# BruceCanovas/supersurfel_fusion

Hardware: AMD Instinct MI355X
Metric: frames_per_sec (higher is better)
Workload: dtype f32; 1 GPU; 640x480 synthetic RGB-D orbit (seed 1234), map seeded with 1000000 supersurfels (~993223 live, ~86081 visible), reference rgbd_benchmark parameters, extract+ICP+fuse per frame; width=640, height=480, n_model=993223, n_visible=86081, superpixels=1200, icp_iter_max=10, icp_forced=False, seed_order=seeded, exchange=none, pipeline_depth=2, extract_batch=8

## Files before the change

### supersurfel_fusion_amd/csrc/lab/host_probes.inc

```

int ssf_dbg_last_icp_record(ssf_handle* h, int64_t* out29) {
    if (!h || !out29) return SSF_ERR_INVALID_ARG;
    for (int i = 0; i < 29; i++) out29[i] = h->h_icp_local[i];
    return SSF_OK;
}
int ssf_dbg_device_icp_records(ssf_handle* h, int64_t* out64) {
    if (!h || !out64) return SSF_ERR_INVALID_ARG;
    HCK(hipStreamSynchronize(h->stream));
    HCK(hipMemcpy(out64, h->d_icp, 64 * sizeof(int64_t), hipMemcpyDeviceToHost));
    return SSF_OK;
}
void ssf_dbg_stall_before_match_us(ssf_handle* h, long long us) { if (h) h->dbg_stall_before_match_us = us; }
int ssf_dbg_host_times(ssf_handle* h, double* out8) {
    if (!h || !out8) return SSF_ERR_INVALID_ARG;
    for (int i = 0; i < 8; i++) { out8[i] = h->host_us[i]; h->host_us[i] = 0; }
    return SSF_OK;
}
double ssf_dbg_extract_only(ssf_handle* h, const void* const* rgb, const void* const* depth, int nlist, int n) {
    if (!h || !rgb || !depth || nlist <= 0 || !h->pending.empty()) return -1.0;
    int nsub = 0;
    double t0 = 0;
    for (int i = 0; i < n; i++) {
        if (i == n / 4) { for (auto& c : h->ctx) (void)hipStreamSynchronize(c.stream); (void)hipStreamSynchronize(h->stream); t0 = now_us(); }
        while (nsub < n && !h->ctx[h->open_ctx].launched) {
            if (submit_extract(h, rgb[nsub % nlist], depth[nsub % nlist], 1, nullptr)) return -1.0;
            nsub++;
        }
        if (activate_oldest(h) || retire_active(h)) return -1.0;
        h->stamp++;
    }
    for (auto& c : h->ctx) (void)hipStreamSynchronize(c.stream);
    (void)hipStreamSynchronize(h->stream);
    return (now_us() - t0) / (double)(n - n / 4);
}
double ssf_dbg_time_icp(ssf_handle* h, int reps, int dbg) {
    if (!h || !h->have_frame) return -1.0;
    Rt T; T.R = m3_transpose(h->pose.R); T.t = negate(m3_mulv(T.R, h->pose.t));
    hipEvent_t e0, e1; (void)hipEventCreate(&e0); (void)hipEventCreate(&e1);
    for (int i = 0; i < 3; i++) launch_icp(h->stream, h->cam, h->model[h->mcur], h->n_visible, h->cc->maps.pix2, h->cc->maps.fpack, T, h->d_icp_replicas, h->d_tickets + 8, h->d_icp, h->mb_dev, ++h->icp_seq, dbg);
    (void)hipEventRecord(e0, h->stream);
    for (int i = 0; i < reps; i++) launch_icp(h->stream, h->cam, h->model[h->mcur], h->n_visible, h->cc->maps.pix2, h->cc->maps.fpack, T, h->d_icp_replicas, h->d_tickets + 8, h->d_icp, h->mb_dev, ++h->icp_seq, dbg);
    (void)hipEventRecord(e1, h->stream);
    (void)hipStreamSynchronize(h->stream);
    float ms = 0.f; (void)hipEventElapsedTime(&ms, e0, e1);
    (void)hipMemsetAsync(h->d_icp_replicas, 0, 2 * SSF_ICP_REPLICAS * 32 * sizeof(long long), h->stream);
    (void)hipMemsetAsync(h->d_tickets, 0, 512 * sizeof(unsigned int), h->stream);
    (void)hipStreamSynchronize(h->stream);
    (void)hipEventDestroy(e0); (void)hipEventDestroy(e1);
    return 1000.0 * ms / reps;
}
double ssf_dbg_time_fuse(ssf_handle* h, int reps, int mode, long long* blocks2 ) {
    if (!h || !h->have_frame || !h->cc) return -1.0;
    SurfelSoA& M = h->model[h->mcur];
    PartitionWs ws;
    uint32_t* set = h->d_part + (size_t)h->part_set * h->part_words;
    ws.sup_vis = set; ws.sup_oov = set + h->part_sup_vis; ws.tot = ws.sup_oov + h->part_sup_oov;
    ws.ticket = h->d_part_ticket; ws.other = h->d_part + (size_t)(h->part_set ^ 1) * h->part_words; ws.words = h->part_words;
    const int S = (mode & 2) ? 0 : h->S, nvis = (mode & 4) ? 0 : h->n_visible, span = (mode & 1) ? 0 : h->oov_tail - h->oov_head;
    auto launch = [&] {
        ClassifyArgs ca = h->classify; ca.plane_depth = h->cc->maps.plane_depth;
        launch_fuse(h->stream, M, h->cc->frame, h->pose, h->stamp, h->id_offset, nvis, AssocTables{h->cc->d_best, h->cc->d_matched, h->d_cand, S},
                    (nvis > 0 && S > 0) ? 1 : 0, h->cfg.nb_supersurfels_max, ShardArgs{0, 1, 0, h->cfg.shard_tile}, h->d_cnt,
                    h->oov[h->ocur], span, ca, h->d_state, h->d_state_oov, h->d_bc_oov, ws, 1);
    };
    hipEvent_t e0, e1; (void)hipEventCreate(&e0); (void)hipEventCreate(&e1);
    for (int i = 0; i < 3 && reps > 0; i++) launch();
    (void)hipEventRecord(e0, h->stream);
    for (int i = 0; i < reps; i++) launch();
    (void)hipEventRecord(e1, h->stream);
    (void)hipStreamSynchronize(h->stream);
    float ms = 0.f; (void)hipEventElapsedTime(&ms, e0, e1);
    (void)hipEventDestroy(e0); (void)hipEventDestroy(e1);
    if (blocks2) {
        const int nb = (span + 255) / 256;
        std::vector<uint32_t> bc((size_t)std::max(nb, 1));
        if (nb > 0) (void)hipMemcpy(bc.data(), h->d_bc_oov, (size_t)nb * 4, hipMemcpyDeviceToHost);
        blocks2[0] = nb; blocks2[1] = 0;
        for (int i = 0; i < nb; i++) blocks2[1] += bc[i] != 0u;
    }
    return reps > 0 ? 1000.0 * ms / reps : 0.0;
}
int ssf_dbg_trace_fuse(ssf_handle* h, unsigned long long* out, int cap_wgs, int* arms4, int mode ) {
    if (!h || !h->have_frame || !h->cc || !out || !arms4) return -1;
    arms4[0] = (mode & 2) ? 0 : (h->S + 31) / 32; arms4[1] = (mode & 2) ? 0 : (h->S + 255) / 256; arms4[2] = (mode & 4) ? 0 : (h->n_visible + 255) / 256;
    long long b2[2];
    unsigned long long* d = nullptr;
    const size_t words = (size_t)3 * 65536;
    if (hipMalloc((void**)&d, words * 8) != hipSuccess) return -2;
    (void)hipMemset(d, 0, words * 8);
    set_fuse_trace(d);
    (void)ssf_dbg_time_fuse(h, 1, mode, b2);
    set_fuse_trace(nullptr);
    std::vector<unsigned long long> all(words);
    (void)hipMemcpy(all.data(), d, words * 8, hipMemcpyDeviceToHost);
    (void)hipFree(d);
    int n = 0;
    for (int i = 0; i < 65536; i++) if (all[3 * (size_t)i]) n = i + 1;
    arms4[3] = n - arms4[0] - arms4[1] - arms4[2];
    const int m = n < cap_wgs ? n : cap_wgs;
    std::memcpy(out, all.data(), (size_t)m * 24);
    return m;
}
int ssf_dbg_pass_stats_enable(int on) { set_pass_stats(on ? 1 : 0); return SSF_OK; }
int ssf_dbg_pass_stats(ssf_handle* h, uint32_t* out64) {
    if (!h || !h->active.ctx || !out64) return SSF_ERR_INVALID_ARG;
    HCK(hipStreamSynchronize(h->active.ctx->stream));
    HCK(hipMemcpy(out64, h->active.maps.epoch, 64 * sizeof(uint32_t), hipMemcpyDeviceToHost));
    return SSF_OK;
}
double ssf_dbg_time_pass(ssf_handle* h, int reps, int rgbd, int dbg, int nb) {
    if (!h || !h->active.ctx) return -1.0;
    ExtractCtx& c = *h->active.ctx;
    nb = std::max(1, std::min(nb, h->batch));
    hipEvent_t e0, e1; (void)hipEventCreate(&e0); (void)hipEventCreate(&e1);
    const int ox[4] = {0, 1, 0, 1}, oy[4] = {0, 1, 1, 0};
    for (int i = 0; i < 4; i++) launch_update_pass(h->stream, h->seg, c.maps, nb, 20 + i, ox[i & 3], oy[i & 3], rgbd != 0, dbg);
    (void)hipEventRecord(e0, h->stream);
    for (int i = 0; i < reps; i++) launch_update_pass(h->stream, h->seg, c.maps, nb, 24 + i, ox[i & 3], oy[i & 3], rgbd != 0, dbg);
    (void)hipEventRecord(e1, h->stream);
    (void)hipStreamSynchronize(h->stream);
    float ms = 0.f; (void)hipEventElapsedTime(&ms, e0, e1);
    (void)hipEventDestroy(e0); (void)hipEventDestroy(e1);
    return 1000.0 * ms / reps;
}
int ssf_dbg_trace_pass(ssf_handle* h, int rgbd, int nb, unsigned long long* out, int cap_wgs, int* grid3) {
    if (!h || !h->active.ctx || !out || !grid3) return -1;
    ExtractCtx& c = *h->active.ctx;
    nb = std::max(1, std::min(nb, h->batch));
    const int ox[4] = {0, 1, 0, 1}, oy[4] = {0, 1, 1, 0};
    grid3[0] = (h->cfg.width + 30 + 31) / 32; grid3[1] = (h->cfg.height + 31) / 32; grid3[2] = nb;
    const int n = grid3[0] * grid3[1] * grid3[2];
    unsigned long long* d = nullptr;
    if (hipMalloc((void**)&d, (size_t)n * 40) != hipSuccess) return -2;
    (void)hipMemset(d, 0, (size_t)n * 40);
    for (int i = 0; i < 4; i++) launch_update_pass(h->stream, h->seg, c.maps, nb, 20 + i, ox[i & 3], oy[i & 3], rgbd != 0, 0);
    (void)hipStreamSynchronize(h->stream);
    set_pass_trace(d);
    launch_update_pass(h->stream, h->seg, c.maps, nb, 24, ox[0], oy[0], rgbd != 0, 0);
    (void)hipStreamSynchronize(h->stream);
    set_pass_trace(nullptr);
    const int m = std::min(n, cap_wgs);
    (void)hipMemcpy(out, d, (size_t)m * 40, hipMemcpyDeviceToHost);
    (void)hipFree(d);
    return m;
// ... 2 lines not shown
```

### supersurfel_fusion_amd/csrc/ssf_device.hpp

```cpp
#pragma once
#include <hip/hip_runtime.h>
#include <stdint.h>
#include <cstddef>
#include "ssf_math.hpp"
#include "../../include/ssf.h"
#include "../../include/ssf_input.h"
#include "../../include/ssf_dynamic.h"

#ifdef SSF_EXPERIMENTS
#include <stdlib.h>
static inline int ssf_env_int_(const char* name, int dflt) { const char* e = getenv(name); return e ? atoi(e) : dflt; }
#define SSF_ENV_INT(name, dflt) ssf_env_int_("SSF_" name, dflt)
#define SSF_ENV_SET(name) (getenv("SSF_" name) != nullptr)
#define SSF_ENV_STR(name) getenv("SSF_" name)
#define SSF_PROBE(dbg, bits) ((((dbg)) & (bits)) != 0)
#else
#define SSF_PROBE(dbg, bits) (false)
#define SSF_ENV_INT(name, dflt) (dflt)
#define SSF_ENV_SET(name) (false)
#define SSF_ENV_STR(name) ((const char*)nullptr)
#endif

namespace ssf {

// ... 77 lines not shown
    for (int i = 0; i < 3; i++) {
        m.log.ent[i] = slab_shift(m.log.ent[i], o); m.log.disp[i] = slab_shift(m.log.disp[i], o);
        m.log.count[i] = slab_shift(m.log.count[i], o);
    }
    m.sp = slab_shift(m.sp, o); m.samples = slab_shift(m.samples, o); m.sample_score = slab_shift(m.sample_score, o);
    m.moments = slab_shift(m.moments, o); m.filt = slab_shift(m.filt, o); m.epoch = slab_shift(m.epoch, o);
    m.pix2 = slab_shift(m.pix2, o); m.fpack = slab_shift(m.fpack, o);
    return m;
}
SSF_HD SurfelSoA batch_slot(SurfelSoA s, size_t o) {
    s.pos = slab_shift(s.pos, o); s.col = slab_shift(s.col, o); s.lab = slab_shift(s.lab, o); s.stamps = slab_shift(s.stamps, o);
    s.r0 = slab_shift(s.r0, o); s.r1 = slab_shift(s.r1, o); s.r2 = slab_shift(s.r2, o); s.shape = slab_shift(s.shape, o);
    s.dims = slab_shift(s.dims, o); s.conf = slab_shift(s.conf, o);
    return s;
}
struct BatchIn {
    const uint8_t* rgb[SSF_MAX_BATCH];
    const void* depth[SSF_MAX_BATCH];
    int color_format, depth_format;
    double depth_scale;
};
template <typename T> SSF_HD T batch_pick(const T* arr, int b) {
    T v = arr[0];
#pragma unroll
    for (int i = 1; i < SSF_MAX_BATCH; i++) v = (b == i) ? arr[i] : v;
    return v;
}

struct Mailbox {
    alignas(64) unsigned long long icp_rec[40];
    Counters cnt;
    unsigned long long cnt_check;
    unsigned long long cnt_seq;
    int all_cnt[5 * SSF_MAX_RANKS];
    unsigned long long all_check;
    unsigned long long all_seq;
    unsigned int p2p_timeout;
    unsigned int extract_abort;
};
#ifndef SSF_ICP_REPLICAS
#define SSF_ICP_REPLICAS 8
#endif
#define SSF_ICP_REC_WORD(w, p, seq) ((((w) & 7) == 7) ? (unsigned long long)(seq) : ((7 * ((w) >> 3) + ((w) & 7)) < 30 ? (unsigned long long)(p)[7 * ((w) >> 3) + ((w) & 7)] : 0ull))

void launch_ingest(hipStream_t st, const SegParams& p, const BatchIn& in, FrameMaps& m, int nb, uint32_t epoch0);
int pass_tile_npx(int nb);
void launch_update_pass(hipStream_t st, const SegParams& p, FrameMaps& m, int nb, int k, int ox, int oy, bool rgbd, int dbg = 0);
size_t pass_team_ws_bytes();
size_t pass_args_bytes(int kmax);
void pass_args_table(const SegParams& p, const FrameMaps& m, int kmax, void* host_out);
void launch_update_passes_team(hipStream_t st, const SegParams& p, FrameMaps& m, int nb, int k0, int k1, bool rgbd, const void* d_pas, void* d_ws,
                               unsigned int* abort_flag);
void launch_init_samples(hipStream_t st, const SegParams& p, FrameMaps& m, int nb, int true_buf);
void launch_eval_samples(hipStream_t st, const SegParams& p, FrameMaps& m, int nb);
void launch_init_disp(hipStream_t st, const SegParams& p, FrameMaps& m, int nb, bool ransac);
void launch_plane_filter(hipStream_t st, const SegParams& p, FrameMaps& m, int nb, int true_buf);
void launch_import_frame(hipStream_t st, const SegParams& p, FrameMaps& m, int nb, SurfelSoA frame, const float* wire, unsigned long long* best, uint8_t* matched);
void launch_export_rows(hipStream_t st, const SegParams& p, const FrameMaps& m, int nb, SurfelSoA frame, float* wire);
void launch_render_moments(hipStream_t st, const SegParams& p, const Cam& cam, FrameMaps& m, int nb);
void launch_render_moments_pixmask(hipStream_t st, const SegParams& p, const Cam& cam, FrameMaps& m, int nb, const uint8_t* pixmask,
                                   uint32_t* pixcnt);
void launch_finalize_surfels(hipStream_t st, const SegParams& p, FrameMaps& m, int nb, SurfelSoA frame, float zmin,
                             float zmax, int stamp0, const uint8_t* dynamic_mask, unsigned mask_bits,
                             unsigned long long* best, uint8_t* matched);
void launch_finalize_surfels_pixmask(hipStream_t st, const SegParams& p, FrameMaps& m, int nb, SurfelSoA frame, float zmin, float zmax,
                                     int stamp0, const uint8_t* dynamic_mask, unsigned mask_bits, unsigned long long* best, uint8_t* matched,
                                     const uint32_t* pixcnt, unsigned pixmask_bits);
void launch_bilateral(hipStream_t st, const void* in, int depth_format, double depth_scale, float* out, int W, int H, float sigma_color,
                      float sigma_space);
void launch_bilateral_batch(hipStream_t st, const BatchIn& in, float* out0, size_t slab, int nb, int W, int H, float sigma_color, float sigma_space);
void launch_boundary_map(hipStream_t st, const SegParams& p, const int32_t* label, int32_t* out);
void launch_preview(hipStream_t st, int W, int H, const int32_t* label, const uint32_t* rgba, uint8_t* out );

struct alignas(64) IcpGo { float T[12]; unsigned long long flag; unsigned long long x; };
static_assert(sizeof(IcpGo) == 64, "one line");
#define SSF_ICP_GO_ABORT (1ull << 63)
#define SSF_ICP_GO_MATCH (1ull << 62)
#define SSF_ICP_GO_CHECK_MASK 0x3FFFFFFFu
SSF_HD unsigned int icp_go_word_weight(unsigned int dword) {
    return dword < 12u ? (2u * dword + 1u) * 0x9E3779B1u : (dword == 14u ? 0x85EBCA6Bu : (dword == 15u ? 0xC2B2AE35u : 0u));
}
SSF_HD unsigned int icp_go_abort_check(unsigned int want) { return ((want * 0x9E3779B1u) >> 2) & SSF_ICP_GO_CHECK_MASK; }
#define SSF_ICP_GO_SLOTS 4
struct MatchArgs { float zmin, zmax; long long id_offset; unsigned long long* best; uint8_t* matched; int32_t* cand; };
struct ClassifyArgs { Cam cam; const float* plane_depth; int delta_t; float conf_thresh, zmin, zmax; };
struct ShardArgs { int rank, nranks, migrate; float tile; };
struct AssocTables { const unsigned long long* best; const uint8_t* matched; const int32_t* cand; int S; };
int icp_variant_mode();
void launch_icp(hipStream_t st, const Cam& cam, SurfelSoA model, int n_visible, const uint2* pix2, const float4* fpack,
                Rt T, long long* replicas, unsigned int* ticket,
                long long* sums29, Mailbox* mb, unsigned long long seq, int dbg = -1, IcpGo* go = nullptr,
                unsigned long long go_seq = 0, const struct P2PView* pv = nullptr, int by_tile = 0, const MatchArgs* match = nullptr);
int icp_resident_max_wgs();
void launch_icp_resident(hipStream_t st, const Cam& cam, SurfelSoA model, int n_visible, const uint2* pix2, const float4* fpack, const Rt* T0,
                         long long* replicas, long long* sums29, Mailbox* mb, unsigned long long seq0, IcpGo* go, unsigned int go_base,
                         int last_idx, const MatchArgs* match);
void launch_bin_rows(hipStream_t st, const Cam& cam, SurfelSoA model, int n, Rt T, uint32_t* count, uint32_t* cursor, SurfelSoA out);
size_t bin_buffer_words(const Cam& cam, size_t capacity);
void launch_match(hipStream_t st, const Cam& cam, SurfelSoA model, int n_visible, const uint2* pix2, const float4* fpack,
                  Rt pose, float zmin, float zmax, long long id_offset,
                  unsigned long long* best, uint8_t* matched, int32_t* cand , int S,
                  const int32_t* orig = nullptr );
struct OovStore { SurfelSoA rows; uint8_t* live; int cap; };
#define PART_GROUP 16
#define PART_REPLICAS 8
struct PartitionWs { uint32_t* sup_vis; uint32_t* sup_oov; uint32_t* tot; uint32_t* ticket; uint32_t* other; int words; };
void launch_fuse(hipStream_t st, SurfelSoA model , SurfelSoA frame, Rt pose, int stamp, long long id_offset,
                 int n_visible, const AssocTables& at, int do_update, int capacity, const ShardArgs& sh, Counters* cnt, OovStore oov,
                 int span_upper, const ClassifyArgs& ca, uint8_t* state_vis, uint8_t* state_oov, uint32_t* bc_oov, const PartitionWs& ws,
                 int tail_in_move = 0 );
#ifdef SSF_EXPERIMENTS
void set_pass_stats(int on);
void set_pass_trace(unsigned long long* device_words );
void set_fuse_trace(unsigned long long* device_words );
#endif
struct MoveTotals { int from_tot, nv , head_old, tail_old ; };
void launch_pack_emigrants(hipStream_t st, SurfelSoA model, const AssocTables& at, long long id_offset, int n_visible,
                           const uint8_t* state_vis, int do_update, const ShardArgs& sh, int32_t* table);
void launch_migrate_in(hipStream_t st, SurfelSoA model, const int32_t* table, int S, int capacity, Counters* cnt, const ShardArgs& sh,
                       const ClassifyArgs& ca, Rt pose, int stamp, uint8_t* state_vis, const PartitionWs& ws);
void launch_rehome_split(hipStream_t st, SurfelSoA dense, int n, int n_visible, int rank, int nranks, float tile, uint32_t* bc, int* tot3,
                         SurfelSoA stay, int32_t* table, int table_rows);
void launch_rehome_unpack(hipStream_t st, const int32_t* table, int n, SurfelSoA dst, int base);
void launch_first_frame(hipStream_t st, SurfelSoA model, SurfelSoA frame, Rt pose, int S, int capacity, const ShardArgs& sh, Counters* cnt);
struct NextIcp {
    Cam cam; const uint2* pix2; const float4* fpack;
    Rt T;
    long long* replicas; unsigned int* ticket; long long* sums; Mailbox* mb; unsigned long long seq;
};
void launch_move_rows(hipStream_t st, SurfelSoA vis_src, SurfelSoA vis_dst, OovStore oov, int nv_upper, int span_upper,
                      const uint8_t* state_vis, const uint8_t* state_oov, const uint32_t* bc_oov, const PartitionWs& ws,
                      Counters* cnt , Mailbox* mb, unsigned long long cnt_seq, const NextIcp* next,
                      const struct P2PView* next_pv = nullptr, const MoveTotals* totals = nullptr);
void launch_oov_compact(hipStream_t st, OovStore src, OovStore dst, int span_upper, int new_head, uint32_t* bc_oov, Counters* cnt,
                        int set_span);
struct ModelView { SurfelSoA vis; OovStore oov; int n_visible, nbv, nvs, oov_head, oov_tail, nbo, nslots; };
void launch_align(hipStream_t st, const Cam& cam, const float* spos, const float* slab, const float* snrm, const float* sconf,
                  int n, SurfelSoA frame, const int32_t* label, const float* plane_depth, Rt T, long long* out40);
void launch_fern_codes(hipStream_t st, const uint8_t* rgb, const float* depth, int W, int H, const uint32_t* fpos,
                       const uint8_t* frgb, const float* fdepth, int n, uint8_t* codes);
#define SSF_P2P_MAX_RANKS 8
struct P2PView { unsigned char* peer[SSF_P2P_MAX_RANKS]; int me, nranks, S; unsigned long long seq, timeout_ticks; };
enum { P2P_FLAG_ASSOC = 0, P2P_FLAG_MIGR = 1 };
#define SSF_P2P_HEADER 8192
SSF_HD size_t p2p_slot(int par, int src) { return (size_t)(par * SSF_P2P_MAX_RANKS + src); }
SSF_HD size_t p2p_spad(int S) { return ((size_t)S + 63) & ~(size_t)63; }
SSF_HD size_t p2p_off_icp(int par, int src) { return p2p_slot(par, src) * 320; }
SSF_HD size_t p2p_off_cnt(int par, int src) { return 16 * 320 + p2p_slot(par, src) * 64; }
SSF_HD size_t p2p_off_flag(int kind, int par, int src) { return 16 * 384 + ((size_t)kind * 16 + p2p_slot(par, src)) * 64; }
SSF_HD size_t p2p_off_best(int S, int par, int src) { return SSF_P2P_HEADER + p2p_slot(par, src) * (size_t)S * 8; }
SSF_HD size_t p2p_off_matched(int S, int par, int src) { return SSF_P2P_HEADER + 16 * (size_t)S * 8 + p2p_slot(par, src) * p2p_spad(S); }
SSF_HD size_t p2p_off_migr(int S, int par, int src) {
    return SSF_P2P_HEADER + 16 * (size_t)S * 8 + 16 * p2p_spad(S) + p2p_slot(par, src) * (size_t)S * SSF_MIGRANT_WORDS * 4;
}
SSF_HD size_t p2p_region_bytes(int S) { return p2p_off_migr(S, 1, SSF_P2P_MAX_RANKS - 1) + (size_t)S * SSF_MIGRANT_WORDS * 4; }
void launch_p2p_counts(hipStream_t st, const P2PView& pv, const Counters* cnt, Mailbox* mb, unsigned long long all_seq);
void launch_p2p_assoc(hipStream_t st, const P2PView& pv, unsigned long long* best, uint8_t* matched, Mailbox* mb);
void launch_p2p_migrants(hipStream_t st, const P2PView& pv, int32_t* table, unsigned int* ticket , Mailbox* mb);
void launch_publish_icp(hipStream_t st, const long long* rec29, Mailbox* mb, unsigned long long seq);
void launch_publish_all_counts(hipStream_t st, const int* all5, int nranks, Mailbox* mb, unsigned long long seq);
void launch_publish_counts(hipStream_t st, Counters* cnt, int shrink_by_removed, Mailbox* mb, unsigned long long seq);
void launch_lab_refresh(hipStream_t st, SurfelSoA s, int n);
void launch_pack_orient(hipStream_t st, SurfelSoA s, int n, float* out9);
void launch_deformation(hipStream_t st, SurfelSoA model, int n, int m, const float* npos, const float* nrot,
                        const float* ntrans, float* nodes16, const float* w4, const int32_t* idx4);

struct KernelTimer;
KernelTimer* current_timer();
void set_current_timer(KernelTimer* t);
void timer_begin(KernelTimer* t, const char* name, hipStream_t st);
// ... 9 lines not shown
```

### supersurfel_fusion_amd/csrc/ssf_extract.hip

```cpp
#include <stdio.h>
#include <stdlib.h>
#include <string.h>
#include <algorithm>
#include <mutex>
#include "ssf_device.hpp"

namespace ssf {

#define HIP_CHECK_LAUNCH() (void)hipGetLastError()

__device__ __forceinline__ int lane_id() { return threadIdx.x & 63; }
__device__ __forceinline__ void atomic_add_i64(long long* p, long long v) {
    atomicAdd(reinterpret_cast<unsigned long long*>(p), static_cast<unsigned long long>(v));
}
template <int CF> __device__ __forceinline__ uint32_t load_rgb(const uint8_t* __restrict__ p, size_t q) {
    if (CF == SSF_COLOR_RGBA8 || CF == SSF_COLOR_BGRA8) {
        const uint32_t v = reinterpret_cast<const uint32_t*>(p)[q];
        return CF == SSF_COLOR_RGBA8 ? (v & 0xFFFFFFu) : (((v & 0xFFu) << 16) | (v & 0xFF00u) | ((v >> 16) & 0xFFu));
    }
    const uint32_t c0 = p[3 * q], c1 = p[3 * q + 1], c2 = p[3 * q + 2];
    return CF == SSF_COLOR_BGR8 ? (c2 | (c1 << 8) | (c0 << 16)) : (c0 | (c1 << 8) | (c2 << 16));
}
template <int DF> __device__ __forceinline__ float load_depth(const void* __restrict__ p, size_t q, double scale) {
    if (DF == SSF_DEPTH_U16_SCALED) return (float)((double)reinterpret_cast<const uint16_t*>(p)[q] * scale);
// ... 994 lines not shown
            for (int j = 0; j < 12; j++) lds_add_i64(&a[j], fx64((double)v[j], SSF_MOM_SCALE, SSF_MOM_LIM));
            lds_add_i64(&a[12], 1);
        } else {
#pragma unroll
            for (int j = 0; j < 12; j++) atomic_add_i64(&m.moments[(size_t)label * 13 + j], fx64((double)v[j], SSF_MOM_SCALE, SSF_MOM_LIM));
            atomic_add_i64(&m.moments[(size_t)label * 13 + 12], 1);
        }
    }
#pragma unroll
    for (int k = 0; k < PX; k++) {
        if (out_label[k] < 0) continue;
        const int i = threadIdx.x + 256 * k;
        const size_t q = (size_t)(Y0 + i / TILE) * p.W + (X0 + i % TILE);
        m.plane_depth[q] = out_depth[k];
        m.pix2[q] = make_uint2((uint32_t)out_label[k], __float_as_uint(out_depth[k]));
    }
    __syncthreads();
    for (int i = threadIdx.x; i < win.size() * 13; i += blockDim.x) {
        long long v = 0;
#pragma unroll
        for (int r = 0; r < MOM_REP(WCAP); r++) v += (long long)w_acc[((i / 13) * MOM_REP(WCAP) + r) * 13 + i % 13];
        if (v != 0) atomic_add_i64(&m.moments[(size_t)win.label_of(i / 13, p.gy) * 13 + i % 13], v);
    }
    if constexpr (PIXMASK)
        for (int i = threadIdx.x; i < win.size(); i += blockDim.x) {
            uint32_t v = 0;
#pragma unroll
            for (int r = 0; r < MOM_REP(WCAP); r++) v += w_pix[i * MOM_REP(WCAP) + r];
            if (v == 0) continue;
            const size_t l = (size_t)win.label_of(i, p.gy);
            atomicAdd(&pixcnt[2 * l], v & 0xFFFFu);
            if (v >> 16) atomicAdd(&pixcnt[2 * l + 1], v >> 16);
        }
}

#define FIN_PER_WG 64
template <bool PIXMASK>
__global__ __launch_bounds__(256) void k_finalize_surfels(SegParams p, FrameMaps m, SurfelSoA f, float zmin, float zmax, int stamp0,
                                                          const uint8_t* __restrict__ dyn_mask, unsigned mask_bits,
                                                          unsigned long long* __restrict__ best, uint8_t* __restrict__ matched,
                                                          const uint32_t* __restrict__ pixcnt, unsigned pixmask_bits) {
    __shared__ float s_axis[2][FIN_PER_WG][3];
    const int wv = threadIdx.x >> 6, l = threadIdx.x & 63;
    const int kk = wv < 2 ? wv * 32 + (l >> 1) : l;
    const int k = blockIdx.x * FIN_PER_WG + kk;
    const bool active = k < p.S && wv < 3;
    const int fb = blockIdx.y;
    const size_t off = (size_t)fb * m.slab;
    m = batch_slot(m, fb); f = batch_slot(f, off);
    best = slab_shift(best, off); matched = slab_shift(matched, off);
    dyn_mask = ((mask_bits >> fb) & 1u) ? slab_shift(dyn_mask, off) : nullptr;
    const int stamp = stamp0 + fb;
    float sum[12]; float conf = 0.f;
#pragma unroll
    for (int j = 0; j < 12; j++) sum[j] = 0.f;
    if (active) {
        const long long* a = &m.moments[(size_t)k * 13];
        const double inv = 1.0 / SSF_MOM_SCALE;
#pragma unroll
        for (int j = 0; j < 12; j++) sum[j] = (float)((double)a[j] * inv);
        conf = (float)a[12];
    }
    V3 pos = v3(sum[0], sum[1], sum[2]), col = v3(sum[3], sum[4], sum[5]);
    Sym3 shape = sym3(sum[6], sum[7], sum[8], sum[9], sum[10], sum[11]);
    const float z = pos.z / conf;
    const bool valid = active && isfinite(z) && conf > 100.0f && z > zmin && z < zmax;
    if (valid) {
        pos = v3(pos.x / conf, pos.y / conf, z);
        shape = sym_sub(sym_div(shape, conf), sym_outer(pos));
    }
    V3 lab = v3(0.f, 0.f, 0.f);
    if (wv < 2) {
        if (valid) {
            const V3 axis = principal_power(principal_start(shape, (l & 1) == 1));
            s_axis[l & 1][kk][0] = axis.x; s_axis[l & 1][kk][1] = axis.y; s_axis[l & 1][kk][2] = axis.z;
        }
    } else if (wv == 2 && active) {
        if (valid) col = lab_to_rgb(v3(col.x / conf, col.y / conf, col.z / conf));
        lab = rgb_to_lab(col);
    }
    __syncthreads();
    if (wv != 2 || !active) return;
    best[k] = SSF_NO_MATCH; matched[k] = 0;
    M3 vecs = m3(v3(0, 0, 0), v3(0, 0, 0), v3(0, 0, 0));
    float d0 = 0.f, d1 = 0.f; int s0 = 0, s1 = 0;
    if (valid) {
        V3 vals;
        principal_finish(shape, v3(s_axis[0][kk][0], s_axis[0][kk][1], s_axis[0][kk][2]),
                         v3(s_axis[1][kk][0], s_axis[1][kk][1], s_axis[1][kk][2]), vecs, vals);
        d0 = vals.x; d1 = vals.y; s0 = stamp; s1 = stamp;
        if (vals.x / vals.y > 50.0f) conf = -1.0f;
    } else
        conf = -1.0f;
    if (dyn_mask && dyn_mask[k]) conf = -1.0f;
    if constexpr (PIXMASK) {
        if ((pixmask_bits >> fb) & 1u) {
            const uint32_t* c = slab_shift(pixcnt, off);
            const uint32_t total = c[2 * k], masked = c[2 * k + 1];
            if (masked > 0u && 2ull * masked >= (unsigned long long)total) conf = -1.0f;
        }
    }
    f.pos[3 * k] = pos.x; f.pos[3 * k + 1] = pos.y; f.pos[3 * k + 2] = pos.z;
    f.col[3 * k] = col.x; f.col[3 * k + 1] = col.y; f.col[3 * k + 2] = col.z;
    f.lab[3 * k] = lab.x; f.lab[3 * k + 1] = lab.y; f.lab[3 * k + 2] = lab.z;
    f.stamps[2 * k] = s0; f.stamps[2 * k + 1] = s1;
    f.r0[3 * k] = vecs.r0.x; f.r0[3 * k + 1] = vecs.r0.y; f.r0[3 * k + 2] = vecs.r0.z;
    f.r1[3 * k] = vecs.r1.x; f.r1[3 * k + 1] = vecs.r1.y; f.r1[3 * k + 2] = vecs.r1.z;
    f.r2[3 * k] = vecs.r2.x; f.r2[3 * k + 1] = vecs.r2.y; f.r2[3 * k + 2] = vecs.r2.z;
    f.shape[6 * k] = shape.xx; f.shape[6 * k + 1] = shape.xy; f.shape[6 * k + 2] = shape.xz;
    f.shape[6 * k + 3] = shape.yy; f.shape[6 * k + 4] = shape.yz; f.shape[6 * k + 5] = shape.zz;
    f.dims[2 * k] = d0; f.dims[2 * k + 1] = d1;
    f.conf[k] = conf;
    m.fpack[4 * k] = make_float4(conf, lab.x, lab.y, lab.z);
    m.fpack[4 * k + 1] = make_float4(vecs.r2.x, vecs.r2.y, vecs.r2.z, 0.f);
    m.fpack[4 * k + 2] = make_float4(pos.x, pos.y, pos.z, 0.f);
}

__global__ __launch_bounds__(256) void k_import_frame(int P, int S, FrameMaps m, SurfelSoA f, const float* __restrict__ wire,
                                                      unsigned long long* __restrict__ best, uint8_t* __restrict__ matched) {
    {
        const size_t off = (size_t)blockIdx.y * m.slab;
        m = batch_slot(m, blockIdx.y); f = batch_slot(f, off); wire = slab_shift(wire, off);
        best = slab_shift(best, off); matched = slab_shift(matched, off);
    }
    const int i = blockIdx.x * blockDim.x + threadIdx.x;
    if (i < P) m.pix2[i] = make_uint2((uint32_t)m.label[i], __float_as_uint(m.plane_depth[i]));
    if (i >= S) return;
    const int k = i;
    const float* wpos = wire; const float* wcol = wpos + 3 * (size_t)S; const int32_t* wst = reinterpret_cast<const int32_t*>(wcol + 3 * (size_t)S);
    const float* wori = reinterpret_cast<const float*>(wst + 2 * (size_t)S); const float* wsh = wori + 9 * (size_t)S;
    const float* wd = wsh + 6 * (size_t)S; const float* wc = wd + 2 * (size_t)S;
    const V3 pos = v3(wpos[3 * k], wpos[3 * k + 1], wpos[3 * k + 2]), col = v3(wcol[3 * k], wcol[3 * k + 1], wcol[3 * k + 2]);
    const V3 lab = rgb_to_lab(col);
    const V3 r2 = v3(wori[9 * k + 6], wori[9 * k + 7], wori[9 * k + 8]);
    const float conf = wc[k];
    f.pos[3 * k] = pos.x; f.pos[3 * k + 1] = pos.y; f.pos[3 * k + 2] = pos.z;
    f.col[3 * k] = col.x; f.col[3 * k + 1] = col.y; f.col[3 * k + 2] = col.z;
    f.lab[3 * k] = lab.x; f.lab[3 * k + 1] = lab.y; f.lab[3 * k + 2] = lab.z;
    f.stamps[2 * k] = wst[2 * k]; f.stamps[2 * k + 1] = wst[2 * k + 1];
#pragma unroll
    for (int j = 0; j < 3; j++) { f.r0[3 * k + j] = wori[9 * k + j]; f.r1[3 * k + j] = wori[9 * k + 3 + j]; f.r2[3 * k + j] = wori[9 * k + 6 + j]; }
#pragma unroll
    for (int j = 0; j < 6; j++) f.shape[6 * k + j] = wsh[6 * k + j];
    f.dims[2 * k] = wd[2 * k]; f.dims[2 * k + 1] = wd[2 * k + 1];
    f.conf[k] = conf;
    m.fpack[4 * k] = make_float4(conf, lab.x, lab.y, lab.z);
    m.fpack[4 * k + 1] = make_float4(r2.x, r2.y, r2.z, 0.f);
    m.fpack[4 * k + 2] = make_float4(pos.x, pos.y, pos.z, 0.f);
    best[k] = SSF_NO_MATCH; matched[k] = 0;
}

__global__ __launch_bounds__(256) void k_export_rows(int S, SurfelSoA f, float* __restrict__ wire, size_t slab) {
    const int k = blockIdx.x * blockDim.x + threadIdx.x;
    if (k >= S) return;
    const size_t off = (size_t)blockIdx.y * slab;
    f = batch_slot(f, off); wire = slab_shift(wire, off);
    float* wpos = wire; float* wcol = wpos + 3 * (size_t)S; int32_t* wst = reinterpret_cast<int32_t*>(wcol + 3 * (size_t)S);
    float* wori = reinterpret_cast<float*>(wst + 2 * (size_t)S); float* wsh = wori + 9 * (size_t)S;
    float* wd = wsh + 6 * (size_t)S; float* wc = wd + 2 * (size_t)S;
#pragma unroll
    for (int j = 0; j < 3; j++) {
        wpos[3 * k + j] = f.pos[3 * k + j]; wcol[3 * k + j] = f.col[3 * k + j];
        wori[9 * k + j] = f.r0[3 * k + j]; wori[9 * k + 3 + j] = f.r1[3 * k + j]; wori[9 * k + 6 + j] = f.r2[3 * k + j];
    }
    wst[2 * k] = f.stamps[2 * k]; wst[2 * k + 1] = f.stamps[2 * k + 1];
#pragma unroll
    for (int j = 0; j < 6; j++) wsh[6 * k + j] = f.shape[6 * k + j];
    wd[2 * k] = f.dims[2 * k]; wd[2 * k + 1] = f.dims[2 * k + 1];
    wc[k] = f.conf[k];
}
__global__ __launch_bounds__(256) void k_boundary_map(SegParams p, const int32_t* __restrict__ label, int32_t* __restrict__ out) {
    __shared__ int tile[TW * TW];
    const int X0 = blockIdx.x * TILE, Y0 = blockIdx.y * TILE;
    load_label_tile(tile, label, X0, Y0, p.W, p.H);
    __syncthreads();
    for (int i = threadIdx.x; i < TILE * TILE; i += blockDim.x) {
        const int x = X0 + i % TILE, y = Y0 + i / TILE;
        if (x < p.W && y < p.H) out[(size_t)y * p.W + x] = tile_boundary(tile, i % TILE + 1, i / TILE + 1);
    }
}

__global__ __launch_bounds__(256) void k_preview(int W, int H, const int32_t* __restrict__ label, const uint32_t* __restrict__ rgba,
                                                 uint8_t* __restrict__ out) {
    const int x = blockIdx.x * 64 + (threadIdx.x & 63), y = blockIdx.y * 4 + (threadIdx.x >> 6);
    if (x >= W || y >= H) return;
    const size_t p = (size_t)y * W + x;
    const int index = label[p];
    uint8_t b0 = 255, b1 = 255, b2 = 255;
    if (!(x < W - 1 && y < H - 1 && (label[p + 1] != index || label[p + W + 1] != index))) {
        const uint32_t c = rgba[p];
        b0 = (uint8_t)(0.8f * (float)((c >> 16) & 255u)); b1 = (uint8_t)(0.8f * (float)((c >> 8) & 255u)); b2 = (uint8_t)(0.8f * (float)(c & 255u));
    }
    out[3 * p] = b0; out[3 * p + 1] = b1; out[3 * p + 2] = b2;
}
void launch_preview(hipStream_t st, int W, int H, const int32_t* label, const uint32_t* rgba, uint8_t* out) {
    hipLaunchKernelGGL(k_preview, dim3((W + 63) / 64, (H + 3) / 4), dim3(256), 0, st, W, H, label, rgba, out);
}

#define BIL_RMAX 16
#define BIL_TILE 16
__device__ __forceinline__ int reflect101(int i, int n) {
    if (n == 1) return 0;
    while (i < 0 || i >= n) i = (i < 0) ? -i : 2 * (n - 1) - i;
    return i;
}
template <int DF>
__global__ __launch_bounds__(256) void k_bilateral(BatchIn bin, float* __restrict__ out0, size_t slab, int W, int H,
                                                   int radius, float ss, float sc) {
    const void* __restrict__ in = batch_pick(bin.depth, (int)blockIdx.z);
    const double scale = bin.depth_scale;
    float* __restrict__ out = slab_shift(out0, (size_t)blockIdx.z * slab);
    __shared__ float tile[(BIL_TILE + 2 * BIL_RMAX) * (BIL_TILE + 2 * BIL_RMAX)];
    __shared__ int s_ext[2 * BIL_RMAX + 1];
    const int X0 = blockIdx.x * BIL_TILE, Y0 = blockIdx.y * BIL_TILE;
    const int tw = BIL_TILE + 2 * radius;
    const bool staged = radius <= BIL_RMAX;
    if (staged) {
        for (int i = threadIdx.x; i < tw * tw; i += blockDim.x) {
            const int gx = reflect101(X0 - radius + i % tw, W), gy = reflect101(Y0 - radius + i / tw, H);
            tile[i] = load_depth<DF>(in, (size_t)gy * W + gx, scale);
        }
        if ((int)threadIdx.x <= 2 * radius) {
            const int dy = (int)threadIdx.x - radius;
            int e = 0;
            while ((e + 1) * (e + 1) + dy * dy <= radius * radius) e++;
            s_ext[threadIdx.x] = e;
        }
    }
    __syncthreads();
    const int lx = threadIdx.x % BIL_TILE, ly = threadIdx.x / BIL_TILE;
    const int x = X0 + lx, y = Y0 + ly;
    if (x >= W || y >= H) return;
// ... 335 lines not shown
```

### supersurfel_fusion_amd/csrc/ssf_handle.hpp

```cpp
#pragma once
#include <algorithm>
#include <climits>
#include <cmath>
#include <cstring>
#include <deque>
#include <initializer_list>
#include <map>
#include <string>
#include <utility>
#include <vector>
#include "ssf_device.hpp"
#include "../../include/ssf_render.h"
#include "../../include/ssf_graph.h"
#include "../../include/ssf_graph_solve.h"
#include "../../include/ssf_keyframes.h"
#include "../../include/ssf_motion.h"
#include "../../include/ssf_odometry.h"
#include "../../include/ssf_navgrid.h"
#include "../../include/ssf_track.h"

struct ncclComm; typedef struct ncclComm* ncclComm_t;
struct Uploader;
namespace ssf {
struct KernelTimer {
// ... 158 lines not shown
    uint4* ferns = nullptr; uint32_t* q = nullptr; uint32_t* table = nullptr; int32_t* stamps = nullptr; uint32_t* diff = nullptr;
    int32_t* rec = nullptr; uint8_t* bytes = nullptr;
    ssf_surfels pool{};
    std::vector<ssf_fern> host_ferns; std::vector<KeyframeMeta> kfs; long long rows_used = 0;
};
struct QueryWs {
    DevBufs bufs;
    unsigned long long* mask = nullptr; uint32_t* cnt = nullptr; uint32_t* bc = nullptr; size_t slots = 0;
    uint32_t* rec = nullptr;
    unsigned char* rows = nullptr; size_t rows_bytes = 0;
};
struct NavGridWs {
    DevBufs bufs;
    float4* rec = nullptr; uint2* rbox = nullptr; size_t slots = 0;
    uint32_t* tcnt = nullptr; uint32_t* cursor = nullptr; size_t tiles = 0;
    uint32_t* list = nullptr; size_t list_cap = 0;
    uint32_t* acc = nullptr; uint16_t* colg = nullptr; int8_t* state = nullptr; size_t cells = 0;
    unsigned long long* stats = nullptr;
    unsigned char* img = nullptr; size_t img_bytes = 0;
};
struct RayIndex {
    float cell, s, k;
    uint32_t mask;
    int cmin[3], cmax[3];
    int n_over, nvs;
    float cabs;
};
struct RaycastWs {
    DevBufs bufs;
    float4* rec = nullptr; uint4* rbox = nullptr; uint32_t* bc = nullptr; uint32_t* over = nullptr; size_t slots = 0;
    uint32_t* off = nullptr; uint32_t* cursor = nullptr; size_t buckets = 0;
    uint32_t* list = nullptr; size_t list_cap = 0;
    unsigned long long* stats = nullptr; int* cbox = nullptr;
    unsigned char* io = nullptr; size_t io_bytes = 0;
    RayIndex ix{};
    bool built = false; unsigned long long gen = 0; long long recentres = 0; float cell = 0, s = 0; int hash_bits = 0;
    long long rows_indexed = 0, rows_oversize = 0, entries = 0;
};
struct ssf_handle {
    ssf_config cfg;
    int S = 0, gx = 0, gy = 0;
    std::string err;
    hipStream_t stream = nullptr; bool own_stream = false; int stream_prio = 0;
    SegParams seg; Cam cam;
    std::vector<ExtractCtx> ctx; int open_ctx = 0, batch = 1;
    std::deque<std::pair<int, int>> pending;
    ActiveFrame active; ActiveFrame* cc = &active;
    uint32_t extract_ordinal = 0;
    const void* const* seq_rgb = nullptr; const void* const* seq_depth = nullptr; const uint8_t* const* seq_pixmask = nullptr; int seq_next = 0, seq_n = 0, seq_on_device = 0, stamp_bias = 0;
    long long n_waiter_matches = 0;
    int seq_k = 0;
    int seq_batches = 0;
    double us_wait_upload = 0.0;
    Uploader* up = nullptr; bool seq_upload = false;
    int in_color = SSF_COLOR_RGB8, in_depth = SSF_DEPTH_F32_METRES; double in_scale = 1.0;
    ncclComm_t comm = nullptr; int* d_all5 = nullptr;
    int deal = 0; long long deal_batches = 0;
    struct P2P {
        unsigned char* region = nullptr; size_t bytes = 0; bool fine = false;
        bool same_device = false; double timeout_s = 30.0;
        P2PView view{}; bool on = false; std::vector<void*> opened;
        unsigned long long seq_icp = 0, seq_cnt = 0, seq_assoc = 0, seq_migr = 0;
    } p2p;
    unsigned long long all_seq = 0; bool all_pending = false, all_valid = false;
    long long all_cnt[5 * SSF_MAX_RANKS];
    SurfelSoA model[2]; int mcur = 0;
    std::vector<void*> allocs;
    struct Guarded { void* base; size_t bytes, guard; };
    std::vector<Guarded> guarded;
    float* d_bf_in = nullptr; float* d_bf_out = nullptr; float* d_orient9 = nullptr; float* d_frame_orient9 = nullptr;
    long long* d_icp = nullptr;
    uint8_t* d_state = nullptr; int32_t* d_cand = nullptr; Counters* d_cnt = nullptr;
    int32_t* d_migrants = nullptr; PartitionWs fuse_ws{}; bool fuse_first = false, fuse_migrate = false, fusing = false;
    MoveTotals fuse_totals{0, 0, 0, 0}; bool move_totals_on = true;
    OovStore oov[2]; int ocur = 0; int oov_head = 0, oov_tail = 0, oov_live = 0; long long n_recentres = 0;
    uint8_t* d_state_oov = nullptr; uint32_t* d_bc_oov = nullptr;
    uint32_t* d_part = nullptr; uint32_t* d_part_ticket = nullptr; int part_words = 0, part_sup_vis = 0, part_sup_oov = 0, part_set = 0;
    SurfelSoA dense; uint8_t* d_live_scratch = nullptr;
    int32_t* d_scratch_map = nullptr;
    long long* d_icp_replicas = nullptr; unsigned int* d_tickets = nullptr; float* d_srgb_lut = nullptr;
    Mailbox* mb_host = nullptr; Mailbox* mb_dev = nullptr;
    unsigned long long icp_seq = 0, cnt_seq = 0;
    struct { bool valid = false; unsigned long long seq = 0; ExtractCtx* ctx = nullptr; int slot = 0; int stamp = 0; Rt pose; } ahead;
    double wait_launched_us = 0.0; long long n_waiter_match_repairs = 0; long long dbg_stall_before_match_us = 0;
    bool icp_ahead = true; int icp_ahead_mode = 1;
    AheadTuner ahead_tuner;
    IcpGo* go = nullptr; bool icp_chain = true; unsigned long long go_count = 0;
    IcpGo* go_res = nullptr; int resident_max_rows = 0; long long n_resident_frames = 0, n_resident_ahead_frames = 0, n_resident_launches = 0;
    bool graph_failed = false; hipStream_t capture_stream = nullptr;
    TileCopy bins;
    ClassifyArgs classify{}; ShardArgs shard{};
    bool pass_team = false; ExtractCtx* team_prev = nullptr;
    long long h_icp_local[SSF_ICP_RECORD];
    long long* h_icp = nullptr; Counters* h_cnt = nullptr;
    int n_model = 0, n_visible = 0, stamp = 0, max_passes = 0;
    Rt pose;
    IcpLoop icp;
    long long id_offset = 0, global_n_model = -1, global_n_visible = -1;
    bool have_frame = false;
    int last_icp_valid = 0, last_icp_iters = 0;
    hipEvent_t ev[4] = {nullptr, nullptr, nullptr, nullptr};
    KernelTimer timer;
    std::vector<std::string> timer_names;
    double seq_mark_us[4][64] = {{0}}, seq_launch_us[32] = {0}, seq_launch_host_us[32] = {0}; int seq_launch_n[32] = {0}, seq_launches = 0;
    double seq_t0_us = 0, seq_done_us[64] = {0};
    double host_us[8] = {0, 0, 0, 0, 0, 0, 0, 0};
    RenderWs render;
    GraphWs graph;
    KeyframeWs kf;
    SolveWs solve;
    QueryWs query;
    MotionWs motion;
    OdoWs odo;
    NavGridWs navgrid;
    RaycastWs raycast;
    unsigned long long model_gen = 0;
};

#define HCK(call)                                                                                    \
    do {                                                                                             \
        hipError_t e_ = (call);                                                                      \
        if (e_ != hipSuccess) {                                                                      \
            h->err = std::string(#call) + ": " + hipGetErrorString(e_);                              \
            return SSF_ERR_DEVICE;                                                                   \
        }                                                                                            \
    } while (0)

#pragma GCC visibility push(hidden)
namespace ssf {
struct DevTemps {
    std::vector<void*> p;
    template <typename T> hipError_t take(T** out, size_t bytes) {
        void* q = nullptr;
        const hipError_t e = hipMalloc(&q, bytes ? bytes : 1);
        if (e == hipSuccess) { p.push_back(q); *out = (T*)q; }
        return e;
    }
    ~DevTemps() { for (void* q : p) (void)hipFree(q); }
};
struct TimerScope { ssf_handle* h; explicit TimerScope(ssf_handle* hh); ~TimerScope(); };
void timer_collect(KernelTimer* t);
inline int sync_collect(ssf_handle* h) {
    HCK(hipStreamSynchronize(h->stream)); if (h->cfg.profile == 1) timer_collect(&h->timer); return SSF_OK;
}
ModelView model_view(const ssf_handle* h, bool visible_only);
int model_at_rest(ssf_handle* h, const char* who = nullptr, const char* lacks = nullptr);
int materialise(ssf_handle* h);
bool frame_inputs_ok(ssf_handle* h, const void* rgb, const void* depth, int on_device);
int process_frame_devmask(ssf_handle* h, const void* rgb, const void* depth, int on_device, const float* prior, const uint8_t* d_pixmask,
                          ssf_frame_result* out);
int store_from_dense(ssf_handle* h, int n, int n_visible);
void drop_shard_sizes(ssf_handle* h);
void set_create_error(const char* what);
template <typename T> bool dalloc(ssf_handle* h, T** p, size_t count);
int wait_seq(ssf_handle* h, const volatile unsigned long long* word, unsigned long long want);
SurfelSoA soa_rows(const SurfelSoA& s, size_t r);
int copy_soa(ssf_handle* h, const SurfelSoA& d, const SurfelSoA& s, size_t n);
inline P2PView p2p_view(ssf_handle* h, unsigned long long seq) { P2PView v = h->p2p.view; v.seq = seq; return v; }
inline Rt pose_from12(const float* p) {
    Rt r; r.R = m3(v3(p[0], p[1], p[2]), v3(p[3], p[4], p[5]), v3(p[6], p[7], p[8])); r.t = v3(p[9], p[10], p[11]); return r;
}
inline void pose_to12(const Rt& r, float* p) {
    p[0] = r.R.r0.x; p[1] = r.R.r0.y; p[2] = r.R.r0.z; p[3] = r.R.r1.x; p[4] = r.R.r1.y; p[5] = r.R.r1.z;
    p[6] = r.R.r2.x; p[7] = r.R.r2.y; p[8] = r.R.r2.z; p[9] = r.t.x; p[10] = r.t.y; p[11] = r.t.z;
}
int align_loop(ssf_handle* h, const float* d_pos, const float* d_lab, const float* d_nrm, const float* d_conf, int n, long long* d_out,
// ... 13 lines not shown
```

### supersurfel_fusion_amd/csrc/ssf_host.hip

```cpp
#include <atomic>
#include <chrono>
#include <cstdio>
#include <cstdlib>
#include <new>
#include <condition_variable>
#include <mutex>
#include <thread>
#include <type_traits>
#include <unistd.h>
#include "ssf_exchange.hpp"
#include "ssf_solvers.hpp"

using namespace ssf;

namespace ssf {
static thread_local KernelTimer* g_timer = nullptr;
KernelTimer* current_timer() { return g_timer; }
void set_current_timer(KernelTimer* t) { g_timer = t; }
void timer_begin(KernelTimer* t, const char* name, hipStream_t st) {
    KernelTimer::Rec r;
    if (!t->pool_free.empty()) { r = t->pool_free.back(); t->pool_free.pop_back(); }
    else { (void)hipEventCreate(&r.e0); (void)hipEventCreate(&r.e1); }
    r.name = name;
    (void)hipEventRecord(r.e0, st);
// ... 673 lines not shown
int copy_soa(ssf_handle* h, const SurfelSoA& d, const SurfelSoA& s, size_t n) {
    if (n == 0) return SSF_OK;
    hipError_t copy_of_a_stream = hipSuccess;
    each_stream([&](auto m, size_t w) { if (!copy_of_a_stream) copy_of_a_stream = hipMemcpyAsync(d.*m, s.*m, 4 * w * n, hipMemcpyDeviceToDevice, h->stream); });
    HCK(copy_of_a_stream);
    return SSF_OK;
}
static int oov_home(const ssf_handle* h) { return h->cfg.nb_supersurfels_max + h->S + 256; }
static int oov_recentre(ssf_handle* h) {
    OovStore& src = h->oov[h->ocur]; OovStore& dst = h->oov[h->ocur ^ 1];
    HCK(hipMemsetAsync(dst.live, 0, (size_t)dst.cap, h->stream));
    launch_oov_compact(h->stream, src, dst, h->oov_tail - h->oov_head, oov_home(h), h->d_bc_oov, h->d_cnt, 1);
    HCK(hipGetLastError());
    h->ocur ^= 1;
    h->oov_head = oov_home(h); h->oov_tail = h->oov_head + h->oov_live;
    h->n_recentres++;
    return SSF_OK;
}
int materialise(ssf_handle* h) {
    int rc = copy_soa(h, h->dense, h->model[h->mcur], (size_t)h->n_visible);
    if (rc) return rc;
    if (h->oov_live > 0) {
        OovStore dst; dst.rows = h->dense; dst.live = h->d_live_scratch; dst.cap = h->cfg.nb_supersurfels_max;
        launch_oov_compact(h->stream, h->oov[h->ocur], dst, h->oov_tail - h->oov_head, h->n_visible, h->d_bc_oov, h->d_cnt, 0);
        HCK(hipGetLastError());
    }
    return SSF_OK;
}
int store_from_dense(ssf_handle* h, int n, int n_visible) {
    h->ahead.valid = false;
    h->bins.drop();
    h->model_gen++;
    int rc = copy_soa(h, h->model[h->mcur], h->dense, (size_t)n_visible);
    if (rc) return rc;
    OovStore& o = h->oov[h->ocur];
    const int head = oov_home(h), n_oov = n - n_visible;
    rc = copy_soa(h, soa_rows(o.rows, (size_t)head), soa_rows(h->dense, (size_t)n_visible), (size_t)n_oov);
    if (rc) return rc;
    HCK(hipMemsetAsync(o.live, 0, (size_t)o.cap, h->stream));
    if (n_oov > 0) HCK(hipMemsetAsync(o.live + head, 1, (size_t)n_oov, h->stream));
    Counters c; std::memset(&c, 0, sizeof(c));
    c.n_model = n; c.n_visible = n_visible; c.oov_head = head; c.oov_tail = head + n_oov; c.oov_live = n_oov;
    c.last[0] = n; c.last[1] = n_visible;
    HCK(hipStreamSynchronize(h->stream));
    HCK(hipMemcpy(h->d_cnt, &c, sizeof(c), hipMemcpyHostToDevice));
    h->n_model = n; h->n_visible = n_visible; h->oov_head = c.oov_head; h->oov_tail = c.oov_tail; h->oov_live = n_oov;
    return SSF_OK;
}
void drop_shard_sizes(ssf_handle* h) { h->all_valid = false; h->all_pending = false; }
}

static int do_match(ssf_handle* h, int exchange = 0) {
    const bool any = total_model(h) > 0 && total_visible(h) > 0;
    const int n = any ? h->n_visible : 0;
    launch_match(h->stream, h->cam, icp_rows(h), n, h->cc->maps.pix2, h->cc->maps.fpack, h->pose, h->cfg.range_min,
                 h->cfg.range_max, h->id_offset, h->cc->d_best, h->cc->d_matched, h->d_cand, h->S, h->bins.valid ? h->bins.d_idx : nullptr);
    if (exchange && h->p2p.on) launch_p2p_assoc(h->stream, p2p_view(h, ++h->p2p.seq_assoc), h->cc->d_best, h->cc->d_matched, h->mb_dev);
    HCK(hipGetLastError());
    return SSF_OK;
}

static int fuse_begin(ssf_handle* h, int migrate) {
    const long long nmodel_g = total_model(h), nvis_g = total_visible(h);
    SurfelSoA& M = h->model[h->mcur];
    h->bins.drop();
    h->fuse_first = !(nmodel_g > 0);
    h->fuse_migrate = migrate && h->cfg.nranks > 1 && !h->fuse_first;
    h->classify.plane_depth = h->cc->maps.plane_depth; h->shard.migrate = h->fuse_migrate ? 1 : 0;
    if (nmodel_g > 0) {
        {
            const int span = h->oov_tail - h->oov_head;
            if (h->oov_head < h->n_visible + h->S + 256 || h->oov[h->ocur].cap - h->oov_tail < 2 * h->S + 256 ||
                span > h->oov_live + h->oov_live / 4 + 65536) { int rc2 = oov_recentre(h); if (rc2) return rc2; }
        }
        h->fuse_totals.from_tot = (single_shard_alone(h) && !h->fuse_migrate && h->move_totals_on) ? 1 : 0;
        h->fuse_totals.nv = h->n_visible; h->fuse_totals.head_old = h->oov_head; h->fuse_totals.tail_old = h->oov_tail;
        PartitionWs& ws = h->fuse_ws;
        {
            uint32_t* set = h->d_part + (size_t)h->part_set * h->part_words;
            ws.sup_vis = set; ws.sup_oov = set + h->part_sup_vis; ws.tot = ws.sup_oov + h->part_sup_oov;
            ws.ticket = h->d_part_ticket; ws.other = h->d_part + (size_t)(h->part_set ^ 1) * h->part_words; ws.words = h->part_words;
            h->part_set ^= 1;
        }
        const AssocTables at{h->cc->d_best, h->cc->d_matched, h->d_cand, h->S};
        launch_fuse(h->stream, M, h->cc->frame, h->pose, h->stamp, h->id_offset, h->n_visible, at, nvis_g > 0 ? 1 : 0,
                    h->cfg.nb_supersurfels_max, h->shard, h->d_cnt, h->oov[h->ocur], h->oov_tail - h->oov_head, h->classify,
                    h->d_state, h->d_state_oov, h->d_bc_oov, ws, h->fuse_totals.from_tot);
        if (h->fuse_migrate)
            launch_pack_emigrants(h->stream, M, at, h->id_offset, h->n_visible, h->d_state, nvis_g > 0 ? 1 : 0, h->shard, h->d_migrants);
    }
    HCK(hipGetLastError());
    h->fusing = true;
    h->model_gen++;
    return SSF_OK;
}
static int fuse_end(ssf_handle* h, const int32_t* d_table, ssf_frame_result* out) {
    SurfelSoA& M = h->model[h->mcur];
    const unsigned long long seq = ++h->cnt_seq;
    h->fusing = false;
    if (!h->fuse_first) {
        const PartitionWs& ws = h->fuse_ws;
        if (h->fuse_migrate && d_table)
            launch_migrate_in(h->stream, M, d_table, h->S, h->cfg.nb_supersurfels_max, h->d_cnt, h->shard, h->classify, h->pose, h->stamp,
                              h->d_state, ws);
        NextIcp next{};
        P2PView next_pv{};
        bool have_next = false;
        if (h->icp_ahead && (h->p2p.on || h->ahead_tuner.current() == 1) && icp_is_one_launch(h) && h->cfg.icp_iter > 0 && !h->pending.empty()) {
            ExtractCtx& nc = h->ctx[h->pending.front().first];
            const int nslot = h->pending.front().second;
            const bool multi = h->ctx.size() > 1;
            bool ready = nc.launched && (!multi || nc.waited);
            if (nc.launched && !ready && (h->icp_ahead_mode == 2 || h->p2p.on || hipEventQuery(nc.ev_done) == hipSuccess)) {
                HCK(hipStreamWaitEvent(h->stream, nc.ev_done, 0)); nc.waited = true; ready = true;
            }
            (void)hipGetLastError();
            if (ready) {
                const FrameMaps nm = batch_slot(nc.maps, nslot);
                IcpLoop first;
                icp_start_from(first, h->pose);
                next = NextIcp{h->cam, nm.pix2, nm.fpack, icp_transform(first), h->d_icp_replicas, h->d_tickets + 8, h->d_icp, h->mb_dev, ++h->icp_seq};
                if (h->p2p.on) next_pv = p2p_view(h, ++h->p2p.seq_icp);
                h->ahead.valid = true; h->ahead.seq = next.seq; h->ahead.ctx = &nc; h->ahead.slot = nslot;
                h->ahead.stamp = h->stamp + 1; h->ahead.pose = h->pose;
                have_next = true;
            }
        }
        if (exchanges_natively(h)) { int rg = comm_gather_counts(h); if (rg) return rg; }
        launch_move_rows(h->stream, M, h->model[h->mcur ^ 1], h->oov[h->ocur], h->n_visible + (h->fuse_migrate ? 2 : 1) * h->S, h->oov_tail - h->oov_head,
                         h->d_state, h->d_state_oov, h->d_bc_oov, ws, h->d_cnt, h->mb_dev, seq, have_next ? &next : nullptr,
                         have_next && h->p2p.on ? &next_pv : nullptr, h->fuse_totals.from_tot ? &h->fuse_totals : nullptr);
        h->mcur ^= 1;
    } else {
        launch_first_frame(h->stream, M, h->cc->frame, h->pose, h->S, h->cfg.nb_supersurfels_max, h->shard, h->d_cnt);
        launch_publish_counts(h->stream, h->d_cnt, 0, h->mb_dev, seq);
        if (exchanges_natively(h)) { int rg = comm_gather_counts(h); if (rg) return rg; }
    }
    HCK(hipGetLastError());
    { int rr = retire_active(h); if (rr) return rr; }
    h->stamp_bias = 1;
    while (h->seq_next < h->seq_n && !h->ctx[h->open_ctx].launched) {
        int rs = seq_submit(h);
        if (rs) { h->stamp_bias = 0; return rs; }
    }
    h->stamp_bias = 0;
    int rc = wait_seq(h, &h->mb_host->cnt_seq, seq);
    if (rc) return rc;
    Counters c;
    for (int attempt = 0;; attempt++) {
        unsigned long long check = seq;
        const int* srcw = reinterpret_cast<const int*>(&h->mb_host->cnt);
        int* dstw = reinterpret_cast<int*>(&c);
        for (int i = 0; i < (int)(sizeof(Counters) / sizeof(int)); i++) {
            dstw[i] = __atomic_load_n(&srcw[i], __ATOMIC_RELAXED);
            check += (unsigned long long)(unsigned int)dstw[i];
        }
        if (check == __atomic_load_n(&h->mb_host->cnt_check, __ATOMIC_ACQUIRE)) break;
        if (attempt > 100000) { h->err = "counter mailbox record failed its checksum"; return SSF_ERR_DEVICE; }
    }
    h->n_model = c.n_model; h->n_visible = c.n_visible;
    h->oov_head = c.oov_head; h->oov_tail = c.oov_tail; h->oov_live = c.oov_live;
    if (__atomic_load_n(&h->mb_host->extract_abort, __ATOMIC_ACQUIRE) != 0u) {
        __atomic_store_n(&h->mb_host->extract_abort, 0u, __ATOMIC_RELEASE);
        h->err = "a team launch of the relabelling passes could not get all its workgroups onto the GPU and gave up (the GPU is oversubscribed: "
                 "several processes?); the frames of that batch are invalid";
        return SSF_ERR_DEVICE;
    }
    if (h->p2p.on && __atomic_load_n(&h->mb_host->p2p_timeout, __ATOMIC_ACQUIRE) != 0u) {
        __atomic_store_n(&h->mb_host->p2p_timeout, 0u, __ATOMIC_RELEASE);
        h->err = "a peer's association / migrant tables never arrived (peer-to-peer exchange)"; return SSF_ERR_DEVICE;
    }
    if (out) {
        std::memset(out, 0, sizeof(*out));
        pose_to12(h->pose, out->pose);
        out->icp_valid = h->last_icp_valid; out->icp_iters = h->last_icp_iters;
        out->n_model = h->n_model; out->n_visible = h->n_visible; out->n_removed = c.n_removed;
        out->n_inserted = c.n_inserted; out->n_updated = c.n_updated; out->stamp = h->stamp;
        ExtractCtx* ec = h->active.ctx;
        float ms;
        if (h->cfg.profile != 0 && ec && ec->timed && hipEventElapsedTime(&ms, ec->ev_t0, ec->ev_t1) == hipSuccess)
            out->stage_ms[0] = ms / (float)ec->nb_launched;
    }
    h->stamp++;
    h->global_n_model = -1; h->global_n_visible = -1;
    if (h->cfg.profile == 1) { HCK(hipStreamSynchronize(h->stream)); timer_collect(&h->timer); }
    return SSF_OK;
}

static int do_fuse(ssf_handle* h, ssf_frame_result* out) {
    int rc = fuse_begin(h, 0);
    return rc ? rc : fuse_end(h, nullptr, out);
}

static bool icp_waiter_can_match(const ssf_handle* h) {
    static const bool off = SSF_ENV_SET("NO_MATCH_IN_WAITER");
    return !off && single_shard_alone(h) && h->cfg.profile == 0 && icp_variant_mode() == 0;
}
static int icp_launch_waiting(ssf_handle* h, IcpWaiter& w) {
    w.seq_rec = ++h->icp_seq;
    w.go_seq = ++h->go_count;
    w.slot = h->go + (w.go_seq % SSF_ICP_GO_SLOTS);
    h->wait_launched_us = now_us();
    Rt none; none.R = m3_identity(); none.t = v3(0, 0, 0);
    const P2PView pv = h->p2p.view;
    const MatchArgs ma{h->cfg.range_min, h->cfg.range_max, h->id_offset, h->cc->d_best, h->cc->d_matched, h->d_cand};
    const int rc = icp_issue(h, none, w.seq_rec, nullptr, w.slot, w.go_seq, h->p2p.on ? &pv : nullptr, icp_waiter_can_match(h) ? &ma : nullptr);
    w.waiting = rc == SSF_OK;
    return rc;
}
static bool icp_resident_ok(const ssf_handle* h) {
    return h->go_res && single_shard_alone(h) && !h->bins.valid && !h->cfg.depth_prefilter && icp_variant_mode() == 0 && h->n_visible > 0 &&
           h->n_visible <= h->resident_max_rows;
}
static int icp_launch_resident(ssf_handle* h, IcpWaiter& w, const Rt* T0, unsigned long long seq0) {
    const int last = h->cfg.icp_iter;
    IcpGo* lines = h->go_res + (size_t)(h->n_resident_launches++ & 1) * (size_t)(last + 1);
    const unsigned long long go_base = h->go_count;
    h->go_count += (unsigned long long)last;
    w.resident = true; w.slot = lines + 1; w.go_seq = go_base + 1;
    h->wait_launched_us = now_us();
    const MatchArgs ma{h->cfg.range_min, h->cfg.range_max, h->id_offset, h->cc->d_best, h->cc->d_matched, h->d_cand};
    launch_icp_resident(h->stream, h->cam, h->model[h->mcur], h->n_visible, h->cc->maps.pix2, h->cc->maps.fpack, T0, h->d_icp_replicas, h->d_icp, h->mb_dev,
                        seq0, lines, (unsigned int)go_base, last, icp_waiter_can_match(h) ? &ma : nullptr);
    HCK(hipGetLastError());
    w.waiting = true;
    if (!w.resident_counted) { w.resident_counted = true; h->n_resident_frames++; if (!T0) h->n_resident_ahead_frames++; }
    return SSF_OK;
}
static void icp_resident_iterate(ssf_handle* h, IcpWaiter& w, const Rt& T, unsigned long long seq_rec) {
    h->wait_launched_us = now_us();
    icp_release_waiting(w.slot, w.go_seq, &T, seq_rec);
    w.slot++; w.go_seq++;
}
static void icp_chain_reset(ssf_handle* h) {
    (void)hipStreamSynchronize(h->stream);
    (void)hipMemsetAsync(h->d_icp_replicas, 0, 2 * SSF_ICP_REPLICAS * 32 * sizeof(long long), h->stream);
    (void)hipMemsetAsync(h->d_tickets, 0, 512 * sizeof(unsigned int), h->stream);
    (void)hipStreamSynchronize(h->stream);
    h->icp_chain = false; h->ahead.valid = false;
}
struct TrackFrame { double t_a = 0.0, t_b = 0.0; int kf = -1; bool timing = false, first_it = true; IcpWaiter w; };
int TileCopy::make_if_large(ssf_handle* h) {
    if (!(h->icp.active && min_rows >= 0 && h->n_visible >= min_rows && h->n_visible > 0 && single_shard_alone(h) && bin_buffer_words(h->cam, 1) != 0)) return SSF_OK;
    if (!d_idx) {
        const size_t N = (size_t)h->cfg.nb_supersurfels_max, bw = bin_buffer_words(h->cam, N);
        const bool ok = bw && dalloc(h, &rows.pos, 12 * N) && dalloc(h, &d_idx, 1) && dalloc(h, &d_count, bw) && dalloc(h, &d_cursor, bw);
        if (!ok) { h->err = "allocation of the tile-sorted copy failed"; return SSF_ERR_DEVICE; }
    }
    Rt T0; T0.R = h->icp.R_init; T0.t = h->icp.t_init;
    launch_bin_rows(h->stream, h->cam, h->model[h->mcur], h->n_visible, T0, d_count, d_cursor, rows);
    HCK(hipGetLastError());
    valid = true;
    return SSF_OK;
}
static inline bool icp_chains(const ssf_handle* h) { return h->icp_chain && h->go && icp_is_one_launch(h) && h->cfg.profile != 1; }
static int icp_loop_chained(ssf_handle* h, TrackFrame& f) {
    IcpWaiter& w = f.w;
    int again = h->icp.active ? 1 : 0, rc;
    const bool resident = again && icp_resident_ok(h);
    while (again) {
        unsigned long long seq_rec;
        if (h->icp.ahead_seq) { seq_rec = h->icp.ahead_seq; h->icp.ahead_seq = 0; }
        else {
            const Rt T = icp_transform(h->icp);
            const unsigned long long xseq = h->p2p.on ? ++h->p2p.seq_icp : 0;
            if (resident) {
                seq_rec = ++h->icp_seq;
                if (w.waiting) icp_resident_iterate(h, w, T, seq_rec);
                else { rc = icp_launch_resident(h, w, &T, seq_rec); if (rc) return rc; }
            } else if (w.waiting) { icp_release_waiting(w.slot, w.go_seq, &T, xseq); seq_rec = w.seq_rec; w.waiting = false; }
            else {
                const P2PView pv = p2p_view(h, xseq);
                seq_rec = ++h->icp_seq;
                rc = icp_issue(h, T, seq_rec, nullptr, nullptr, 0, h->p2p.on ? &pv : nullptr);
                if (rc) return rc;
            }
        }
        if (resident) { if (!w.waiting) { rc = icp_launch_resident(h, w, nullptr, 0); if (rc) return rc; } }
        else if (h->icp.iter + 1 < h->cfg.icp_iter || (!f.timing && icp_waiter_can_match(h))) {
            rc = icp_launch_waiting(h, w);
            if (rc) return rc;
        }
        rc = icp_fetch(h, seq_rec, w.waiting ? &w : nullptr);
        if (rc) { if (w.waiting) icp_release_waiting(w.slot, w.go_seq, nullptr); icp_chain_reset(h); return rc; }
        if (f.first_it) { h->host_us[5] += now_us() - f.t_a; f.first_it = false; if (f.kf >= 0 && f.kf < 64) h->seq_mark_us[1][f.kf] = now_us() - h->seq_t0_us; }
        icp_update(h, (const int64_t*)h->h_icp, &again);
    }
    return SSF_OK;
}
static int icp_loop_plain(ssf_handle* h, TrackFrame& f) {
    int again = h->icp.active ? 1 : 0, rc;
    while (again) {
        if (h->p2p.on) {
            const P2PView pv = p2p_view(h, ++h->p2p.seq_icp);
            rc = icp_accumulate(h, true, nullptr, &pv);
        } else if (h->comm) {
            rc = icp_accumulate(h, false);
            if (rc) return rc;
            { ScopedKernel sk("exchange_icp_record", h->stream);
              NCK(rccl_api()->AllReduce(h->d_icp, h->d_icp, SSF_ICP_RECORD, ncclInt64, ncclSum, h->comm, h->stream)); }
            const unsigned long long seq = ++h->icp_seq;
            launch_publish_icp(h->stream, h->d_icp, h->mb_dev, seq);
            HCK(hipGetLastError());
            rc = icp_fetch(h, seq);
        } else if (h->icp.ahead_seq) {
            rc = icp_fetch(h, h->icp.ahead_seq);
            h->icp.ahead_seq = 0;
        } else
            rc = icp_accumulate(h, true);
        if (rc) return rc;
        if (f.first_it) { h->host_us[5] += now_us() - f.t_a; f.first_it = false; }
        icp_update(h, (const int64_t*)h->h_icp, &again);
    }
    return SSF_OK;
}
static int icp_loop_end(ssf_handle* h, TrackFrame& f) {
    IcpWaiter& w = f.w;
    int valid = 0; bool matched_by_waiter = false;
    if (w.waiting && !f.timing && icp_waiter_can_match(h)) {
        icp_end(h, &valid);
#ifdef SSF_EXPERIMENTS
        if (h->dbg_stall_before_match_us > 0) usleep((useconds_t)h->dbg_stall_before_match_us);
#endif
        icp_release_waiting(w.slot, w.go_seq, &h->pose, 0, true);
        matched_by_waiter = true;
        if (now_us() - h->wait_launched_us > 100000.0) { matched_by_waiter = false; h->n_waiter_match_repairs++; }
    } else {
        if (w.waiting) icp_release_waiting(w.slot, w.go_seq, nullptr);
        icp_end(h, &valid);
    }
    f.t_b = now_us();
    if (f.kf >= 0 && f.kf < 64) h->seq_mark_us[2][f.kf] = f.t_b - h->seq_t0_us;
    if (f.timing) HCK(hipEventRecord(h->ev[2], h->stream));
    if (matched_by_waiter) h->n_waiter_matches++;
    else { const int rc = do_match(h, 1); if (rc) return rc; }
    if (h->comm) {
        RcclApi* api = rccl_api();
        ScopedKernel sk("exchange_association", h->stream);
        NCK(api->AllReduce(h->cc->d_best, h->cc->d_best, h->S, ncclInt64, ncclMin, h->comm, h->stream));
        NCK(api->AllReduce(h->cc->d_matched, h->cc->d_matched, h->S, ncclUint8, ncclMax, h->comm, h->stream));
    }
    return SSF_OK;
}
static int exchange_and_fuse(ssf_handle* h, ssf_frame_result* r) {
    if (!exchanges_natively(h)) return do_fuse(h, r);
    static const int migrate = SSF_ENV_SET("NO_MIGRATE") ? 0 : 1;
    const int rc = fuse_begin(h, migrate);
    if (rc) { h->fusing = false; return rc; }
    if (h->fuse_migrate && h->p2p.on) launch_p2p_migrants(h->stream, p2p_view(h, ++h->p2p.seq_migr), h->d_migrants, h->d_tickets + 320, h->mb_dev);
    else if (h->fuse_migrate) {
        RcclApi* api = rccl_api();
        ScopedKernel sk("exchange_migrants", h->stream);
        const ncclResult_t nr = api->AllReduce(h->d_migrants, h->d_migrants, (size_t)SSF_MIGRANT_WORDS * h->S, ncclInt32, ncclSum, h->comm, h->stream);
        if (nr != ncclSuccess) {
            h->fusing = false;
            h->err = std::string("ncclAllReduce (migrant table): ") + (api->GetErrorString ? api->GetErrorString(nr) : "RCCL error");
            return SSF_ERR_DEVICE;
        }
    }
    return fuse_end(h, h->d_migrants, r);
}
static int stage_times(ssf_handle* h, ssf_frame_result* r) {
    HCK(hipEventRecord(h->ev[3], h->stream));
    HCK(hipEventSynchronize(h->ev[3]));
    float ms;
    ExtractCtx* ec = h->cc->ctx;
    if (hipEventElapsedTime(&ms, ec->ev_t0, ec->ev_t1) == hipSuccess) r->stage_ms[0] = ms / (float)ec->nb_launched;
    if (hipEventElapsedTime(&ms, h->ev[1], h->ev[2]) == hipSuccess) r->stage_ms[1] = ms;
    if (hipEventElapsedTime(&ms, h->ev[2], h->ev[3]) == hipSuccess) r->stage_ms[2] = ms;
    return SSF_OK;
}

static int process_oldest(ssf_handle* h, const float* prior, ssf_frame_result* out) {
    TimerScope ts(h);
    int rc = activate_oldest(h);
    if (rc) return rc;
    TrackFrame f;
    f.t_a = now_us();
    f.kf = h->seq_n > 0 ? h->seq_k : -1;
    if (f.kf >= 0 && f.kf < 64) { h->seq_mark_us[0][f.kf] = f.t_a - h->seq_t0_us; h->seq_mark_us[1][f.kf] = 0; }
    if (h->ctx.size() > 1 && hipEventQuery(h->cc->ctx->ev_done) == hipSuccess) h->host_us[4] += 1;
    f.timing = h->cfg.profile != 0 && h->cc->ctx->timed;
    if (f.timing) HCK(hipEventRecord(h->ev[1], h->stream));
    if (exchanges_natively(h)) { rc = comm_counts(h); if (rc) return rc; }
    icp_begin(h, prior);
    rc = h->bins.make_if_large(h);
    if (!rc) rc = icp_chains(h) ? icp_loop_chained(h, f) : icp_loop_plain(h, f);
    if (!rc) rc = icp_loop_end(h, f);
    ssf_frame_result r;
    if (!rc) rc = exchange_and_fuse(h, &r);
    if (rc) return rc;
    if (h->pending.empty()) h->ahead_tuner.sequence_break(); else h->ahead_tuner.frame_done(now_us(), r.icp_iters);
    h->host_us[1] += f.t_b - f.t_a; h->host_us[2] += now_us() - f.t_b; h->host_us[3] += 1;
    if (f.timing) { rc = stage_times(h, &r); if (rc) return rc; }
    if (out) *out = r;
    return SSF_OK;
}
static int process_frame_impl(ssf_handle* h, const void* rgb, const void* depth, int on_device, const float* prior,
                              const uint8_t* mask, ssf_frame_result* out, const uint8_t* pixmask = nullptr, int pixmask_on_device = -1) {
    if (!frame_args_ok(h, rgb, depth, on_device)) return SSF_ERR_INVALID_ARG;
    if (!h->pending.empty()) { h->err = "frames are pending in the extract pipeline: use ssf_process_submitted"; return SSF_ERR_STATE; }
    int rc;
    { TimerScope ts(h); rc = submit_extract(h, rgb, depth, on_device, mask, pixmask, pixmask_on_device < 0 ? on_device : pixmask_on_device); }
    return rc ? rc : process_oldest(h, prior, out);
}

namespace ssf {
bool frame_inputs_ok(ssf_handle* h, const void* rgb, const void* depth, int on_device) { return frame_args_ok(h, rgb, depth, on_device); }
int process_frame_devmask(ssf_handle* h, const void* rgb, const void* depth, int on_device, const float* prior, const uint8_t* d_pixmask,
                          ssf_frame_result* out) {
    return process_frame_impl(h, rgb, depth, on_device ? 1 : 0, prior, nullptr, out, d_pixmask, 1);
}
int copy_rows(ssf_handle* h, const ssf_surfels& dst, size_t d0, const ssf_surfels& src, size_t s0, size_t n, hipMemcpyKind kind) {
    if (n == 0) return SSF_OK;
    auto one = [&](auto* d, const auto* s, size_t w) { return d ? hipMemcpyAsync(d + w * d0, s + w * s0, 4 * w * n, kind, h->stream) : hipSuccess; };
    HCK(one(dst.positions, src.positions, 3)); HCK(one(dst.colors, src.colors, 3)); HCK(one(dst.stamps, src.stamps, 2));
    HCK(one(dst.orientations, src.orientations, 9)); HCK(one(dst.shapes, src.shapes, 6)); HCK(one(dst.dims, src.dims, 2));
    HCK(one(dst.confidences, src.confidences, 1));
    return SSF_OK;
}
static ssf_surfels soa_surfels(const SurfelSoA& s) { return ssf_surfels{s.pos, s.col, s.stamps, nullptr, s.shape, s.dims, s.conf}; }
ModelView model_view(const ssf_handle* h, bool visible_only) {
    ModelView mv;
    mv.vis = h->model[h->mcur]; mv.oov = h->oov[h->ocur];
    mv.n_visible = h->n_visible; mv.nbv = (h->n_visible + 255) / 256; mv.nvs = 256 * mv.nbv;
    mv.oov_head = h->oov_head; mv.oov_tail = h->oov_tail;
    mv.nbo = visible_only ? 0 : (h->oov_tail - h->oov_head + 255) / 256;
    mv.nslots = 256 * (mv.nbv + mv.nbo);
    return mv;
}
int model_at_rest(ssf_handle* h, const char* who, const char* lacks) {
    if (!h->pending.empty() || h->fusing) { h->err = "frames are pending in the extract pipeline"; return SSF_ERR_STATE; }
    if (who && h->cfg.nranks > 1) { h->err = std::string(who) + ": a sharded handle (cfg.nranks > 1) " + lacks; return SSF_ERR_STATE; }
    return SSF_OK;
}
int align_loop(ssf_handle* h, const float* d_pos, const float* d_lab, const float* d_nrm, const float* d_conf, int n, long long* d_out,
               const float* init_pose, float* rel_pose, int* valid, int* iters, int* pairs_last) {
    hipStream_t st = h->stream;
    int rc = SSF_OK;
    M3 R_init = m3_identity(); V3 t_init = v3(0, 0, 0);
    if (init_pose) { const Rt p0 = pose_from12(init_pose); R_init = p0.R; t_init = p0.t; }
    double tf_inc[16], JtJ[36];
    for (int i = 0; i < 16; i++) tf_inc[i] = (i % 5 == 0) ? 1.0 : 0.0;
    for (int i = 0; i < 36; i++) JtJ[i] = 0.0;
    M3 R_inc = m3_identity(); V3 t_inc = v3(0, 0, 0);
    bool ok = true;
    int it = 0, pairs = 0;
    static const int tri[6][6] = {{0, 1, 2, 3, 4, 5}, {1, 6, 7, 8, 9, 10}, {2, 7, 11, 12, 13, 14},
                                  {3, 8, 12, 15, 16, 17}, {4, 9, 13, 16, 18, 19}, {5, 10, 14, 17, 19, 20}};
    while (it < h->cfg.icp_iter) {
        it++;
        inc_to_float(tf_inc, R_inc, t_inc);
        Rt T; T.R = m3_mul(R_inc, R_init); T.t = add(m3_mulv(R_inc, t_init), t_inc);
        launch_align(st, h->cam, d_pos, d_lab, d_nrm, d_conf, n, h->cc->frame, h->cc->maps.label, h->cc->maps.plane_depth, T, d_out);
        long long rec[40];
        if (hipGetLastError() != hipSuccess || hipMemcpyAsync(rec, d_out, 37 * sizeof(long long), hipMemcpyDeviceToHost, st) != hipSuccess ||
            hipStreamSynchronize(st) != hipSuccess) { rc = SSF_ERR_DEVICE; h->err = "align iteration failed on the device"; break; }
        pairs = (int)rec[29];
        if (pairs < 100) { ok = false; break; }
        float cs[3], ct[3], scale;
        for (int i = 0; i < 3; i++) {
            const uint32_t a = (uint32_t)rec[30 + i], b = (uint32_t)rec[33 + i];
            std::memcpy(&cs[i], &a, 4); std::memcpy(&ct[i], &b, 4);
        }
        { const uint32_t a = (uint32_t)rec[36]; std::memcpy(&scale, &a, 4); }
        double Jtr[6];
        for (int i = 0; i < 6; i++) {
            for (int j = 0; j < 6; j++) JtJ[i * 6 + j] = (double)rec[tri[i][j]] / SSF_ICP_SCALE_JTJ;
            Jtr[i] = (double)rec[21 + i] / SSF_ICP_SCALE_JTR;
        }
        double tf_iter[16];
        align_increment(JtJ, Jtr, scale, cs, ct, tf_iter);
        mat4_lmul(tf_iter, tf_inc);
// ... 95 lines not shown
int ssf_create(const ssf_config* cfg, ssf_handle** out) {
    if (!cfg || !out) { g_create_err = "null argument"; return SSF_ERR_INVALID_ARG; }
    if (cfg->width <= 0 || cfg->height <= 0 || cfg->cell_size <= 0 || cfg->nb_samples <= 0 || cfg->nb_samples > 64 ||
        cfg->nb_supersurfels_max <= 0 || cfg->nranks < 1 || cfg->rank < 0 || cfg->rank >= cfg->nranks) {
        g_create_err = "invalid configuration"; return SSF_ERR_INVALID_ARG;
    }
    int ndev = 0;
    if (hipGetDeviceCount(&ndev) != hipSuccess || ndev <= 0) {
        g_create_err = "no HIP device: libssf_hip.so needs a gfx950 GPU (there is no CPU fallback)";
        return SSF_ERR_NO_DEVICE;
    }
    if (cfg->device_id < 0 || cfg->device_id >= ndev) { g_create_err = "device_id out of range"; return SSF_ERR_INVALID_ARG; }
    if (hipSetDevice(cfg->device_id) != hipSuccess) { g_create_err = "hipSetDevice failed"; return SSF_ERR_DEVICE; }
    ssf_handle* h = new (std::nothrow) ssf_handle();
    if (!h) return SSF_ERR_DEVICE;
    h->cfg = *cfg;
    const int W = cfg->width, H = cfg->height, c = cfg->cell_size;
    h->gx = (W + c - 1) / c; h->gy = (H + c - 1) / c; h->S = h->gx * h->gy;
    if (cfg->nb_supersurfels_max < h->S) { delete h; g_create_err = "nb_supersurfels_max < nbSuperpixels"; return SSF_ERR_INVALID_ARG; }
#ifndef SSF_MOVE_TOTALS_DEFAULT
#define SSF_MOVE_TOTALS_DEFAULT 1
#endif
    h->move_totals_on = SSF_ENV_INT("MOVE_TOTALS", SSF_MOVE_TOTALS_DEFAULT) != 0;
    h->icp_ahead_mode = SSF_ENV_INT("ICP_AHEAD", 1);
    h->icp_ahead = h->icp_ahead_mode != 0;
    h->ahead_tuner.forced = SSF_ENV_INT("ICP_AHEAD", -1);
    h->icp_chain = SSF_ENV_INT("ICP_CHAIN", 1) != 0;
    if (SSF_ENV_SET("NO_GRAPH")) h->graph_failed = true;
    if (cfg->stream) h->stream = (hipStream_t)cfg->stream;
    else {
        int least = 0, greatest = 0;
        (void)hipDeviceGetStreamPriorityRange(&least, &greatest);
        const int prio = SSF_ENV_INT("TRACK_PRIORITY", greatest);
        h->stream = stream_pool().take(cfg->device_id, prio);
        if (!h->stream) { delete h; g_create_err = "hipStreamCreate failed"; return SSF_ERR_DEVICE; }
        h->own_stream = true; h->stream_prio = prio;
    }
    SegParams& p = h->seg;
    p.W = W; p.H = H; p.cell = c; p.gx = h->gx; p.gy = h->gy; p.S = h->S; p.nb_samples = cfg->nb_samples;
    p.min_size = (int)((float)(c * c) / 4.f);
    p.lambda_pos = cfg->lambda_pos; p.lambda_bound = cfg->lambda_bound; p.lambda_size = cfg->lambda_size;
    p.lambda_disp = cfg->lambda_disp; p.thresh_disp = cfg->thresh_disp;
    p.filter_alpha = cfg->filter_alpha; p.filter_beta = cfg->filter_beta; p.filter_threshold = cfg->filter_threshold;
    p.filter_iter = cfg->filter_iter; p.seed = cfg->rng_seed;
    p.inv_gx = 1.0f / (float)h->gx;
    p.cell_magic = c > 1 ? (uint32_t)((0x100000000ull + (uint64_t)c - 1) / (uint64_t)c) : 0u;
    p.win_cells_max = tile_window_cells_max(p);
    h->cam.fx = cfg->fx; h->cam.fy = cfg->fy; h->cam.cx = cfg->cx; h->cam.cy = cfg->cy; h->cam.W = W; h->cam.H = H;
    h->classify = ClassifyArgs{h->cam, nullptr, cfg->delta_t, cfg->conf_thresh, cfg->range_min, cfg->range_max};
    h->shard = ShardArgs{cfg->rank, cfg->nranks, 0, cfg->shard_tile};
    const size_t P = (size_t)W * H, S = h->S, N = cfg->nb_supersurfels_max, NS = S * cfg->nb_samples;
    const size_t NT32 = (size_t)((W + 30 + 31) / 32) * ((H + 31) / 32), NT64 = (size_t)((W + 62 + 63) / 64) * ((H + 31) / 32);
    const size_t NT = std::max(NT32, 2 * NT64);
    const int nctx = std::max(0, std::min(cfg->pipeline_depth, SSF_MAX_PIPELINE_DEPTH)) + 1;
    h->batch = std::max(1, std::min(cfg->extract_batch, SSF_MAX_BATCH));
    h->ctx.resize(nctx);
    h->pass_team = SSF_ENV_INT("PASS_TEAM", 0) != 0;
    bool ok = dalloc(h, &h->d_srgb_lut, 256) && dalloc(h, &h->d_tickets, 512);
    {
        const int ne = pass_geometry_entries(W, H);
        std::vector<uint2> tab((size_t)ne);
        p.pass_geom = nullptr; p.pass_ntile = ne / 2;
        pass_geometry_table(p, tab.data());
        uint2* d_geom = nullptr;
        ok = ok && dalloc(h, &d_geom, (size_t)ne) && hipMemcpy(d_geom, tab.data(), (size_t)ne * sizeof(uint2), hipMemcpyHostToDevice) == hipSuccess;
        if (ok) p.pass_geom = d_geom;
    }
    auto carve = [&](ExtractCtx& c, char* base) -> size_t {
        size_t off = 0;
        auto take = [&](auto*& ptr, size_t count) {
            using T = typename std::remove_reference<decltype(*ptr)>::type;
            off = (off + 255) & ~(size_t)255;
            ptr = reinterpret_cast<T*>(base + off);
            off += std::max<size_t>(count, 1) * sizeof(T);
        };
        FrameMaps& m = c.maps;
        take(m.rgba, P); take(m.disp, P); take(m.label, P); take(m.inlier, P); take(m.plane_depth, P);
        take(m.sp, S); take(m.samples, NS); take(m.sample_score, NS); take(m.moments, 13 * S); take(m.filt, 11 * S); take(m.epoch, 64); take(m.pix2, P); take(m.fpack, 4 * S);
        for (int b = 0; b < 2; b++) take(m.sums[b].r, S);
        for (int b = 0; b < 3; b++) { take(m.log.ent[b], NT * 256); take(m.log.disp[b], NT * 256); take(m.log.count[b], NT); }
        SurfelSoA& f = c.frame;
        take(f.pos, 3 * S); take(f.col, 3 * S); take(f.lab, 3 * S); take(f.stamps, 2 * S); take(f.r0, 3 * S); take(f.r1, 3 * S);
        take(f.r2, 3 * S); take(f.shape, 6 * S); take(f.dims, 2 * S); take(f.conf, S);
        take(c.d_best, S); take(c.d_matched, S); take(c.d_rgb_in, 4 * P); take(c.d_depth_in, P); take(c.d_depth_filt, P); take(c.d_mask, S);
        take(c.d_wire, 26 * S);
        take(c.d_pixmask, P); take(c.d_pixcnt, 2 * S);
        return (off + 255) & ~(size_t)255;
    };
    size_t slab_bytes = 0;
    for (int ci = 0; ci < nctx && ok; ci++) {
        ExtractCtx& c = h->ctx[ci];
        slab_bytes = carve(c, nullptr);
        char* base = nullptr;
        ok = dalloc(h, &base, slab_bytes * h->batch);
        if (!ok) break;
        (void)carve(c, base);
        FrameMaps& m = c.maps;
        m.slab = slab_bytes;
        m.srgb_lut = h->d_srgb_lut;
        (void)hipMemsetAsync(base, 0, slab_bytes * h->batch, h->stream);
        if (nctx == 1) c.stream = h->stream;
        else {
            int least = 0, greatest = 0;
            (void)hipDeviceGetStreamPriorityRange(&least, &greatest);
            static const bool ctx0_up = SSF_ENV_INT("CTX0_PRIORITY", 1) != 0;
            const int prio = (ci == 0 && ctx0_up && least - greatest >= 2) ? least - 1 : least;
            c.stream = stream_pool().take(h->cfg.device_id, prio); ok = c.stream != nullptr; c.own_stream = ok; c.stream_prio = prio;
        }
        if (ok && h->pass_team) {
            const int kmax = 4 * std::max(cfg->seg_iter, 0);
            std::vector<char> tab(pass_args_bytes(std::max(kmax, 1)));
            pass_args_table(p, c.maps, kmax, tab.data());
            ok = dalloc(h, &c.d_pas, tab.size()) && dalloc(h, &c.d_team_ws, pass_team_ws_bytes()) &&
                 hipMemcpy(c.d_pas, tab.data(), tab.size(), hipMemcpyHostToDevice) == hipSuccess;
        }
        ok = ok && hipEventCreateWithFlags(&c.ev_done, hipEventDisableTiming) == hipSuccess &&
             hipEventCreateWithFlags(&c.ev_consumed, hipEventDisableTiming) == hipSuccess &&
             hipEventCreate(&c.ev_t0) == hipSuccess && hipEventCreate(&c.ev_t1) == hipSuccess;
    }
    const size_t OC = 3 * N + 4 * S + 1024;
    h->part_sup_vis = 6 * (int)(((N + 255) / 256 + 2) / PART_GROUP + 1);
    h->part_sup_oov = (int)(((OC + 255) / 256 + 8) / PART_GROUP + 1);
    h->part_words = h->part_sup_vis + h->part_sup_oov + 8 * PART_REPLICAS;
    ok = ok && dalloc(h, &h->d_part, 2 * (size_t)h->part_words) && dalloc(h, &h->d_part_ticket, 128);
    if (ok) {
        void* q = nullptr;
        int large_bar = 0;
        (void)hipDeviceGetAttribute(&large_bar, hipDeviceAttributeIsLargeBar, cfg->device_id);
        const size_t n_res = cfg->icp_iter > 0 && cfg->icp_iter < 4096 ? 2 * ((size_t)cfg->icp_iter + 1) : 0;
        if (large_bar && hipExtMallocWithFlags(&q, (SSF_ICP_GO_SLOTS + n_res) * sizeof(IcpGo), hipDeviceMallocFinegrained) == hipSuccess) {
            h->allocs.push_back(q); h->go = (IcpGo*)q;
            (void)hipMemset(q, 0, (SSF_ICP_GO_SLOTS + n_res) * sizeof(IcpGo));
            if (n_res) { h->go_res = h->go + SSF_ICP_GO_SLOTS; h->resident_max_rows = 256 * icp_resident_max_wgs(); }
        } else { (void)hipGetLastError(); h->go = nullptr; }
    }
    ok = ok && alloc_surfels(h, h->model[0], N) && alloc_surfels(h, h->model[1], N) && alloc_surfels(h, h->dense, N) &&
         alloc_surfels(h, h->oov[0].rows, OC) && alloc_surfels(h, h->oov[1].rows, OC) && dalloc(h, &h->oov[0].live, OC) &&
         dalloc(h, &h->oov[1].live, OC) && dalloc(h, &h->d_state_oov, OC) && dalloc(h, &h->d_bc_oov, (OC + 255) / 256 + 8) &&
         dalloc(h, &h->d_live_scratch, N) && dalloc(h, &h->d_bf_in, P) && dalloc(h, &h->d_bf_out, P) &&
         dalloc(h, &h->d_icp, 64) && dalloc(h, &h->d_state, N + 16) && dalloc(h, &h->d_cand, N) &&
         dalloc(h, &h->d_cnt, 2) && dalloc(h, &h->d_migrants, (size_t)SSF_MIGRANT_WORDS * S) && dalloc(h, &h->d_scratch_map, P) && dalloc(h, &h->d_icp_replicas, 2 * SSF_ICP_REPLICAS * 32)     ;
#ifdef SSF_EXPERIMENTS
    h->bins.min_rows = SSF_ENV_INT("BIN_MIN_ROWS", SSF_BIN_MIN_ROWS_DEFAULT);
#endif
    if (ok) {
        ok = hipHostMalloc((void**)&h->mb_host, sizeof(Mailbox), hipHostMallocCoherent) == hipSuccess ||
             hipHostMalloc((void**)&h->mb_host, sizeof(Mailbox), hipHostMallocDefault) == hipSuccess;
        if (ok) { std::memset(h->mb_host, 0, sizeof(Mailbox)); ok = hipHostGetDevicePointer((void**)&h->mb_dev, h->mb_host, 0) == hipSuccess; }
    }
    for (int i = 0; i < 4 && ok; i++) ok = hipEventCreate(&h->ev[i]) == hipSuccess;
    if (!ok) { g_create_err = std::string("device allocation failed: ") + hipGetErrorString(hipGetLastError()); ssf_destroy(h); return SSF_ERR_DEVICE; }
    {
        float lut[256];
        for (int c8 = 0; c8 < 256; c8++) lut[c8] = srgb_expand((float)c8 / 255.0f);
        (void)hipMemcpy(h->d_srgb_lut, lut, sizeof(lut), hipMemcpyHostToDevice);
    }
    (void)hipMemsetAsync(h->d_icp_replicas, 0, 2 * SSF_ICP_REPLICAS * 32 * sizeof(long long), h->stream);
    (void)hipMemsetAsync(h->d_tickets, 0, 512 * sizeof(unsigned int), h->stream);
    (void)hipMemsetAsync(h->d_part, 0, 2 * (size_t)h->part_words * sizeof(uint32_t), h->stream);
    (void)hipMemsetAsync(h->d_part_ticket, 0, 128 * sizeof(uint32_t), h->stream);
    (void)hipMemsetAsync(h->d_cand, 0xFF, N * sizeof(int32_t), h->stream);
    h->oov[0].cap = h->oov[1].cap = (int)OC;
    h->oov_head = h->oov_tail = oov_home(h); h->oov_live = 0;
    {
        Counters c0; std::memset(&c0, 0, sizeof(c0)); c0.oov_head = c0.oov_tail = h->oov_head;
        (void)hipMemcpy(h->d_cnt, &c0, sizeof(c0), hipMemcpyHostToDevice);
    }
// ... 615 lines not shown
```

### supersurfel_fusion_amd/csrc/ssf_track_fuse.hip

```cpp
#include <stdlib.h>
#include <algorithm>
#include "ssf_slots.hpp"

namespace ssf {

__device__ __forceinline__ long long wsum64(long long v) {
#pragma unroll
    for (int o = 32; o > 0; o >>= 1) v += __shfl_xor(v, o, 64);
    return v;
}
__device__ __forceinline__ V3 ld3(const float* __restrict__ p, size_t i) { return v3(p[3 * i], p[3 * i + 1], p[3 * i + 2]); }
__device__ __forceinline__ void st3(float* __restrict__ p, size_t i, V3 v) { p[3 * i] = v.x; p[3 * i + 1] = v.y; p[3 * i + 2] = v.z; }
__device__ __forceinline__ Sym3 ld6(const float* __restrict__ p, size_t i) {
    return sym3(p[6 * i], p[6 * i + 1], p[6 * i + 2], p[6 * i + 3], p[6 * i + 4], p[6 * i + 5]);
}
__device__ __forceinline__ void st6(float* __restrict__ p, size_t i, Sym3 c) {
    p[6 * i] = c.xx; p[6 * i + 1] = c.xy; p[6 * i + 2] = c.xz; p[6 * i + 3] = c.yy; p[6 * i + 4] = c.yz; p[6 * i + 5] = c.zz;
}

#ifndef ICP_SLOTS
#define ICP_SLOTS 16
#endif
template <bool UNIFORM, typename Emit>
__device__ __forceinline__ void icp_row_terms_(const Cam& cam, const uint2* __restrict__ pix2, const float4* __restrict__ fpack,
// ... 227 lines not shown
            const bool need = mine[j] && (unsigned int)(acc[j] & CNT_MASK) != expect[j];
            got[j] = need ? __hip_atomic_exchange(&counted[wr[j] * 32 + wk[j]], 0ull, __ATOMIC_RELAXED, __HIP_MEMORY_SCOPE_AGENT) : 0ull;
        }
#pragma unroll
        for (int j = 0; j < WPT; j++) {
            acc[j] += got[j];
            done = done && (!mine[j] || (unsigned int)(acc[j] & CNT_MASK) == expect[j]);
        }
        if (__syncthreads_and(done ? 1 : 0)) break;
        if (tid == 0 && (round & 15u) == 15u && wall_clock64() - t0 > SSF_ICP_COLLECT_WAIT_TICKS) s_expired = 1;
        __syncthreads();
        if (s_expired) return false;
        __builtin_amdgcn_s_sleep(1);
    }
#pragma unroll
    for (int j = 0; j < WPT; j++)
        if (mine[j]) part[wr[j] * 32 + wk[j]] = (long long)(acc[j] - (acc[j] & CNT_MASK)) >> ICP_CNT_BITS;
    __syncthreads();
    if (tid < 64) {
        __shared__ unsigned long long pay[30];
        long long tot = 0;
        if (tid < ICP_CNT_WORDS)
            for (int q = 0; q < SSF_ICP_REPLICAS; q++) tot += part[q * 32 + tid];
        const long long hi27 = (long long)shfl_u64((unsigned long long)tot, 29);
        if (tid == 27) tot = (long long)(((unsigned long long)hi27 << 40) + (unsigned long long)tot);
        if (tid >= 29) tot = 0;
        if (tid < 29) {
            sums[tid] = tot;
            pay[tid] = (unsigned long long)tot;
        }
        const unsigned long long check = (unsigned long long)wsum64(tot) + seq;
        if (tid == 0) pay[29] = check;
        __builtin_amdgcn_s_waitcnt(0xc07f);
        if (tid < 40)
            __hip_atomic_store(&mb->icp_rec[tid], SSF_ICP_REC_WORD(tid, pay, seq), __ATOMIC_RELAXED, __HIP_MEMORY_SCOPE_SYSTEM);
    }
    return true;
}
__device__ __forceinline__ unsigned int xcd_block(unsigned int b, unsigned int nb) {
    const unsigned int q = nb >> 3, r = nb & 7u, x = b & 7u;
    return (x < r ? x * (q + 1u) : r * (q + 1u) + (x - r) * q) + (b >> 3);
}
__device__ __forceinline__ int match_bid_wave(int f, unsigned long long key, unsigned long long* __restrict__ best) {
    unsigned long long todo = __ballot(1);
    const unsigned int klo = (unsigned int)key, khi = (unsigned int)(key >> 32);
    while (todo) {
        const int leader = __ffsll((long long)todo) - 1;
        const int f0 = __builtin_amdgcn_readlane(f, leader);
        const unsigned long long same = __ballot(f == f0) & todo;
        unsigned long long m = ~0ull, rest = same;
        while (rest) {
            const int o = __ffsll((long long)rest) - 1;
            const unsigned long long ko = ((unsigned long long)(unsigned int)__builtin_amdgcn_readlane((int)khi, o) << 32) |
                                          (unsigned long long)(unsigned int)__builtin_amdgcn_readlane((int)klo, o);
            m = ko < m ? ko : m;
            rest &= rest - 1ull;
        }
        if (lane() == leader) atomicMin(&best[f0], m);
        todo &= ~same;
    }
    return f;
}
#ifdef SSF_EXPERIMENTS
#include "lab/icp_arms.inc"
#endif
__device__ __forceinline__ int match_row(const Cam& cam, const SurfelSoA& model, int j, int id, const uint2* __restrict__ pix2,
                                         const float4* __restrict__ fpack, const Rt& pose, float zmin, float zmax,
                                         long long id_offset, unsigned long long* __restrict__ best, uint8_t* __restrict__ matched,
                                         bool wave_agg = false);
__device__ __forceinline__ int match_values(const Cam& cam, float m_conf, const V3& mp, const V3& m_r2, const V3& m_lab, int id,
                                            const uint2* __restrict__ pix2, const float4* __restrict__ fpack, const Rt& pose, float zmin,
                                            float zmax, long long id_offset, unsigned long long* __restrict__ best,
                                            uint8_t* __restrict__ matched, bool wave_agg);
__device__ __forceinline__ void match_sorted_rows(const Cam& cam, const SurfelSoA& sorted, int n_visible, const uint2* __restrict__ pix2,
                                                  const float4* __restrict__ fpack, const Rt& pose, const MatchArgs& ma) {
    for (int j = (int)(xcd_block(blockIdx.x, gridDim.x) * blockDim.x + threadIdx.x); j < n_visible; j += gridDim.x * blockDim.x) {
        const float4* __restrict__ rec = reinterpret_cast<const float4*>(sorted.pos) + 3 * (size_t)j;
        float4 a = rec[0], b = rec[1], c = rec[2];
        asm volatile("" : "+v"(a.x), "+v"(b.x), "+v"(c.x));
        const int oid = __float_as_int(b.w);
        ma.cand[oid] = match_values(cam, a.w, v3(a.x, a.y, a.z), v3(c.x, c.y, c.z), v3(b.x, b.y, b.z), oid, pix2, fpack, pose, ma.zmin, ma.zmax, ma.id_offset, ma.best, ma.matched, true);
    }
}
#define SSF_ICP_DBG_COUNTED 0x40000000
#ifndef SSF_ICP_GO_WAIT_TICKS
#define SSF_ICP_GO_WAIT_TICKS 25000000ull
#endif
#ifndef SSF_ICP_NUM_SGPR
#define SSF_ICP_NUM_SGPR 80
#endif
__device__ __forceinline__ int icp_wait_word(IcpGo* go, unsigned int want, unsigned int& w) {
    int ok = 0, told = 0;
    const unsigned int l = threadIdx.x;
    const unsigned int* gw = reinterpret_cast<const unsigned int*>(go);
    const unsigned int weight = icp_go_word_weight(l);
    w = 0u;
    const unsigned long long t0 = wall_clock64();
    for (unsigned int spin = 0; spin < (1u << 24); spin++) {
        w = l < 16u ? __hip_atomic_load(&gw[l], __ATOMIC_RELAXED, __HIP_MEMORY_SCOPE_SYSTEM) : 0u;
        const unsigned int flo = (unsigned int)__builtin_amdgcn_readlane((int)w, 12), fhi = (unsigned int)__builtin_amdgcn_readlane((int)w, 13);
        if (flo == want) {
            if (fhi & 0x80000000u) {
                if ((fhi & SSF_ICP_GO_CHECK_MASK) == icp_go_abort_check(want)) { told = 1; break; }
            } else {
                unsigned int sum = w * weight;
#pragma unroll
                for (int o = 1; o < 16; o <<= 1) sum += __shfl_xor(sum, o, 64);
                sum = (unsigned int)__builtin_amdgcn_readfirstlane((int)sum);
                if (((sum >> 2) & SSF_ICP_GO_CHECK_MASK) == (fhi & SSF_ICP_GO_CHECK_MASK)) {
                    ok = (fhi & 0x40000000u) ? 2 : 1; told = 1;
                    break;
                }
            }
        }
        if ((spin & 63u) == 63u && wall_clock64() - t0 > SSF_ICP_GO_WAIT_TICKS) break;
        __builtin_amdgcn_s_sleep(1);
    }
    if (!told && l == 0u) __hip_atomic_store(&go->flag, (unsigned long long)want | ((unsigned long long)icp_go_abort_check(want) << 32) | SSF_ICP_GO_ABORT, __ATOMIC_RELAXED, __HIP_MEMORY_SCOPE_SYSTEM);
    return ok;
}
template <bool P2P, int MODE>
__global__ __launch_bounds__(256) __attribute__((amdgpu_num_sgpr(SSF_ICP_NUM_SGPR))) void k_icp(Cam cam, SurfelSoA model, int n_visible,
                                             const uint2* __restrict__ pix2, const float4* __restrict__ fpack,
                                             Rt T, long long* __restrict__ replicas, unsigned int* ticket,
                                             long long* __restrict__ sums, Mailbox* mb, unsigned long long seq, int dbg,
                                             IcpGo* go, unsigned long long go_seq, P2PView pv, int by_tile, MatchArgs ma) {
    __builtin_amdgcn_s_setprio(3);
    unsigned int n_wg = gridDim.x;
    constexpr unsigned int WG = 256;
    asm volatile("" : "+s"(dbg), "+s"(by_tile), "+s"(n_visible), "+s"(n_wg));
    __shared__ unsigned long long red[29 * ICP_SLOTS];
    __shared__ float s_T[12];
    __shared__ int s_go;
    __shared__ unsigned long long s_p2p_seq;
    for (int i = threadIdx.x; i < 29 * ICP_SLOTS; i += WG) red[i] = 0ull;
    if (go) {
        if (threadIdx.x < 64) {
            const unsigned int l = threadIdx.x;
            unsigned int w;
            const int ok = icp_wait_word(go, (unsigned int)go_seq, w);
            if (ok) {
                if (l < 12u) s_T[l] = __uint_as_float(w);
                const unsigned int xlo = (unsigned int)__builtin_amdgcn_readlane((int)w, 14), xhi = (unsigned int)__builtin_amdgcn_readlane((int)w, 15);
                if (P2P && l == 0u) s_p2p_seq = ((unsigned long long)xhi << 32) | xlo;
            }
            if (l == 0u) s_go = ok;
        }
        __syncthreads();
        if (!s_go) return;
        T.R = m3(v3(s_T[0], s_T[1], s_T[2]), v3(s_T[3], s_T[4], s_T[5]), v3(s_T[6], s_T[7], s_T[8]));
        T.t = v3(s_T[9], s_T[10], s_T[11]);
        if constexpr (!P2P && (MODE == 0 || MODE == 3)) {
            if (s_go == 2) {
                auto sT = [&](int i) { return __uint_as_float(__builtin_amdgcn_readfirstlane(__float_as_uint(s_T[i]))); };
                T.R = m3(v3(sT(0), sT(1), sT(2)), v3(sT(3), sT(4), sT(5)), v3(sT(6), sT(7), sT(8)));
                T.t = v3(sT(9), sT(10), sT(11));
                if constexpr (MODE == 3) { if (ma.best) match_sorted_rows(cam, model, n_visible, pix2, fpack, T, ma); return; }
                if (ma.best && !by_tile)
                    for (int id = blockIdx.x * WG + threadIdx.x; id < n_visible; id += n_wg * WG)
                        ma.cand[id] = match_row(cam, model, id, id, pix2, fpack, T, ma.zmin, ma.zmax, ma.id_offset, ma.best, ma.matched);
                return;
            }
        }
    }
    const unsigned long long p2p_seq = (P2P && go) ? s_p2p_seq : pv.seq;
    __syncthreads();
    const M3 R = T.R; const V3 t = T.t;
    const int slot = lane() & (ICP_SLOTS - 1);
    unsigned int blk = blockIdx.x; (void)by_tile;
    if constexpr (MODE == 3) {
        blk = xcd_block(blockIdx.x, n_wg);
        const float4* __restrict__ rec = reinterpret_cast<const float4*>(model.pos);
        for (int id = blk * WG + threadIdx.x; id < n_visible; id += n_wg * WG) {
            float4 a = rec[3 * id], b = rec[3 * id + 1], c = rec[3 * id + 2];
            asm volatile("" : "+v"(a.x), "+v"(b.x), "+v"(c.x));
            icp_row(cam, pix2, fpack, R, t, v3(a.x, a.y, a.z), v3(b.x, b.y, b.z), v3(c.x, c.y, c.z), red, slot, 0);
        }
    } else
#ifdef SSF_EXPERIMENTS
    if (MODE != 0) icp_lab_arm<MODE>(cam, model, n_visible, pix2, fpack, R, t, red, slot, blk);
    else
#endif
        for (int id = blk * WG + threadIdx.x; id < n_visible; id += n_wg * WG) {
            V3 mpos = ld3(model.pos, id), mlab = ld3(model.lab, id), mnrm = ld3(model.r2, id);
            asm volatile("" : "+v"(mpos.x), "+v"(mlab.x), "+v"(mnrm.x));
            icp_row(cam, pix2, fpack, R, t, mpos, mlab, mnrm, red, slot, dbg);
        }
    __syncthreads();
    __shared__ int s_last;
    if (SSF_PROBE(dbg, 4)) {
        icp_fold(red, replicas);
        return;
    }
    if constexpr (!P2P) {
        if (dbg & SSF_ICP_DBG_COUNTED) {
            unsigned long long* counted = reinterpret_cast<unsigned long long*>(replicas) + SSF_ICP_REPLICAS * 32;
            icp_fold_counted(red, counted);
            if (blockIdx.x == n_wg - 1) icp_collect_counted(counted, sums, mb, seq, n_wg, threadIdx.x);
            return;
        }
    }
    icp_fold(red, replicas);
    if (threadIdx.x == 0) s_last = grid_arrive(ticket);
    __syncthreads();
    if (s_last) icp_publish<P2P>(replicas, sums, mb, seq, pv, p2p_seq);
}

__global__ __launch_bounds__(256, 7) __attribute__((amdgpu_num_sgpr(SSF_ICP_NUM_SGPR))) void k_icp_resident(Cam cam, SurfelSoA model, int n_visible,
                                             const uint2* __restrict__ pix2, const float4* __restrict__ fpack,
                                             Rt T, unsigned long long* __restrict__ counted, long long* __restrict__ sums, Mailbox* mb,
                                             unsigned long long seq, IcpGo* go, unsigned int go_base, int have_first, int last_idx,
                                             MatchArgs ma) {
    __builtin_amdgcn_s_setprio(3);
    unsigned int n_wg = gridDim.x;
    asm volatile("" : "+s"(n_visible), "+s"(n_wg), "+s"(last_idx), "+s"(go_base));
    __shared__ unsigned long long red[29 * ICP_SLOTS];
    __shared__ float s_T[12];
    __shared__ int s_go;
    __shared__ unsigned long long s_seq;
    const int id = (int)(blockIdx.x * 256u + threadIdx.x);
    const bool live = id < n_visible;
    float m_conf = 0.0f;
    V3 mpos = v3(0, 0, 0), mlab = v3(0, 0, 0), mnrm = v3(0, 0, 0);
    if (live) { m_conf = model.conf[id]; mpos = ld3(model.pos, id); mlab = ld3(model.lab, id); mnrm = ld3(model.r2, id); }
    asm volatile("" : "+v"(m_conf), "+v"(mpos.x), "+v"(mlab.x), "+v"(mnrm.x));
    const int slot = lane() & (ICP_SLOTS - 1);
    if (threadIdx.x == 0) {
        const float t12[12] = {T.R.r0.x, T.R.r0.y, T.R.r0.z, T.R.r1.x, T.R.r1.y, T.R.r1.z, T.R.r2.x, T.R.r2.y, T.R.r2.z, T.t.x, T.t.y, T.t.z};
#pragma unroll
        for (int i = 0; i < 12; i++) s_T[i] = t12[i];
        s_seq = seq; s_go = 1;
    }
    for (int idx = have_first ? 0 : 1; idx <= last_idx; idx++) {
        asm volatile("" : "+v"(m_conf), "+v"(mpos.x), "+v"(mpos.y), "+v"(mpos.z), "+v"(mlab.x), "+v"(mlab.y), "+v"(mlab.z), "+v"(mnrm.x), "+v"(mnrm.y), "+v"(mnrm.z));
        asm volatile("" : "+s"(cam.fx), "+s"(cam.fy), "+s"(cam.cx), "+s"(cam.cy), "+s"(cam.W), "+s"(cam.H));
        for (int i = threadIdx.x; i < 29 * ICP_SLOTS; i += 256) red[i] = 0ull;
        if (idx > 0 && threadIdx.x < 64) {
            const unsigned int l = threadIdx.x;
            unsigned int w;
            const int ok = icp_wait_word(go + idx, go_base + (unsigned int)idx, w);
            if (ok) {
                if (l < 12u) s_T[l] = __uint_as_float(w);
                const unsigned int xlo = (unsigned int)__builtin_amdgcn_readlane((int)w, 14), xhi = (unsigned int)__builtin_amdgcn_readlane((int)w, 15);
                if (l == 0u) s_seq = ((unsigned long long)xhi << 32) | xlo;
            }
            if (l == 0u) s_go = ok;
        }
        __syncthreads();
        if (!s_go) return;
        if (s_go == 2) {
            auto sT = [&](int i) { return __uint_as_float(__builtin_amdgcn_readfirstlane(__float_as_uint(s_T[i]))); };
            Rt P; P.R = m3(v3(sT(0), sT(1), sT(2)), v3(sT(3), sT(4), sT(5)), v3(sT(6), sT(7), sT(8)));
            P.t = v3(sT(9), sT(10), sT(11));
            if (ma.best && live) ma.cand[id] = match_values(cam, m_conf, mpos, mnrm, mlab, id, pix2, fpack, P, ma.zmin, ma.zmax, ma.id_offset, ma.best, ma.matched, false);
            return;
        }
        T.R = m3(v3(s_T[0], s_T[1], s_T[2]), v3(s_T[3], s_T[4], s_T[5]), v3(s_T[6], s_T[7], s_T[8]));
        T.t = v3(s_T[9], s_T[10], s_T[11]);
        seq = s_seq;
        if (live) icp_row(cam, pix2, fpack, T.R, T.t, mpos, mlab, mnrm, red, slot, 0);
        __syncthreads();
        icp_fold_counted(red, counted);
        unsigned int tid = threadIdx.x;
        asm volatile("" : "+v"(tid));
        if (blockIdx.x == n_wg - 1 && !icp_collect_counted(counted, sums, mb, seq, n_wg, tid)) {
            const unsigned int want = go_base + (unsigned int)idx + 1u;
            if (threadIdx.x == 0 && idx < last_idx)
                __hip_atomic_store(&go[idx + 1].flag, (unsigned long long)want | ((unsigned long long)icp_go_abort_check(want) << 32) | SSF_ICP_GO_ABORT, __ATOMIC_RELAXED, __HIP_MEMORY_SCOPE_SYSTEM);
            return;
        }
        __syncthreads();
    }
}

__device__ __forceinline__ bool align_pair(const Cam& cam, const float* __restrict__ spos, const float* __restrict__ slab,
                                           const float* __restrict__ snrm, const float* __restrict__ sconf, int id,
                                           const SurfelSoA& frame, const int32_t* __restrict__ label,
                                           const float* __restrict__ plane_depth, const M3& R, const V3& t,
                                           V3& pv, V3& sn, V3& tp, V3& tn) {
    if (sconf && !(sconf[id] > 0.0f)) return false;
    pv = add(m3_mulv(R, ld3(spos, id)), t);
    const int u = pixel_round(pv.x * cam.fx / pv.z + cam.cx), v = pixel_round(pv.y * cam.fy / pv.z + cam.cy);
    if (!(u >= 0 && u < cam.W && v >= 0 && v < cam.H)) return false;
    const size_t q = (size_t)v * cam.W + u;
    const int tid = label[q];
    if (!(frame.conf[tid] > 0.0f)) return false;
    const float dist_color = len3(sub(ld3(slab, id), ld3(frame.lab, tid)));
    const float td = plane_depth[q];
    if (!isfinite(td)) return false;
    sn = unit3(ld3(snrm, id));
    sn = unit3(m3_mulv(R, sn));
    tn = unit3(ld3(frame.r2, tid));
    tp = v3(td * ((float)u - cam.cx) / cam.fx, td * ((float)v - cam.cy) / cam.fy, td);
    return dist_color < 20.0f && len3(sub(pv, tp)) < 0.1f && fabsf(dot3(sn, tn)) > 0.8f;
}
__global__ __launch_bounds__(1024) void k_align(Cam cam, const float* __restrict__ spos, const float* __restrict__ slab,
                                                const float* __restrict__ snrm, const float* __restrict__ sconf, int n,
                                                SurfelSoA frame, const int32_t* __restrict__ label,
                                                const float* __restrict__ plane_depth, Rt T, long long* __restrict__ out) {
    __shared__ unsigned long long acc[8];
    __shared__ unsigned long long red[29 * 16];
    __shared__ float s_c[7];
    __shared__ int s_pairs;
    for (int i = threadIdx.x; i < 29 * 16; i += blockDim.x) red[i] = 0ull;
    if (threadIdx.x < 8) acc[threadIdx.x] = 0ull;
    __syncthreads();
    const M3 R = T.R; const V3 t = T.t;
    V3 pv, sn, tp, tn;
    for (int id = threadIdx.x; id < n; id += blockDim.x) {
        if (!align_pair(cam, spos, slab, snrm, sconf, id, frame, label, plane_depth, R, t, pv, sn, tp, tn)) continue;
        atomicAdd(&acc[0], (unsigned long long)fx64((double)pv.x, SSF_ALIGN_SCALE_POS, SSF_ALIGN_LIM));
        atomicAdd(&acc[1], (unsigned long long)fx64((double)pv.y, SSF_ALIGN_SCALE_POS, SSF_ALIGN_LIM));
        atomicAdd(&acc[2], (unsigned long long)fx64((double)pv.z, SSF_ALIGN_SCALE_POS, SSF_ALIGN_LIM));
        atomicAdd(&acc[3], (unsigned long long)fx64((double)tp.x, SSF_ALIGN_SCALE_POS, SSF_ALIGN_LIM));
        atomicAdd(&acc[4], (unsigned long long)fx64((double)tp.y, SSF_ALIGN_SCALE_POS, SSF_ALIGN_LIM));
        atomicAdd(&acc[5], (unsigned long long)fx64((double)tp.z, SSF_ALIGN_SCALE_POS, SSF_ALIGN_LIM));
        atomicAdd(&acc[6], 1ull);
    }
    __syncthreads();
    if (threadIdx.x == 0) {
        const int pairs = (int)acc[6];
        s_pairs = pairs;
        for (int i = 0; i < 6; i++) s_c[i] = (float)((double)(long long)acc[i] / SSF_ALIGN_SCALE_POS) / (float)pairs;
        out[29] = pairs;
    }
    __syncthreads();
    const int pairs = s_pairs;
    if (pairs < 100) {
        if (threadIdx.x < 29) out[threadIdx.x] = 0;
        if (threadIdx.x >= 30 && threadIdx.x < 37) out[threadIdx.x] = 0;
        return;
    }
    const V3 cs = v3(s_c[0], s_c[1], s_c[2]), ct = v3(s_c[3], s_c[4], s_c[5]);
    for (int id = threadIdx.x; id < n; id += blockDim.x) {
        if (!align_pair(cam, spos, slab, snrm, sconf, id, frame, label, plane_depth, R, t, pv, sn, tp, tn)) continue;
        const V3 a = v3(tp.x - ct.x, tp.y - ct.y, tp.z - ct.z), b = v3(pv.x - cs.x, pv.y - cs.y, pv.z - cs.z);
        atomicAdd(&acc[7], (unsigned long long)fx64((double)((a.x * a.x + a.y * a.y) + a.z * a.z), SSF_ALIGN_SCALE_D2, SSF_ALIGN_LIM));
// ... 20 lines not shown
#pragma unroll
        for (int i = 0; i < 6; i++)
#pragma unroll
            for (int j = i; j < 6; j++, k++)
                atomicAdd(&red[k * 16 + slot], (unsigned long long)(long long)fx32(x1[i] * x1[j] + x2[i] * x2[j], 1048576.0f));
#pragma unroll
        for (int i = 0; i < 6; i++)
            atomicAdd(&red[(21 + i) * 16 + slot], (unsigned long long)(long long)fx32(dn1 * x1[i] + dn2 * x2[i], 16777216.0f));
        atomicAdd(&red[27 * 16 + slot], (unsigned long long)fx64((double)(dn2 * dn2), 17592186044416.0, 4611686018427387904.0));
        atomicAdd(&red[28 * 16 + slot], 1ull);
    }
    __syncthreads();
    if (threadIdx.x < 29) {
        unsigned long long tot = 0;
        for (int sidx = 0; sidx < 16; sidx++) tot += red[threadIdx.x * 16 + sidx];
        out[threadIdx.x] = (long long)tot;
    }
    if (threadIdx.x < 7) out[30 + threadIdx.x] = (long long)__float_as_uint(s_c[threadIdx.x]);
}

__global__ void k_fern_codes(const uint8_t* __restrict__ rgb, const float* __restrict__ depth, int W, int H,
                             const uint32_t* __restrict__ fpos, const uint8_t* __restrict__ frgb,
                             const float* __restrict__ fdepth, int n, uint8_t* __restrict__ codes) {
    const int k = blockIdx.x * blockDim.x + threadIdx.x;
    if (k >= n) return;
    const int x = (int)min(fpos[2 * k], (uint32_t)W - 1u), y = (int)min(fpos[2 * k + 1], (uint32_t)H - 1u);
    const size_t q = (size_t)y * W + x;
    uint8_t r = 0;
    r |= rgb[3 * q] > frgb[3 * k] ? 1 : 0;
    r |= rgb[3 * q + 1] > frgb[3 * k + 1] ? 2 : 0;
    r |= rgb[3 * q + 2] > frgb[3 * k + 2] ? 4 : 0;
    r |= depth[q] > fdepth[k] ? 8 : 0;
    codes[k] = r;
}

__device__ __forceinline__ int match_row(const Cam& cam, const SurfelSoA& model, int j, int id, const uint2* __restrict__ pix2,
                                         const float4* __restrict__ fpack, const Rt& pose, float zmin, float zmax,
                                         long long id_offset, unsigned long long* __restrict__ best, uint8_t* __restrict__ matched,
                                         bool wave_agg) {
    float m_conf = model.conf[j];
    V3 mp = ld3(model.pos, j), m_r2 = ld3(model.r2, j), m_lab = ld3(model.lab, j);
    asm volatile("" : "+v"(m_conf), "+v"(mp.x), "+v"(m_r2.x), "+v"(m_lab.x));
    return match_values(cam, m_conf, mp, m_r2, m_lab, id, pix2, fpack, pose, zmin, zmax, id_offset, best, matched, wave_agg);
}
__device__ __forceinline__ int match_values(const Cam& cam, float m_conf, const V3& mp, const V3& m_r2, const V3& m_lab, int id,
                                            const uint2* __restrict__ pix2, const float4* __restrict__ fpack, const Rt& pose, float zmin,
                                            float zmax, long long id_offset, unsigned long long* __restrict__ best,
                                            uint8_t* __restrict__ matched, bool wave_agg) {
    (void)wave_agg;
    if (!(m_conf > 0.0f)) return -1;
    const M3 R = pose.R; const V3 t = pose.t;
    const M3 Rt_ = m3_transpose(R);
    const V3 tview = negate(m3_mulv(Rt_, t));
    const V3 pv = add(m3_mulv(Rt_, mp), tview);
    if (!(pv.z > zmin && pv.z < zmax)) return -1;
    const int px = pixel_round(pv.x * cam.fx / pv.z + cam.cx), py = pixel_round(pv.y * cam.fy / pv.z + cam.cy);
    if (!(px >= 0 && px < cam.W && py >= 0 && py < cam.H)) return -1;
    const int f = (int)pix2[(size_t)py * cam.W + px].x;
    matched[f] = 1;
    float4 f0 = fpack[4 * f], f1 = fpack[4 * f + 1], f2 = fpack[4 * f + 2];
    asm volatile("" : "+v"(f0.y), "+v"(f1.x), "+v"(f2.x));
    if (!(f0.x > 0.0f)) return -1;
    const V3 fp = add(m3_mulv(R, v3(f2.x, f2.y, f2.z)), t);
    const V3 fn = unit3(row_mul(v3(f1.x, f1.y, f1.z), Rt_));
    const V3 mn = unit3(m_r2);
    const float dist = len3(sub(mp, fp));
    const float lab_dist = len3(sub(m_lab, v3(f0.y, f0.z, f0.w)));
    const float delta_norm = fabsf(dot3(mn, fn));
    if (!(lab_dist < 15.0f && delta_norm > 0.8f && dist < 0.05f)) return -1;
    const unsigned long long key = ((unsigned long long)__float_as_uint(dist) << 32) |
                                   (unsigned long long)(uint32_t)(id_offset + id);
    if (wave_agg) return match_bid_wave(f, key, best);
    atomicMin(&best[f], key);
    return f;
}
template <bool SORTED>
__global__ __launch_bounds__(256) void k_match(Cam cam, SurfelSoA model, int n_visible, const uint2* __restrict__ pix2,
                                               const float4* __restrict__ fpack, Rt pose, float zmin, float zmax,
                                               long long id_offset, unsigned long long* __restrict__ best,
                                               uint8_t* __restrict__ matched, int32_t* __restrict__ cand, const int32_t* __restrict__ orig) {
    __builtin_amdgcn_s_setprio(3);
    if constexpr (SORTED) {
        (void)orig;
        const MatchArgs ma{zmin, zmax, id_offset, best, matched, cand};
        match_sorted_rows(cam, model, n_visible, pix2, fpack, pose, ma);
        return;
    } else {
        const int j = blockIdx.x * blockDim.x + threadIdx.x, id = j; (void)orig;
        if (j >= n_visible) return;
        cand[id] = match_row(cam, model, j, id, pix2, fpack, pose, zmin, zmax, id_offset, best, matched, false);
    }
}

#include "ssf_tile_rows.inc"

struct ClsPre { int st; int pix; float pz; };
__device__ __forceinline__ ClsPre classify_pre(const Cam& cam, float conf, int last_seen, const V3& pos, const Rt& pose, int stamp,
                                               int delta_t, float conf_thresh, float zmin, float zmax) {
    ClsPre r; r.pix = 0; r.pz = 0.0f;
    const int time_diff = stamp - last_seen;
    if ((time_diff > delta_t && conf < conf_thresh && stamp > delta_t) || conf <= 0.0f) { r.st = 2; return r; }
    const M3 Rv = m3_transpose(pose.R);
    const V3 tv = negate(m3_mulv(Rv, pose.t));
    const V3 p = add(m3_mulv(Rv, pos), tv);
    r.st = 1;
    if (p.z > zmin && p.z < zmax) {
        const float u = cam.fx * p.x / p.z + cam.cx, v = cam.fy * p.y / p.z + cam.cy;
        if (u >= 0.0f && u < (float)cam.W && v >= 0.0f && v < (float)cam.H) {
            r.st = -1; r.pix = ((int)floorf(v)) * cam.W + (int)floorf(u); r.pz = p.z;
        }
    }
    return r;
}
__device__ __forceinline__ int classify_post(const ClsPre& r, float z) { return r.st >= 0 ? r.st : (r.pz < 0.8f * z ? 2 : 0); }
__device__ __forceinline__ int classify_values(const Cam& cam, float conf, int last_seen, const V3& pos, const Rt& pose,
                                               const float* __restrict__ plane_depth, int stamp, int delta_t, float conf_thresh,
                                               float zmin, float zmax) {
    const ClsPre r = classify_pre(cam, conf, last_seen, pos, pose, stamp, delta_t, conf_thresh, zmin, zmax);
    return r.st >= 0 ? r.st : classify_post(r, plane_depth[r.pix]);
}
__device__ __forceinline__ int classify_row(const Cam& cam, const SurfelSoA& M, size_t idx, const Rt& pose,
                                            const float* __restrict__ plane_depth, int stamp, int delta_t, float conf_thresh,
                                            float zmin, float zmax) {
    const int st = classify_values(cam, M.conf[idx], M.stamps[2 * idx + 1], ld3(M.pos, idx), pose, plane_depth, stamp, delta_t,
                                   conf_thresh, zmin, zmax);
    if (st == 2) M.conf[idx] = -1.0f;
    return st;
}
#ifndef OOV_PER_WG
#define OOV_PER_WG 4
#endif
__device__ __forceinline__ void classify_oov_block(const Cam& cam, const OovStore& O, const Rt& pose, const float* __restrict__ plane_depth,
                                                   int stamp, int delta_t, float conf_thresh, float zmin, float zmax,
                                                   uint8_t* __restrict__ state_oov, uint32_t* __restrict__ bc_oov, PartitionWs ws,
                                                   const Counters* __restrict__ cnt, int wg, int nb_oov) {
    __shared__ int h2[OOV_PER_WG][4][2];
    const int wv = threadIdx.x >> 6;
    const long long head = cnt->oov_head, tail = cnt->oov_tail;
    int cls[OOV_PER_WG];
    uint8_t lv[OOV_PER_WG]; float conf[OOV_PER_WG]; int seen[OOV_PER_WG]; V3 pos[OOV_PER_WG]; ClsPre pre[OOV_PER_WG]; float z[OOV_PER_WG];
    bool in[OOV_PER_WG];
#pragma unroll
    for (int j = 0; j < OOV_PER_WG; j++) {
        const long long phys = head + ((long long)wg * OOV_PER_WG + j) * 256  + threadIdx.x;
        in[j] = phys < tail;
        const size_t q = (size_t)(in[j] ? phys : tail - 1);
        lv[j] = O.live[q]; conf[j] = O.rows.conf[q]; seen[j] = O.rows.stamps[2 * q + 1]; pos[j] = ld3(O.rows.pos, q);
    }
#pragma unroll
    for (int j = 0; j < OOV_PER_WG; j++) {
        int lvj = lv[j];
        asm volatile("" : "+v"(lvj), "+v"(conf[j]), "+v"(seen[j]), "+v"(pos[j].x), "+v"(pos[j].y), "+v"(pos[j].z));
        lv[j] = in[j] ? (uint8_t)lvj : (uint8_t)0;
    }
#pragma unroll
    for (int j = 0; j < OOV_PER_WG; j++) {
        pre[j] = classify_pre(cam, conf[j], seen[j], pos[j], pose, stamp, delta_t, conf_thresh, zmin, zmax);
        if (!lv[j]) { pre[j].st = 7; pre[j].pix = 0; }
        if (pre[j].st >= 0) pre[j].pix = 0;
    }
#pragma unroll
    for (int j = 0; j < OOV_PER_WG; j++) z[j] = plane_depth[pre[j].pix];
#pragma unroll
    for (int j = 0; j < OOV_PER_WG; j++) asm volatile("" : "+v"(z[j]));
#pragma unroll
    for (int j = 0; j < OOV_PER_WG; j++) {
        cls[j] = classify_post(pre[j], z[j]);
        if (lv[j]) {
            const long long phys = head + ((long long)wg * OOV_PER_WG + j) * 256  + threadIdx.x;
            if (cls[j] == 2) O.rows.conf[phys] = -1.0f;
            state_oov[phys] = (uint8_t)cls[j];
        }
    }
#pragma unroll
    for (int j = 0; j < OOV_PER_WG; j++) {
        const int k0 = __popcll(__ballot(cls[j] == 0)), k2 = __popcll(__ballot(cls[j] == 2));
        if (lane() == 0) { h2[j][wv][0] = k0; h2[j][wv][1] = k2; }
    }
    __syncthreads();
    if (threadIdx.x < 2 * OOV_PER_WG) {
        const int j = threadIdx.x >> 1, which = threadIdx.x & 1, ob = wg * OOV_PER_WG + j;
        const uint32_t k = h2[j][0][which] + h2[j][1][which] + h2[j][2][which] + h2[j][3][which];
        if (ob < nb_oov) {
            const uint32_t other = __shfl_xor(k, 1, 64);
            if (which == 0) bc_oov[ob] = k | (other << 16);
            if (k) {
                atomic_add_done(&ws.tot[(ob & (PART_REPLICAS - 1)) * 8 + 6 + which], k);
                if (which == 0) atomicAdd(&ws.sup_oov[ob / PART_GROUP], k);
            }
        }
    }
}
#define UPD_PER_WG 32
__device__ __forceinline__ int tile_owner(const V3& pw, int nranks, float tile);
__device__ __forceinline__ float pick3(const V3& v, int k) { return k == 0 ? v.x : (k == 1 ? v.y : v.z); }
__device__ __forceinline__ void update_group(SurfelSoA M, SurfelSoA F, Rt pose, int stamp, long long id_offset, int n_visible,
                                             const unsigned long long* __restrict__ best, const uint8_t* __restrict__ matched,
                                             int S, Counters* cnt, int f0, const ClassifyArgs& ca, uint8_t* __restrict__ state_vis,
                                             PartitionWs ws, const ShardArgs& sh) {
    const int wv = threadIdx.x >> 6, l = lane();
    if (wv == 3) return;
    const int f = wv == 0 ? f0 + (l >> 1) : f0 + (wv - 1) * 16 + (l >> 2);
    if (f >= S) return;
    unsigned int mt = matched[f];
    unsigned long long bk = best[f];
    float f_conf = F.conf[f];
    V3 f_pos = v3(0.f, 0.f, 0.f), f_lab = v3(0.f, 0.f, 0.f);
    Sym3 f_shape = sym3(0.f, 0.f, 0.f, 0.f, 0.f, 0.f);
    if (wv == 0) { f_pos = ld3(F.pos, f); f_shape = ld6(F.shape, f); } else f_lab = ld3(F.lab, f);
    asm volatile("" : "+v"(mt), "+v"(bk), "+v"(f_conf), "+v"(f_pos.x), "+v"(f_shape.xx), "+v"(f_lab.x));
    if (!mt || bk == SSF_NO_MATCH) return;
    const long long local = (long long)(uint32_t)(bk & 0xFFFFFFFFull) - id_offset;
    if (local < 0 || local >= n_visible) return;
    const size_t m = (size_t)local;
    float m_conf = M.conf[m];
    V3 model_position = v3(0.f, 0.f, 0.f), model_lab = v3(0.f, 0.f, 0.f);
    Sym3 model_shape = sym3(0.f, 0.f, 0.f, 0.f, 0.f, 0.f);
    if (wv == 0) { model_position = ld3(M.pos, m); model_shape = ld6(M.shape, m); } else model_lab = ld3(M.lab, m);
    asm volatile("" : "+v"(m_conf), "+v"(model_position.x), "+v"(model_shape.xx), "+v"(model_lab.x));
    const float ratio = 1.0f / (m_conf + f_conf);
    if (wv == 0) {
        const int which = l & 1;
        const M3 R = pose.R; const V3 t = pose.t;
        const V3 frame_position = add(m3_mulv(R, f_pos), t);
        const Sym3 frame_shape = rot_sym(R, f_shape);
        Sym3 f1, m1, fused_shape, fused_1;
        V3 fused_position;
        const float w = ratio * f_conf;
        bool info = false;
        if (sym_inverse(frame_shape, f1) && sym_inverse(model_shape, m1)) {
            fused_1 = sym_add(sym_scale(w, f1), sym_scale(1.0f - w, m1));
            if (sym_inverse(fused_1, fused_shape)) {
                fused_position = sym_mul(fused_shape, add(sym_mul(sym_scale(w, f1), frame_position),
                                                          sym_mul(sym_scale(1.0f - w, m1), model_position)));
                info = true;
            }
        }
        if (!info) {
            fused_shape = sym_scale(ratio, sym_add(sym_scale(f_conf, frame_shape), sym_scale(m_conf, model_shape)));
            fused_position = scale(ratio, add(scale(f_conf, frame_position), scale(m_conf, model_position)));
        }
        const V3 axis = principal_power(principal_start(fused_shape, which == 1));
        const int l0 = l & ~1;
        const V3 r0 = v3(__shfl(axis.x, l0, 64), __shfl(axis.y, l0, 64), __shfl(axis.z, l0, 64));
        const V3 r2 = v3(__shfl(axis.x, l0 + 1, 64), __shfl(axis.y, l0 + 1, 64), __shfl(axis.z, l0 + 1, 64));
        if (which == 0) {
            M3 vecs; V3 vals;
            principal_finish(fused_shape, r0, r2, vecs, vals);
            int st = classify_values(ca.cam, m_conf + f_conf, stamp, fused_position, pose, ca.plane_depth, stamp, ca.delta_t,
                                     ca.conf_thresh, ca.zmin, ca.zmax);
            const bool removed = st == 2;
            if (sh.migrate && !removed && tile_owner(fused_position, sh.nranks, sh.tile) != sh.rank) {
                st = 2;
                atomic_add_done(&cnt->n_emigrated, 1);
            }
            st3(M.pos, m, fused_position);
            M.conf[m] = removed ? -1.0f : m_conf + f_conf;
            st6(M.shape, m, fused_shape);
            st3(M.r0, m, vecs.r0); st3(M.r1, m, vecs.r1); st3(M.r2, m, vecs.r2);
            M.dims[2 * m] = vals.x; M.dims[2 * m + 1] = vals.y;
            M.stamps[2 * m + 1] = stamp;
            state_vis[m] = (uint8_t)st;
            atomic_add_done(&cnt->n_updated, 1);
            const int vb = (int)(m >> 8);
            atomicAdd(&ws.sup_vis[(vb / PART_GROUP) * 6 + st], 1u);
            atomic_add_done(&ws.tot[(vb & (PART_REPLICAS - 1)) * 8 + st], 1u);
        }
    } else {
        const int ch = min(l & 3, 2), l0 = l & ~3;
        const V3 frame_lab = f_lab;
        const V3 lin = lab_to_linear_rgb(scale(ratio, add(scale(f_conf, frame_lab), scale(m_conf, model_lab))));
        const float c255 = srgb_to_255(pick3(lin, ch));
        const V3 fused_color = v3(__shfl(c255, l0, 64), __shfl(c255, l0 + 1, 64), __shfl(c255, l0 + 2, 64));
        const float e = srgb_expand(c255 / 255.0f);
        const V3 q = xyz_from_linear(__shfl(e, l0, 64), __shfl(e, l0 + 1, 64), __shfl(e, l0 + 2, 64));
        const float fq = lab_f(pick3(q, ch));
        const V3 lab = lab_from_f(__shfl(fq, l0, 64), __shfl(fq, l0 + 1, 64), __shfl(fq, l0 + 2, 64));
        if ((l & 3) == 0) { st3(M.col, m, fused_color); st3(M.lab, m, lab); }
    }
}

__device__ __forceinline__ int tile_owner(const V3& pw, int nranks, float tile) {
    const int ix = (int)floorf(pw.x / tile), iy = (int)floorf(pw.y / tile), iz = (int)floorf(pw.z / tile);
    const uint32_t h = ((uint32_t)ix * 73856093u) ^ ((uint32_t)iy * 19349663u) ^ ((uint32_t)iz * 83492791u);
    return (int)(h % (uint32_t)nranks);
}
__device__ __forceinline__ int shard_owner(const SurfelSoA& F, int f, const Rt& pose, int nranks, float tile) {
    if (nranks <= 1) return 0;
// ... 41 lines not shown
    const int r = block_rank_1024(flag, wave_tot, total);
    const int k = base + before + r;
    const int g_first = ((base + before) >> 8) / PART_GROUP;
    if (flag && base_total + before + r < capacity) {
        const V3 f_pos = ld3(F.pos, f), f_col = ld3(F.col, f), f_lab = ld3(F.lab, f);
        const V3 f_r0 = ld3(F.r0, f), f_r1 = ld3(F.r1, f), f_r2 = ld3(F.r2, f);
        const Sym3 f_shape = ld6(F.shape, f);
        const float f_d0 = F.dims[2 * f], f_d1 = F.dims[2 * f + 1];
        const float new_conf = F.conf[f];
        const V3 new_pos = add(m3_mulv(R, f_pos), t);
        const int st = classify_values(ca.cam, new_conf, stamp, new_pos, pose, ca.plane_depth, stamp, ca.delta_t, ca.conf_thresh,
                                       ca.zmin, ca.zmax);
        st3(M.pos, k, new_pos);
        M.conf[k] = st == 2 ? -1.0f : new_conf;
        st3(M.col, k, f_col);
        st3(M.lab, k, f_lab);
        M.stamps[2 * k] = stamp; M.stamps[2 * k + 1] = stamp;
        M.dims[2 * k] = f_d0; M.dims[2 * k + 1] = f_d1;
        st3(M.r0, k, row_mul(f_r0, Rt_));
        st3(M.r1, k, row_mul(f_r1, Rt_));
        st3(M.r2, k, row_mul(f_r2, Rt_));
        st6(M.shape, k, rot_sym(R, f_shape));
        state_vis[k] = (uint8_t)st;
        atomicAdd(&s_cls[(k >> 8) / PART_GROUP - g_first][st], 1u);
    }
    __syncthreads();
    if (threadIdx.x < 6) {
        const int seg = threadIdx.x / 3, st = threadIdx.x % 3;
        const uint32_t n = s_cls[seg][st];
        if (n) {
            atomicAdd(&ws.sup_vis[(g_first + seg) * 6 + 3 + st], n);
            atomic_add_done(&ws.tot[(chunk & (PART_REPLICAS - 1)) * 8 + 3 + st], n);
        }
    }
    if (chunk == nchunks - 1 && threadIdx.x == 0)
        atomic_store_done(&cnt->n_inserted, min(base_total + before + total, capacity) - base_total);
}
__device__ __forceinline__ Counters finalise_counters(Counters* cnt, Counters c, int shrink_by_removed, int keep_inserted = 0);
__device__ __forceinline__ void mailbox_counters(const Counters& c, Mailbox* mb, unsigned long long seq);
__device__ __forceinline__ Counters frame_counters(const Counters& c_in, const uint32_t* tot) {
    const int a0 = (int)tot[0], a1 = (int)tot[1], a2 = (int)tot[2], c0 = (int)tot[3], c1 = (int)tot[4], c2 = (int)tot[5];
    const int b0 = (int)tot[6], b2 = (int)tot[7], b1 = c_in.oov_live - b0 - b2;
    Counters c = c_in;
    c.n_model = c_in.n_model + c_in.n_inserted;
    c.n_state0 = a0 + b0 + c0; c.n_state1 = a1 + b1 + c1; c.n_state2 = a2 + b2 + c2;
    c.n_visible = a0 + b0 + c0; c.n_removed = (a2 + b2 + c2) - c_in.n_emigrated;
    c.mv_nv = c_in.n_visible; c.mv_a0 = a0; c.mv_b0 = b0; c.mv_nc = c_in.n_inserted;
    c.mv_head_old = c_in.oov_head; c.mv_tail_old = c_in.oov_tail; c.mv_head_new = c_in.oov_head - a1;
    c.oov_head = c_in.oov_head - a1; c.oov_tail = c_in.oov_tail + c1;
    c.oov_live = (c_in.oov_live - b0 - b2) + a1 + c1;
    return c;
}
#ifdef SSF_EXPERIMENTS
__device__ unsigned long long* g_fuse_trace = nullptr;
void set_fuse_trace(unsigned long long* p) { (void)hipMemcpyToSymbol(HIP_SYMBOL(g_fuse_trace), &p, sizeof(p)); }
#endif
__global__ __launch_bounds__(256) void k_update_insert(SurfelSoA M, SurfelSoA F, Rt pose, int stamp, long long id_offset,
                                                       int n_visible, const unsigned long long* __restrict__ best,
                                                       const uint8_t* __restrict__ matched, const int32_t* __restrict__ cand, int S,
                                                       int do_update, int capacity, int rank, int nranks, float tile, Counters* cnt,
                                                       int nupd, int nchunks, int nb_vis, int nb_oov, OovStore O, ClassifyArgs ca,
                                                       uint8_t* __restrict__ state_vis, uint8_t* __restrict__ state_oov,
                                                       uint32_t* __restrict__ bc_oov, PartitionWs ws, int migrate, int tail_in_move) {
    __builtin_amdgcn_s_setprio(3);
    __shared__ int wave_tot[16];
    __shared__ int hist[4][6];
    __shared__ int s_last;
    __shared__ uint32_t tot[8];
    const int b = blockIdx.x;
#ifdef SSF_EXPERIMENTS
    unsigned long long* const trace = g_fuse_trace;
    if (trace && threadIdx.x == 0) trace[3 * (size_t)b] = wall_clock64();
#endif
    if (b >= nupd + nchunks + nb_vis)
        classify_oov_block(ca.cam, O, pose, ca.plane_depth, stamp, ca.delta_t, ca.conf_thresh, ca.zmin, ca.zmax, state_oov, bc_oov,
                           ws, cnt, b - nupd - nchunks - nb_vis, nb_oov);
    else if (b >= nupd + nchunks) {
        const int vb = b - nupd - nchunks, i = vb * blockDim.x + threadIdx.x, wv = threadIdx.x >> 6;
        int cls = 7;
        if (i < n_visible) {
            int f = cand[i];
            float conf = M.conf[i]; int seen = M.stamps[2 * (size_t)i + 1]; V3 pos = ld3(M.pos, (size_t)i);
            asm volatile("" : "+v"(f), "+v"(conf), "+v"(seen), "+v"(pos.x));
            const bool rewritten = do_update && f >= 0 && (uint32_t)(best[f] & 0xFFFFFFFFull) == (uint32_t)(id_offset + i);
            if (!rewritten) {
                cls = classify_values(ca.cam, conf, seen, pos, pose, ca.plane_depth, stamp, ca.delta_t, ca.conf_thresh, ca.zmin, ca.zmax);
                if (cls == 2) M.conf[i] = -1.0f;
                state_vis[i] = (uint8_t)cls;
            }
        }
#pragma unroll
        for (int c = 0; c < 3; c++) { const int k = __popcll(__ballot(cls == c)); if (lane() == 0) hist[wv][c] = k; }
        __syncthreads();
        if (threadIdx.x < 3) {
            const uint32_t k = hist[0][threadIdx.x] + hist[1][threadIdx.x] + hist[2][threadIdx.x] + hist[3][threadIdx.x];
            if (k) {
                atomicAdd(&ws.sup_vis[(vb / PART_GROUP) * 6 + threadIdx.x], k);
                atomic_add_done(&ws.tot[(vb & (PART_REPLICAS - 1)) * 8 + threadIdx.x], k);
            }
        }
    } else if (b >= nupd)
        insert_chunk(M, F, pose, stamp, matched, S, capacity, rank, nranks, tile, cnt, wave_tot, b - nupd, nchunks, ca, state_vis, ws);
    else if (do_update) {
        ShardArgs sh; sh.rank = rank; sh.nranks = nranks; sh.migrate = (migrate && nranks > 1) ? 1 : 0; sh.tile = tile;
        update_group(M, F, pose, stamp, id_offset, n_visible, best, matched, S, cnt, b * UPD_PER_WG, ca, state_vis, ws, sh);
    }
#ifdef SSF_EXPERIMENTS
    if (trace) {
        __syncthreads();
        if (threadIdx.x == 0) trace[3 * (size_t)b + 1] = wall_clock64();
        asm volatile("s_waitcnt vmcnt(0) lgkmcnt(0)" ::: "memory");
        __syncthreads();
        if (threadIdx.x == 0) trace[3 * (size_t)b + 2] = wall_clock64();
    }
#endif
    if (tail_in_move) return;
    asm volatile("s_waitcnt vmcnt(0)" ::: "memory");
    __syncthreads();
    if (threadIdx.x == 0) s_last = grid_arrive(ws.ticket);
    __syncthreads();
    if (!s_last) return;
    if (threadIdx.x < 8) {
        uint32_t v = 0;
#pragma unroll
        for (int r = 0; r < PART_REPLICAS; r++) v += __hip_atomic_load(&ws.tot[r * 8 + threadIdx.x], __ATOMIC_RELAXED, __HIP_MEMORY_SCOPE_AGENT);
        tot[threadIdx.x] = v;
    }
    __syncthreads();
    if (threadIdx.x >= 64) {
        for (int i = threadIdx.x - 64; i < ws.words; i += blockDim.x - 64) ws.other[i] = 0u;
    } else if (threadIdx.x == 0) {
        Counters c_in = *cnt;
        c_in.n_inserted = __hip_atomic_load(&cnt->n_inserted, __ATOMIC_RELAXED, __HIP_MEMORY_SCOPE_AGENT);
        c_in.n_updated = __hip_atomic_load(&cnt->n_updated, __ATOMIC_RELAXED, __HIP_MEMORY_SCOPE_AGENT);
        c_in.n_emigrated = __hip_atomic_load(&cnt->n_emigrated, __ATOMIC_RELAXED, __HIP_MEMORY_SCOPE_AGENT);
        cnt[1] = finalise_counters(cnt, frame_counters(c_in, tot), 1);
    }
}

__global__ __launch_bounds__(1024) void k_first_frame(SurfelSoA M, SurfelSoA F, Rt pose, int S, int capacity, int rank,
                                                      int nranks, float tile, Counters* cnt) {
    __shared__ int wave_tot[16];
    int running = 0;
    for (int c0 = 0; c0 < S; c0 += 1024) {
        const int f = c0 + threadIdx.x;
        const bool flag = (f < S) && shard_owner(F, f, pose, nranks, tile) == rank;
        int total;
        const int r = block_rank_1024(flag, wave_tot, total);
        const int k = running + r;
        if (flag && k < capacity) {
            st3(M.pos, k, ld3(F.pos, f)); st3(M.col, k, ld3(F.col, f)); st3(M.lab, k, ld3(F.lab, f));
            M.stamps[2 * k] = F.stamps[2 * f]; M.stamps[2 * k + 1] = F.stamps[2 * f + 1];
            st3(M.r0, k, ld3(F.r0, f)); st3(M.r1, k, ld3(F.r1, f)); st3(M.r2, k, ld3(F.r2, f));
            st6(M.shape, k, ld6(F.shape, f));
            M.dims[2 * k] = F.dims[2 * f]; M.dims[2 * k + 1] = F.dims[2 * f + 1];
            M.conf[k] = F.conf[f];
        }
        running += total;
    }
    if (threadIdx.x == 0) {
        const int n = min(running, capacity);
        cnt->n_model = n; cnt->n_visible = n; cnt->n_inserted = 0; cnt->n_removed = 0;
    }
}

struct RowRegs { V3 pos, col, lab, r0, r1, r2; Sym3 shape; int s0, s1; float d0, d1, conf; };
__device__ __forceinline__ RowRegs load_row(const SurfelSoA& A, size_t i) {
// ... 140 lines not shown
                store_row(O.rows, j, row);
                O.live[j] = 1;
            }
        }
    } else {
        const int ob = blockIdx.x - nb_vis;
        const long long phys = (long long)mv_head_old + (long long)ob * blockDim.x + threadIdx.x;
        if (phys < mv_tail_old) {
            int lv = (int)O.live[phys], st = (int)state_oov[phys];
            asm volatile("" : "+v"(lv), "+v"(st));
            if (lv) cls = st;
        }
        const unsigned long long mask = __ballot(cls == 0);
        if (cls == 0) in_wave = __popcll(mask & ((1ull << lane()) - 1ull));
        if (lane() == 0) hist[wv][0] = __popcll(mask);
        if (__syncthreads_count(cls == 0)) {
            const int g0 = ob / PART_GROUP, nw = g0 + (ob - g0 * PART_GROUP);
            for (int w = threadIdx.x; w < nw; w += blockDim.x) {
                const uint32_t v = w < g0 ? ws.sup_oov[w] : (bc_oov[g0 * PART_GROUP + (w - g0)] & 0xFFFFu);
                if (v) atomicAdd(&base[0], v);
            }
            __syncthreads();
        }
        if (cls == 0) {
            int before = 0;
            for (int w = 0; w < wv; w++) before += hist[w][0];
            const size_t j = (size_t)mv_a0() + base[0] + before + in_wave;
            if (ICP) { copy_row_keep(O.rows, (size_t)phys, Vn, j, pos, lab, nrm); keep = true; }
            else copy_row(O.rows, (size_t)phys, Vn, j);
        }
        if (cls == 0 || cls == 2) O.live[phys] = 0;
    }
    if (ICP) {
        if (keep) icp_row(nx.cam, nx.pix2, nx.fpack, nx.T.R, nx.T.t, pos, lab, nrm, red, lane() & (ICP_SLOTS - 1), 0);
        const int nkeep = __syncthreads_count(keep);
        if (P2P && new_n_visible() == 0) {
            if (blockIdx.x == 0) icp_publish<true>(nx.replicas, nx.sums, nx.mb, nx.seq, pv, pv.seq);
            return;
        }
        const bool vis = (int)blockIdx.x < nb_vis;
        const int nbr = (mv_nv + mv_nc + 255) / 256;
        if (vis ? (int)blockIdx.x >= nbr : nkeep == 0) return;
        __shared__ int s_last;
        icp_fold(red, nx.replicas);
        if (threadIdx.x == 0) {
            SSF_ARRIVE_RELEASE();
            unsigned int rows = (unsigned int)nkeep;
            bool report = true;
            if (vis) {
                const unsigned int g = blockIdx.x & 63u, in_group = ((unsigned int)nbr - g + 63u) / 64u;
                unsigned long long* gw = reinterpret_cast<unsigned long long*>(nx.ticket + 128) + g;
                const unsigned long long before = __hip_atomic_fetch_add(gw, ((unsigned long long)rows << 32) | 1ull, __ATOMIC_RELAXED,
                                                                         __HIP_MEMORY_SCOPE_AGENT);
                report = (unsigned int)(before & 0xFFFFFFFFull) == in_group - 1;
                if (report) {
                    rows += (unsigned int)(before >> 32);
                    __hip_atomic_store(gw, 0ull, __ATOMIC_RELAXED, __HIP_MEMORY_SCOPE_AGENT);
                }
            }
            int last = 0;
            if (report) {
                const unsigned int total = (unsigned int)new_n_visible();
                const unsigned int before = rows ? __hip_atomic_fetch_add(&nx.ticket[65], rows, __ATOMIC_RELAXED, __HIP_MEMORY_SCOPE_AGENT) : 0u;
                last = rows != 0u && before + rows == total;
                if (last) __hip_atomic_store(&nx.ticket[65], 0u, __ATOMIC_RELAXED, __HIP_MEMORY_SCOPE_AGENT);
            }
            if (last) SSF_ARRIVE_ACQUIRE();
            s_last = last;
        }
        __syncthreads();
        if (s_last) icp_publish<P2P>(nx.replicas, nx.sums, nx.mb, nx.seq, pv, pv.seq);
    }
}

__global__ __launch_bounds__(256) void k_pack_emigrants(SurfelSoA M, const unsigned long long* __restrict__ best,
                                                        const uint8_t* __restrict__ matched, long long id_offset, int n_visible,
                                                        const uint8_t* __restrict__ state_vis, int S, int do_update, int nranks,
                                                        float tile, int32_t* __restrict__ table) {
    const int f = blockIdx.x * blockDim.x + threadIdx.x;
    if (f >= S) return;
    int32_t w[SSF_MIGRANT_WORDS];
#pragma unroll
    for (int i = 0; i < SSF_MIGRANT_WORDS; i++) w[i] = 0;
    if (do_update && matched[f] && best[f] != SSF_NO_MATCH) {
        const long long local = (long long)(uint32_t)(best[f] & 0xFFFFFFFFull) - id_offset;
        if (local >= 0 && local < n_visible) {
            const size_t m = (size_t)local;
            const float conf = M.conf[m];
            if (state_vis[m] == 2 && conf > 0.0f) {
                const RowRegs r = load_row(M, m);
                w[0] = tile_owner(r.pos, nranks, tile) + 1;
                const float v[26] = {r.pos.x, r.pos.y, r.pos.z, r.col.x, r.col.y, r.col.z, __int_as_float(r.s0), __int_as_float(r.s1),
                                     r.r0.x, r.r0.y, r.r0.z, r.r1.x, r.r1.y, r.r1.z, r.r2.x, r.r2.y, r.r2.z,
                                     r.shape.xx, r.shape.xy, r.shape.xz, r.shape.yy, r.shape.yz, r.shape.zz, r.d0, r.d1, r.conf};
#pragma unroll
                for (int i = 0; i < 26; i++) w[2 + i] = __float_as_int(v[i]);
            }
        }
    }
    int32_t* o = table + (size_t)SSF_MIGRANT_WORDS * f;
#pragma unroll
    for (int i = 0; i < SSF_MIGRANT_WORDS; i++) o[i] = w[i];
}
__global__ __launch_bounds__(1024) void k_migrate_in(SurfelSoA M, const int32_t* __restrict__ table, int S, int rank, int capacity,
                                                     Counters* cnt, ClassifyArgs ca, Rt pose, int stamp,
                                                     uint8_t* __restrict__ state_vis, PartitionWs ws) {
    __shared__ int wave_tot[16];
    __shared__ int s_in[4];
    if (threadIdx.x < 4) s_in[threadIdx.x] = 0;
    const Counters c1 = cnt[1];
    const int base_row = c1.mv_nv + c1.mv_nc;
    const int total_before = c1.n_model + c1.n_state2;
    int running = 0;
    __syncthreads();
    for (int f0 = 0; f0 < S; f0 += 1024) {
        const int f = f0 + threadIdx.x;
        const bool flag = f < S && table[(size_t)SSF_MIGRANT_WORDS * f] - 1 == rank;
        int total;
        const int r = block_rank_1024(flag, wave_tot, total);
        if (flag && total_before + running + r < capacity) {
            const int32_t* w = table + (size_t)SSF_MIGRANT_WORDS * f;
            float v[26];
#pragma unroll
            for (int i = 0; i < 26; i++) v[i] = __int_as_float(w[2 + i]);
            RowRegs row;
            row.pos = v3(v[0], v[1], v[2]); row.col = v3(v[3], v[4], v[5]); row.lab = rgb_to_lab(row.col);
            row.s0 = __float_as_int(v[6]); row.s1 = __float_as_int(v[7]);
            row.r0 = v3(v[8], v[9], v[10]); row.r1 = v3(v[11], v[12], v[13]); row.r2 = v3(v[14], v[15], v[16]);
            row.shape = sym3(v[17], v[18], v[19], v[20], v[21], v[22]); row.d0 = v[23]; row.d1 = v[24]; row.conf = v[25];
            const int st = classify_values(ca.cam, row.conf, row.s1, row.pos, pose, ca.plane_depth, stamp, ca.delta_t, ca.conf_thresh,
                                           ca.zmin, ca.zmax);
            if (st == 2) row.conf = -1.0f;
            const size_t k = (size_t)base_row + running + r;
            store_row(M, k, row);
            state_vis[k] = (uint8_t)st;
            atomicAdd(&ws.sup_vis[((k >> 8) / PART_GROUP) * 6 + 3 + st], 1u);
            atomicAdd(&s_in[st], 1);
        } else if (flag)
            atomicAdd(&s_in[3], 1);
        running += min(total, max(0, capacity - total_before - running));
        __syncthreads();
    }
    __syncthreads();
    if (threadIdx.x == 0) {
        const int in0 = s_in[0], in1 = s_in[1], in2 = s_in[2], n_in = in0 + in1 + in2, lost = s_in[3];
        if (n_in || lost) {
            for (int q = 0; q < 2; q++) {
                Counters c = cnt[q];
                c.n_model += in0 + in1; c.n_visible += in0;
                c.oov_tail += in1; c.oov_live += in1; c.mv_nc += n_in;
                if (q == 1) { c.n_state0 += in0; c.n_state1 += in1; c.n_state2 += in2; c.n_removed += in2 + lost; }
                c.last[0] = c.n_model; c.last[1] = c.n_visible; if (q == 1) c.last[2] = c.n_removed; else c.last[2] += in2 + lost;
                cnt[q] = c;
            }
        }
    }
}

__device__ __forceinline__ int rehome_class(const SurfelSoA& D, int i, int n, int rank, int nranks, float tile) {
    if (i >= n) return 2;
    return (D.conf[i] > 0.0f && tile_owner(ld3(D.pos, i), nranks, tile) != rank) ? 1 : 0;
}
__global__ __launch_bounds__(256) void k_rehome_count(SurfelSoA D, int n, int n_visible, int rank, int nranks, float tile, uint32_t* __restrict__ bc) {
    __shared__ int part[4][3];
    const int i = blockIdx.x * blockDim.x + threadIdx.x;
    const int c = rehome_class(D, i, n, rank, nranks, tile);
    const int k0 = __popcll(__ballot(c == 0)), k1 = __popcll(__ballot(c == 1)), k2 = __popcll(__ballot(c == 0 && i < n_visible));
    if (lane() == 0) { part[threadIdx.x >> 6][0] = k0; part[threadIdx.x >> 6][1] = k1; part[threadIdx.x >> 6][2] = k2; }
// ... 285 lines not shown
    for (int i = threadIdx.x; i < S; i += blockDim.x) {
        unsigned long long b = __hip_atomic_load(&best[i], __ATOMIC_RELAXED, __HIP_MEMORY_SCOPE_AGENT);
        uint8_t m = __hip_atomic_load(&matched[i], __ATOMIC_RELAXED, __HIP_MEMORY_SCOPE_AGENT);
        for (int r = 0; r < pv.nranks; r++) {
            if (r == pv.me) continue;
            const unsigned long long* sb = reinterpret_cast<const unsigned long long*>(mine + p2p_off_best(S, par, r));
            const uint8_t* sm = mine + p2p_off_matched(S, par, r);
            const unsigned long long ob = __hip_atomic_load(&sb[i], __ATOMIC_RELAXED, __HIP_MEMORY_SCOPE_SYSTEM);
            const uint8_t om = __hip_atomic_load(&sm[i], __ATOMIC_RELAXED, __HIP_MEMORY_SCOPE_SYSTEM);
            b = ob < b ? ob : b; m = om > m ? om : m;
        }
        best[i] = b; matched[i] = m;
    }
}
__global__ __launch_bounds__(1024) void k_p2p_assoc(P2PView pv, unsigned long long* __restrict__ best, uint8_t* __restrict__ matched, Mailbox* mb) {
    __shared__ int s_ok;
    p2p_assoc_exchange(pv, best, matched, &s_ok, mb);
}
__global__ __launch_bounds__(256) void k_p2p_migr_share(P2PView pv, const int32_t* __restrict__ table, unsigned int* ticket) {
    const int par = (int)(pv.seq & 1ull), S = pv.S;
    const int f = blockIdx.x * blockDim.x + threadIdx.x;
    if (f < S) {
        const unsigned long long* src = reinterpret_cast<const unsigned long long*>(table + (size_t)SSF_MIGRANT_WORDS * f);
        unsigned long long w[SSF_MIGRANT_WORDS / 2];
        w[0] = src[0];
        const bool full = (unsigned int)w[0] != 0u;
#pragma unroll
        for (int k = 1; k < SSF_MIGRANT_WORDS / 2; k++) w[k] = full ? src[k] : 0ull;
#pragma unroll
        for (int r = 0; r < SSF_P2P_MAX_RANKS; r++) {
            if (r >= pv.nranks || r == pv.me) continue;
            unsigned long long* dst = reinterpret_cast<unsigned long long*>(pv.peer[r] + p2p_off_migr(S, par, pv.me)) + (size_t)(SSF_MIGRANT_WORDS / 2) * f;
            unsigned long long sink = __hip_atomic_exchange(&dst[0], w[0], __ATOMIC_RELAXED, __HIP_MEMORY_SCOPE_SYSTEM);
            if (full) {
#pragma unroll
                for (int k = 1; k < SSF_MIGRANT_WORDS / 2; k++) sink ^= __hip_atomic_exchange(&dst[k], w[k], __ATOMIC_RELAXED, __HIP_MEMORY_SCOPE_SYSTEM);
            }
            asm volatile("" :: "v"(sink));
        }
    }
    asm volatile("s_waitcnt vmcnt(0)" ::: "memory");
    __syncthreads();
    __shared__ int s_last;
    if (threadIdx.x == 0) s_last = grid_arrive(ticket);
    __syncthreads();
    if (s_last) p2p_raise_flags(pv, P2P_FLAG_MIGR);
}
__global__ __launch_bounds__(256) void k_p2p_migr_gather(P2PView pv, int32_t* __restrict__ table, Mailbox* mb) {
    const int par = (int)(pv.seq & 1ull), S = pv.S;
    __shared__ int s_ok;
    if (threadIdx.x == 0) {
        s_ok = p2p_wait_flags(pv, P2P_FLAG_MIGR) ? 1 : 0;
        if (!s_ok) __hip_atomic_store(&mb->p2p_timeout, 1u, __ATOMIC_RELAXED, __HIP_MEMORY_SCOPE_SYSTEM);
    }
    __syncthreads();
    if (!s_ok) return;
    const int f = blockIdx.x * blockDim.x + threadIdx.x;
    if (f >= S) return;
    unsigned char* mine = p2p_peer(pv, pv.me);
    int32_t* own = table + (size_t)SSF_MIGRANT_WORDS * f;
    for (int r = 0; r < pv.nranks; r++) {
        if (r == pv.me) continue;
        const unsigned long long* src = reinterpret_cast<const unsigned long long*>(mine + p2p_off_migr(S, par, r)) + (size_t)(SSF_MIGRANT_WORDS / 2) * f;
        const unsigned long long w0 = __hip_atomic_load(&src[0], __ATOMIC_RELAXED, __HIP_MEMORY_SCOPE_SYSTEM);
        if ((unsigned int)w0 == 0u) continue;
        own[0] += (int32_t)(unsigned int)w0; own[1] += (int32_t)(unsigned int)(w0 >> 32);
#pragma unroll
        for (int k = 1; k < SSF_MIGRANT_WORDS / 2; k++) {
            const unsigned long long w = __hip_atomic_load(&src[k], __ATOMIC_RELAXED, __HIP_MEMORY_SCOPE_SYSTEM);
            own[2 * k] += (int32_t)(unsigned int)w; own[2 * k + 1] += (int32_t)(unsigned int)(w >> 32);
        }
    }
}

int icp_variant_mode() {
    static const int mode = SSF_ENV_INT("ICP_WRED", 0) ? 2 : (SSF_ENV_INT("ICP_PER_LANE", 0) > 1 ? 1 : 0);
    return mode;
}
void launch_icp(hipStream_t st, const Cam& cam, SurfelSoA model, int n_visible, const uint2* pix2, const float4* fpack,
                Rt T, long long* replicas, unsigned int* ticket,
                long long* sums29, Mailbox* mb, unsigned long long seq, int dbg_arg, IcpGo* go, unsigned long long go_seq,
                const P2PView* pv, int by_tile, const MatchArgs* match) {
    ScopedKernel sk("icp_accumulate", st);
    const MatchArgs ma = match ? *match : MatchArgs{0.f, 0.f, 0, nullptr, nullptr, nullptr};
    const int mode = dbg_arg > 0 && dbg_arg != 4 ? 0 : icp_variant_mode();
    const int per_lane = mode == 1 ? std::max(2, SSF_ENV_INT("ICP_PER_LANE", 0)) : 1;
    const int per_block = 256 * per_lane;
    int grid = (n_visible + per_block - 1) / per_block;
    if (grid < 1) grid = 1;
    if (grid > 4096) grid = 4096;
    static const int counted = SSF_ENV_INT("ICP_COUNTED", 1);
    const int dbg = (dbg_arg < 0 ? 0 : dbg_arg) | ((counted && !pv && dbg_arg < 0) ? SSF_ICP_DBG_COUNTED : 0);
    const P2PView none{};
    const P2PView& v = pv ? *pv : none;
    if (by_tile && !pv) { hipLaunchKernelGGL((k_icp<false, 3>), dim3(grid), dim3(256), 0, st, cam, model, n_visible, pix2, fpack, T, replicas, ticket, sums29, mb, seq, dbg, go, go_seq, v, by_tile, ma); return; }
#ifdef SSF_EXPERIMENTS
    if (mode == 2 && !pv) { hipLaunchKernelGGL((k_icp<false, 2>), dim3(grid), dim3(256), 0, st, cam, model, n_visible, pix2, fpack, T, replicas, ticket, sums29, mb, seq, dbg, go, go_seq, v, by_tile, ma); return; }
    if (mode == 1 && pv) { hipLaunchKernelGGL((k_icp<true, 1>), dim3(grid), dim3(256), 0, st, cam, model, n_visible, pix2, fpack, T, replicas, ticket, sums29, mb, seq, dbg, go, go_seq, v, by_tile, ma); return; }
    if (mode == 1) { hipLaunchKernelGGL((k_icp<false, 1>), dim3(grid), dim3(256), 0, st, cam, model, n_visible, pix2, fpack, T, replicas, ticket, sums29, mb, seq, dbg, go, go_seq, v, by_tile, ma); return; }
#endif
    if (pv) hipLaunchKernelGGL((k_icp<true, 0>), dim3(grid), dim3(256), 0, st, cam, model, n_visible, pix2, fpack, T, replicas, ticket, sums29, mb, seq, dbg, go, go_seq, v, by_tile, ma);
    else hipLaunchKernelGGL((k_icp<false, 0>), dim3(grid), dim3(256), 0, st, cam, model, n_visible, pix2, fpack, T, replicas, ticket, sums29, mb, seq, dbg, go, go_seq, v, by_tile, ma);
}
int icp_resident_max_wgs() { return 1024; }
void launch_icp_resident(hipStream_t st, const Cam& cam, SurfelSoA model, int n_visible, const uint2* pix2, const float4* fpack, const Rt* T0,
                         long long* replicas, long long* sums29, Mailbox* mb, unsigned long long seq0, IcpGo* go, unsigned int go_base,
                         int last_idx, const MatchArgs* match) {
    ScopedKernel sk("icp_resident", st);
    const MatchArgs ma = match ? *match : MatchArgs{0.f, 0.f, 0, nullptr, nullptr, nullptr};
    Rt none; none.R = m3_identity(); none.t = v3(0, 0, 0);
    unsigned long long* counted = reinterpret_cast<unsigned long long*>(replicas) + SSF_ICP_REPLICAS * 32;
    hipLaunchKernelGGL(k_icp_resident, dim3((n_visible + 255) / 256), dim3(256), 0, st, cam, model, n_visible, pix2, fpack, T0 ? *T0 : none, counted, sums29,
                       mb, seq0, go, go_base, T0 ? 1 : 0, last_idx, ma);
}
void launch_match(hipStream_t st, const Cam& cam, SurfelSoA model, int n_visible, const uint2* pix2, const float4* fpack,
                  Rt pose, float zmin, float zmax, long long id_offset,
                  unsigned long long* best, uint8_t* matched, int32_t* cand, int S, const int32_t* orig) {
    (void)S;
    if (n_visible <= 0) return;
    ScopedKernel sk("match", st);
    if (orig) hipLaunchKernelGGL(k_match<true>, dim3((n_visible + 255) / 256), dim3(256), 0, st, cam, model, n_visible, pix2, fpack,
                                 pose, zmin, zmax, id_offset, best, matched, cand, orig);
    else hipLaunchKernelGGL(k_match<false>, dim3((n_visible + 255) / 256), dim3(256), 0, st, cam, model, n_visible, pix2, fpack,
                            pose, zmin, zmax, id_offset, best, matched, cand, orig);
}
void launch_fuse(hipStream_t st, SurfelSoA model, SurfelSoA frame, Rt pose, int stamp, long long id_offset, int n_visible,
                 const AssocTables& at, int do_update, int capacity, const ShardArgs& sh, Counters* cnt, OovStore oov, int span_upper,
                 const ClassifyArgs& ca, uint8_t* state_vis, uint8_t* state_oov, uint32_t* bc_oov, const PartitionWs& ws, int tail_in_move) {
    ScopedKernel sk("update_insert", st);
    const int S = at.S, nchunks = (S + 255) / 256, nb_oov = (span_upper + 255) / 256, nb_vis = (n_visible + 255) / 256;
    const int nupd = (S + UPD_PER_WG - 1) / UPD_PER_WG;
    hipLaunchKernelGGL(k_update_insert, dim3(nupd + nchunks + nb_vis + (nb_oov + OOV_PER_WG - 1) / OOV_PER_WG), dim3(256), 0, st, model,
                       frame, pose, stamp, id_offset,
                       n_visible, at.best, at.matched, at.cand, S, do_update, capacity, sh.rank, sh.nranks, sh.tile, cnt, nupd, nchunks, nb_vis,
                       nb_oov, oov, ca, state_vis, state_oov, bc_oov, ws, sh.migrate, tail_in_move);
}
void launch_pack_emigrants(hipStream_t st, SurfelSoA model, const AssocTables& at, long long id_offset, int n_visible,
                           const uint8_t* state_vis, int do_update, const ShardArgs& sh, int32_t* table) {
    ScopedKernel sk("pack_emigrants", st);
    hipLaunchKernelGGL(k_pack_emigrants, dim3((at.S + 255) / 256), dim3(256), 0, st, model, at.best, at.matched, id_offset, n_visible,
                       state_vis, at.S, do_update, sh.nranks, sh.tile, table);
}
void launch_migrate_in(hipStream_t st, SurfelSoA model, const int32_t* table, int S, int capacity, Counters* cnt, const ShardArgs& sh,
                       const ClassifyArgs& ca, Rt pose, int stamp, uint8_t* state_vis, const PartitionWs& ws) {
    ScopedKernel sk("migrate_in", st);
    hipLaunchKernelGGL(k_migrate_in, dim3(1), dim3(1024), 0, st, model, table, S, sh.rank, capacity, cnt, ca, pose, stamp, state_vis, ws);
}
void launch_first_frame(hipStream_t st, SurfelSoA model, SurfelSoA frame, Rt pose, int S, int capacity, const ShardArgs& sh, Counters* cnt) {
    ScopedKernel sk("first_frame", st);
    hipLaunchKernelGGL(k_first_frame, dim3(1), dim3(1024), 0, st, model, frame, pose, S, capacity, sh.rank, sh.nranks, sh.tile, cnt);
}
void launch_move_rows(hipStream_t st, SurfelSoA vis_src, SurfelSoA vis_dst, OovStore oov, int nv_upper, int span_upper,
                      const uint8_t* state_vis, const uint8_t* state_oov, const uint32_t* bc_oov, const PartitionWs& ws,
                      Counters* cnt, Mailbox* mb, unsigned long long cnt_seq, const NextIcp* next, const P2PView* next_pv,
                      const MoveTotals* totals) {
    const int nb_vis = std::max(1, (nv_upper + 255) / 256), nb_oov = (span_upper + 255) / 256;
    const MoveTotals mt = totals ? *totals : MoveTotals{0, 0, 0, 0};
    auto kernel = !next ? k_move_rows<false, false> : (next_pv ? k_move_rows<true, true> : k_move_rows<true, false>);
    ScopedKernel sk(next ? "reorder_move_icp" : "reorder_move", st);
    hipLaunchKernelGGL(kernel, dim3(nb_vis + nb_oov), dim3(256), 0, st, vis_src, vis_dst, oov, state_vis, state_oov, bc_oov, ws, cnt, nb_vis,
                       next ? *next : NextIcp{}, mb, cnt_seq, next_pv ? *next_pv : P2PView{}, mt);
}
void launch_oov_compact(hipStream_t st, OovStore src, OovStore dst, int span_upper, int new_head, uint32_t* bc_oov, Counters* cnt,
                        int set_span) {
    const int nb = (span_upper + 255) / 256;
    ScopedKernel sk("oov_compact", st);
    if (nb > 0) {
        hipLaunchKernelGGL(k_oov_count, dim3(nb), dim3(256), 0, st, src, bc_oov, cnt);
        hipLaunchKernelGGL(k_oov_scan, dim3(1), dim3(1024), 0, st, bc_oov, nb, cnt);
        hipLaunchKernelGGL(k_oov_compact, dim3(nb), dim3(256), 0, st, src, dst, bc_oov, new_head, cnt);
    }
    if (set_span) hipLaunchKernelGGL(k_oov_set_span, dim3(1), dim3(1), 0, st, cnt, new_head);
}
void launch_align(hipStream_t st, const Cam& cam, const float* spos, const float* slab, const float* snrm, const float* sconf,
                  int n, SurfelSoA frame, const int32_t* label, const float* plane_depth, Rt T, long long* out40) {
    ScopedKernel sk("align_iteration", st);
    hipLaunchKernelGGL(k_align, dim3(1), dim3(1024), 0, st, cam, spos, slab, snrm, sconf, n, frame, label, plane_depth, T, out40);
}
void launch_fern_codes(hipStream_t st, const uint8_t* rgb, const float* depth, int W, int H, const uint32_t* fpos,
                       const uint8_t* frgb, const float* fdepth, int n, uint8_t* codes) {
    if (n <= 0) return;
    hipLaunchKernelGGL(k_fern_codes, dim3((n + 63) / 64), dim3(64), 0, st, rgb, depth, W, H, fpos, frgb, fdepth, n, codes);
}
void launch_p2p_counts(hipStream_t st, const P2PView& pv, const Counters* cnt, Mailbox* mb, unsigned long long all_seq) {
    ScopedKernel sk("p2p_counts", st);
    hipLaunchKernelGGL(k_p2p_counts, dim3(1), dim3(64), 0, st, pv, cnt, mb, all_seq);
}
void launch_p2p_assoc(hipStream_t st, const P2PView& pv, unsigned long long* best, uint8_t* matched, Mailbox* mb) {
    ScopedKernel sk("p2p_assoc", st);
    hipLaunchKernelGGL(k_p2p_assoc, dim3(1), dim3(1024), 0, st, pv, best, matched, mb);
}
void launch_p2p_migrants(hipStream_t st, const P2PView& pv, int32_t* table, unsigned int* ticket, Mailbox* mb) {
    ScopedKernel sk("p2p_migrants", st);
    const int grid = (pv.S + 255) / 256;
    hipLaunchKernelGGL(k_p2p_migr_share, dim3(grid), dim3(256), 0, st, pv, table, ticket);
    hipLaunchKernelGGL(k_p2p_migr_gather, dim3(grid), dim3(256), 0, st, pv, table, mb);
}
void launch_publish_icp(hipStream_t st, const long long* rec, Mailbox* mb, unsigned long long seq) {
    hipLaunchKernelGGL(k_publish_icp, dim3(1), dim3(64), 0, st, rec, mb, seq);
}
void launch_publish_all_counts(hipStream_t st, const int* all5, int nranks, Mailbox* mb, unsigned long long seq) {
    hipLaunchKernelGGL(k_publish_all_counts, dim3(1), dim3(64), 0, st, all5, 5 * nranks, mb, seq);
}
void launch_publish_counts(hipStream_t st, Counters* cnt, int shrink_by_removed, Mailbox* mb, unsigned long long seq) {
    hipLaunchKernelGGL(k_publish_counts, dim3(1), dim3(1), 0, st, cnt, shrink_by_removed, mb, seq);
}
void launch_lab_refresh(hipStream_t st, SurfelSoA s, int n) {
    if (n <= 0) return;
    hipLaunchKernelGGL(k_lab_refresh, dim3((n + 255) / 256), dim3(256), 0, st, s, n);
}
void launch_deformation(hipStream_t st, SurfelSoA model, int n, int m, const float* npos, const float* nrot,
                        const float* ntrans, float* nodes16, const float* w4, const int32_t* idx4) {
    if (n <= 0) return;
    ScopedKernel sk("apply_deformation", st);
    hipLaunchKernelGGL(k_pack_nodes, dim3((m + 255) / 256), dim3(256), 0, st, m, npos, nrot, ntrans, reinterpret_cast<float4*>(nodes16));
    hipLaunchKernelGGL(k_deformation, dim3((n + 255) / 256), dim3(256), 0, st, model, n, reinterpret_cast<const float4*>(nodes16), w4, idx4);
}

// ... 2 lines not shown
```

Baseline: 11980 frames/s.

## Replicate association best-match table per XCC to cut cross-die atomic contention

Adds eight per-XCC replicas of the frame-to-model best-match table. The in-ICP matcher picks its replica from the hardware XCC id and does its atomic-min there, and the fuse and classify readers take the minimum across the base table and all replicas. The goal is to avoid contended atomics on one table across chiplets during matching. In exchange, extraction must initialise nine times as many entries, every fuse lookup reads nine words, and the association buffer grows.

```diff
diff --git a/supersurfel_fusion_amd/csrc/lab/host_probes.inc b/supersurfel_fusion_amd/csrc/lab/host_probes.inc
--- a/supersurfel_fusion_amd/csrc/lab/host_probes.inc
+++ b/supersurfel_fusion_amd/csrc/lab/host_probes.inc
@@ -11,6 +11,7 @@
     return SSF_OK;
 }
 void ssf_dbg_stall_before_match_us(ssf_handle* h, long long us) { if (h) h->dbg_stall_before_match_us = us; }
+long long ssf_dbg_assoc_replica_frames(ssf_handle* h) { return h ? h->n_assoc_replica_frames : -1; }
 int ssf_dbg_host_times(ssf_handle* h, double* out8) {
     if (!h || !out8) return SSF_ERR_INVALID_ARG;
     for (int i = 0; i < 8; i++) { out8[i] = h->host_us[i]; h->host_us[i] = 0; }
@@ -59,7 +60,7 @@
     const int S = (mode & 2) ? 0 : h->S, nvis = (mode & 4) ? 0 : h->n_visible, span = (mode & 1) ? 0 : h->oov_tail - h->oov_head;
     auto launch = [&] {
         ClassifyArgs ca = h->classify; ca.plane_depth = h->cc->maps.plane_depth;
-        launch_fuse(h->stream, M, h->cc->frame, h->pose, h->stamp, h->id_offset, nvis, AssocTables{h->cc->d_best, h->cc->d_matched, h->d_cand, S},
+        launch_fuse(h->stream, M, h->cc->frame, h->pose, h->stamp, h->id_offset, nvis, AssocTables{h->cc->d_best, h->cc->d_matched, h->d_cand, S, 0},
                     (nvis > 0 && S > 0) ? 1 : 0, h->cfg.nb_supersurfels_max, ShardArgs{0, 1, 0, h->cfg.shard_tile}, h->d_cnt,
                     h->oov[h->ocur], span, ca, h->d_state, h->d_state_oov, h->d_bc_oov, ws, 1);
     };
diff --git a/supersurfel_fusion_amd/csrc/ssf_device.hpp b/supersurfel_fusion_amd/csrc/ssf_device.hpp
--- a/supersurfel_fusion_amd/csrc/ssf_device.hpp
+++ b/supersurfel_fusion_amd/csrc/ssf_device.hpp
@@ -183,10 +183,13 @@
 }
 SSF_HD unsigned int icp_go_abort_check(unsigned int want) { return ((want * 0x9E3779B1u) >> 2) & SSF_ICP_GO_CHECK_MASK; }
 #define SSF_ICP_GO_SLOTS 4
-struct MatchArgs { float zmin, zmax; long long id_offset; unsigned long long* best; uint8_t* matched; int32_t* cand; };
-struct ClassifyArgs { Cam cam; const float* plane_depth; int delta_t; float conf_thresh, zmin, zmax; };
+#define SSF_ASSOC_REPLICAS 8
+SSF_HD int assoc_stride(int S) { return (S + 15) & ~15; }
+SSF_HD size_t assoc_table_words(int S) { return (size_t)(1 + SSF_ASSOC_REPLICAS) * (size_t)assoc_stride(S); }
+struct MatchArgs { float zmin, zmax; long long id_offset; unsigned long long* best; uint8_t* matched; int32_t* cand; int rstride; };
+struct ClassifyArgs { Cam cam; const float* plane_depth; int delta_t; float conf_thresh, zmin, zmax; int assoc_rstride; };
 struct ShardArgs { int rank, nranks, migrate; float tile; };
-struct AssocTables { const unsigned long long* best; const uint8_t* matched; const int32_t* cand; int S; };
+struct AssocTables { const unsigned long long* best; const uint8_t* matched; const int32_t* cand; int S; int rstride; };
 int icp_variant_mode();
 void launch_icp(hipStream_t st, const Cam& cam, SurfelSoA model, int n_visible, const uint2* pix2, const float4* fpack,
                 Rt T, long long* replicas, unsigned int* ticket,
diff --git a/supersurfel_fusion_amd/csrc/ssf_extract.hip b/supersurfel_fusion_amd/csrc/ssf_extract.hip
--- a/supersurfel_fusion_amd/csrc/ssf_extract.hip
+++ b/supersurfel_fusion_amd/csrc/ssf_extract.hip
@@ -1100,6 +1100,8 @@
     __syncthreads();
     if (wv != 2 || !active) return;
     best[k] = SSF_NO_MATCH; matched[k] = 0;
+#pragma unroll
+    for (int x = 1; x <= SSF_ASSOC_REPLICAS; x++) best[(size_t)x * assoc_stride(p.S) + k] = SSF_NO_MATCH;
     M3 vecs = m3(v3(0, 0, 0), v3(0, 0, 0), v3(0, 0, 0));
     float d0 = 0.f, d1 = 0.f; int s0 = 0, s1 = 0;
     if (valid) {
@@ -1166,6 +1168,8 @@
     m.fpack[4 * k + 1] = make_float4(r2.x, r2.y, r2.z, 0.f);
     m.fpack[4 * k + 2] = make_float4(pos.x, pos.y, pos.z, 0.f);
     best[k] = SSF_NO_MATCH; matched[k] = 0;
+#pragma unroll
+    for (int x = 1; x <= SSF_ASSOC_REPLICAS; x++) best[(size_t)x * assoc_stride(S) + k] = SSF_NO_MATCH;
 }
 
 __global__ __launch_bounds__(256) void k_export_rows(int S, SurfelSoA f, float* __restrict__ wire, size_t slab) {
diff --git a/supersurfel_fusion_amd/csrc/ssf_handle.hpp b/supersurfel_fusion_amd/csrc/ssf_handle.hpp
--- a/supersurfel_fusion_amd/csrc/ssf_handle.hpp
+++ b/supersurfel_fusion_amd/csrc/ssf_handle.hpp
@@ -264,6 +264,10 @@
     Mailbox* mb_host = nullptr; Mailbox* mb_dev = nullptr;
     unsigned long long icp_seq = 0, cnt_seq = 0;
     struct { bool valid = false; unsigned long long seq = 0; ExtractCtx* ctx = nullptr; int slot = 0; int stamp = 0; Rt pose; } ahead;
+    int assoc_rstride = 0;
+#ifdef SSF_EXPERIMENTS
+    long long n_assoc_replica_frames = 0;
+#endif
     double wait_launched_us = 0.0; long long n_waiter_match_repairs = 0; long long dbg_stall_before_match_us = 0;
     bool icp_ahead = true; int icp_ahead_mode = 1;
     AheadTuner ahead_tuner;
diff --git a/supersurfel_fusion_amd/csrc/ssf_host.hip b/supersurfel_fusion_amd/csrc/ssf_host.hip
--- a/supersurfel_fusion_amd/csrc/ssf_host.hip
+++ b/supersurfel_fusion_amd/csrc/ssf_host.hip
@@ -779,7 +779,7 @@
             ws.ticket = h->d_part_ticket; ws.other = h->d_part + (size_t)(h->part_set ^ 1) * h->part_words; ws.words = h->part_words;
             h->part_set ^= 1;
         }
-        const AssocTables at{h->cc->d_best, h->cc->d_matched, h->d_cand, h->S};
+        const AssocTables at{h->cc->d_best, h->cc->d_matched, h->d_cand, h->S, h->assoc_rstride};
         launch_fuse(h->stream, M, h->cc->frame, h->pose, h->stamp, h->id_offset, h->n_visible, at, nvis_g > 0 ? 1 : 0,
                     h->cfg.nb_supersurfels_max, h->shard, h->d_cnt, h->oov[h->ocur], h->oov_tail - h->oov_head, h->classify,
                     h->d_state, h->d_state_oov, h->d_bc_oov, ws, h->fuse_totals.from_tot);
@@ -893,6 +893,13 @@
     static const bool off = SSF_ENV_SET("NO_MATCH_IN_WAITER");
     return !off && single_shard_alone(h) && h->cfg.profile == 0 && icp_variant_mode() == 0;
 }
+static int assoc_replica_stride(const ssf_handle* h) {
+#ifdef SSF_EXPERIMENTS
+    static const bool off = SSF_ENV_INT("ASSOC_REPLICAS", 1) == 0;
+    if (off) return 0;
+#endif
+    return (icp_waiter_can_match(h) && !h->bins.valid) ? assoc_stride(h->S) : 0;
+}
 static int icp_launch_waiting(ssf_handle* h, IcpWaiter& w) {
     w.seq_rec = ++h->icp_seq;
     w.go_seq = ++h->go_count;
@@ -900,7 +907,7 @@
     h->wait_launched_us = now_us();
     Rt none; none.R = m3_identity(); none.t = v3(0, 0, 0);
     const P2PView pv = h->p2p.view;
-    const MatchArgs ma{h->cfg.range_min, h->cfg.range_max, h->id_offset, h->cc->d_best, h->cc->d_matched, h->d_cand};
+    const MatchArgs ma{h->cfg.range_min, h->cfg.range_max, h->id_offset, h->cc->d_best, h->cc->d_matched, h->d_cand, h->assoc_rstride};
     const int rc = icp_issue(h, none, w.seq_rec, nullptr, w.slot, w.go_seq, h->p2p.on ? &pv : nullptr, icp_waiter_can_match(h) ? &ma : nullptr);
     w.waiting = rc == SSF_OK;
     return rc;
@@ -916,7 +923,7 @@
     h->go_count += (unsigned long long)last;
     w.resident = true; w.slot = lines + 1; w.go_seq = go_base + 1;
     h->wait_launched_us = now_us();
-    const MatchArgs ma{h->cfg.range_min, h->cfg.range_max, h->id_offset, h->cc->d_best, h->cc->d_matched, h->d_cand};
+    const MatchArgs ma{h->cfg.range_min, h->cfg.range_max, h->id_offset, h->cc->d_best, h->cc->d_matched, h->d_cand, h->assoc_rstride};
     launch_icp_resident(h->stream, h->cam, h->model[h->mcur], h->n_visible, h->cc->maps.pix2, h->cc->maps.fpack, T0, h->d_icp_replicas, h->d_icp, h->mb_dev,
                         seq0, lines, (unsigned int)go_base, last, icp_waiter_can_match(h) ? &ma : nullptr);
     HCK(hipGetLastError());
@@ -1021,6 +1028,9 @@
 #endif
         icp_release_waiting(w.slot, w.go_seq, &h->pose, 0, true);
         matched_by_waiter = true;
+#ifdef SSF_EXPERIMENTS
+        if (h->assoc_rstride) h->n_assoc_replica_frames++;
+#endif
         if (now_us() - h->wait_launched_us > 100000.0) { matched_by_waiter = false; h->n_waiter_match_repairs++; }
     } else {
         if (w.waiting) icp_release_waiting(w.slot, w.go_seq, nullptr);
@@ -1082,10 +1092,12 @@
     if (exchanges_natively(h)) { rc = comm_counts(h); if (rc) return rc; }
     icp_begin(h, prior);
     rc = h->bins.make_if_large(h);
+    h->assoc_rstride = rc ? 0 : assoc_replica_stride(h);
     if (!rc) rc = icp_chains(h) ? icp_loop_chained(h, f) : icp_loop_plain(h, f);
     if (!rc) rc = icp_loop_end(h, f);
     ssf_frame_result r;
     if (!rc) rc = exchange_and_fuse(h, &r);
+    h->assoc_rstride = 0;
     if (rc) return rc;
     if (h->pending.empty()) h->ahead_tuner.sequence_break(); else h->ahead_tuner.frame_done(now_us(), r.icp_iters);
     h->host_us[1] += f.t_b - f.t_a; h->host_us[2] += now_us() - f.t_b; h->host_us[3] += 1;
@@ -1347,7 +1359,7 @@
         SurfelSoA& f = c.frame;
         take(f.pos, 3 * S); take(f.col, 3 * S); take(f.lab, 3 * S); take(f.stamps, 2 * S); take(f.r0, 3 * S); take(f.r1, 3 * S);
         take(f.r2, 3 * S); take(f.shape, 6 * S); take(f.dims, 2 * S); take(f.conf, S);
-        take(c.d_best, S); take(c.d_matched, S); take(c.d_rgb_in, 4 * P); take(c.d_depth_in, P); take(c.d_depth_filt, P); take(c.d_mask, S);
+        take(c.d_best, assoc_table_words(S)); take(c.d_matched, S); take(c.d_rgb_in, 4 * P); take(c.d_depth_in, P); take(c.d_depth_filt, P); take(c.d_mask, S);
         take(c.d_wire, 26 * S);
         take(c.d_pixmask, P); take(c.d_pixcnt, 2 * S);
         return (off + 255) & ~(size_t)255;
diff --git a/supersurfel_fusion_amd/csrc/ssf_track_fuse.hip b/supersurfel_fusion_amd/csrc/ssf_track_fuse.hip
--- a/supersurfel_fusion_amd/csrc/ssf_track_fuse.hip
+++ b/supersurfel_fusion_amd/csrc/ssf_track_fuse.hip
@@ -333,6 +333,21 @@
         ma.cand[oid] = match_values(cam, a.w, v3(a.x, a.y, a.z), v3(c.x, c.y, c.z), v3(b.x, b.y, b.z), oid, pix2, fpack, pose, ma.zmin, ma.zmax, ma.id_offset, ma.best, ma.matched, true);
     }
 }
+__device__ __forceinline__ unsigned long long* assoc_bid_table(const MatchArgs& ma) {
+    const unsigned int xcc = __builtin_amdgcn_s_getreg((3 << 11) | (0 << 6) | 20) & 7u;
+    return ma.rstride ? ma.best + (size_t)(1u + xcc) * (size_t)ma.rstride : ma.best;
+}
+__device__ __forceinline__ unsigned long long assoc_best(const unsigned long long* __restrict__ best, int f, int rstride) {
+    unsigned long long v = best[f];
+    if (rstride) {
+        unsigned long long r[SSF_ASSOC_REPLICAS];
+#pragma unroll
+        for (int x = 0; x < SSF_ASSOC_REPLICAS; x++) r[x] = best[(size_t)(1 + x) * (size_t)rstride + f];
+#pragma unroll
+        for (int x = 0; x < SSF_ASSOC_REPLICAS; x++) v = r[x] < v ? r[x] : v;
+    }
+    return v;
+}
 #define SSF_ICP_DBG_COUNTED 0x40000000
 #ifndef SSF_ICP_GO_WAIT_TICKS
 #define SSF_ICP_GO_WAIT_TICKS 25000000ull
@@ -407,9 +422,11 @@
                 T.R = m3(v3(sT(0), sT(1), sT(2)), v3(sT(3), sT(4), sT(5)), v3(sT(6), sT(7), sT(8)));
                 T.t = v3(sT(9), sT(10), sT(11));
                 if constexpr (MODE == 3) { if (ma.best) match_sorted_rows(cam, model, n_visible, pix2, fpack, T, ma); return; }
-                if (ma.best && !by_tile)
+                if (ma.best && !by_tile) {
+                    unsigned long long* const bid = assoc_bid_table(ma);
                     for (int id = blockIdx.x * WG + threadIdx.x; id < n_visible; id += n_wg * WG)
-                        ma.cand[id] = match_row(cam, model, id, id, pix2, fpack, T, ma.zmin, ma.zmax, ma.id_offset, ma.best, ma.matched);
+                        ma.cand[id] = match_row(cam, model, id, id, pix2, fpack, T, ma.zmin, ma.zmax, ma.id_offset, bid, ma.matched);
+                }
                 return;
             }
         }
@@ -503,7 +520,7 @@
             auto sT = [&](int i) { return __uint_as_float(__builtin_amdgcn_readfirstlane(__float_as_uint(s_T[i]))); };
             Rt P; P.R = m3(v3(sT(0), sT(1), sT(2)), v3(sT(3), sT(4), sT(5)), v3(sT(6), sT(7), sT(8)));
             P.t = v3(sT(9), sT(10), sT(11));
-            if (ma.best && live) ma.cand[id] = match_values(cam, m_conf, mpos, mnrm, mlab, id, pix2, fpack, P, ma.zmin, ma.zmax, ma.id_offset, ma.best, ma.matched, false);
+            if (ma.best && live) ma.cand[id] = match_values(cam, m_conf, mpos, mnrm, mlab, id, pix2, fpack, P, ma.zmin, ma.zmax, ma.id_offset, assoc_bid_table(ma), ma.matched, false);
             return;
         }
         T.R = m3(v3(s_T[0], s_T[1], s_T[2]), v3(s_T[3], s_T[4], s_T[5]), v3(s_T[6], s_T[7], s_T[8]));
@@ -690,7 +707,7 @@
     __builtin_amdgcn_s_setprio(3);
     if constexpr (SORTED) {
         (void)orig;
-        const MatchArgs ma{zmin, zmax, id_offset, best, matched, cand};
+        const MatchArgs ma{zmin, zmax, id_offset, best, matched, cand, 0};
         match_sorted_rows(cam, model, n_visible, pix2, fpack, pose, ma);
         return;
     } else {
@@ -811,7 +828,7 @@
     const int f = wv == 0 ? f0 + (l >> 1) : f0 + (wv - 1) * 16 + (l >> 2);
     if (f >= S) return;
     unsigned int mt = matched[f];
-    unsigned long long bk = best[f];
+    unsigned long long bk = assoc_best(best, f, ca.assoc_rstride);
     float f_conf = F.conf[f];
     V3 f_pos = v3(0.f, 0.f, 0.f), f_lab = v3(0.f, 0.f, 0.f);
     Sym3 f_shape = sym3(0.f, 0.f, 0.f, 0.f, 0.f, 0.f);
@@ -1019,7 +1036,7 @@
             int f = cand[i];
             float conf = M.conf[i]; int seen = M.stamps[2 * (size_t)i + 1]; V3 pos = ld3(M.pos, (size_t)i);
             asm volatile("" : "+v"(f), "+v"(conf), "+v"(seen), "+v"(pos.x));
-            const bool rewritten = do_update && f >= 0 && (uint32_t)(best[f] & 0xFFFFFFFFull) == (uint32_t)(id_offset + i);
+            const bool rewritten = do_update && f >= 0 && (uint32_t)(assoc_best(best, f, ca.assoc_rstride) & 0xFFFFFFFFull) == (uint32_t)(id_offset + i);
             if (!rewritten) {
                 cls = classify_values(ca.cam, conf, seen, pos, pose, ca.plane_depth, stamp, ca.delta_t, ca.conf_thresh, ca.zmin, ca.zmax);
                 if (cls == 2) M.conf[i] = -1.0f;
@@ -1326,8 +1343,9 @@
     int32_t w[SSF_MIGRANT_WORDS];
 #pragma unroll
     for (int i = 0; i < SSF_MIGRANT_WORDS; i++) w[i] = 0;
-    if (do_update && matched[f] && best[f] != SSF_NO_MATCH) {
-        const long long local = (long long)(uint32_t)(best[f] & 0xFFFFFFFFull) - id_offset;
+    const unsigned long long bk = assoc_best(best, f, 0);
+    if (do_update && matched[f] && bk != SSF_NO_MATCH) {
+        const long long local = (long long)(uint32_t)(bk & 0xFFFFFFFFull) - id_offset;
         if (local >= 0 && local < n_visible) {
             const size_t m = (size_t)local;
             const float conf = M.conf[m];
@@ -1779,7 +1797,7 @@
                 long long* sums29, Mailbox* mb, unsigned long long seq, int dbg_arg, IcpGo* go, unsigned long long go_seq,
                 const P2PView* pv, int by_tile, const MatchArgs* match) {
     ScopedKernel sk("icp_accumulate", st);
-    const MatchArgs ma = match ? *match : MatchArgs{0.f, 0.f, 0, nullptr, nullptr, nullptr};
+    const MatchArgs ma = match ? *match : MatchArgs{0.f, 0.f, 0, nullptr, nullptr, nullptr, 0};
     const int mode = dbg_arg > 0 && dbg_arg != 4 ? 0 : icp_variant_mode();
     const int per_lane = mode == 1 ? std::max(2, SSF_ENV_INT("ICP_PER_LANE", 0)) : 1;
     const int per_block = 256 * per_lane;
@@ -1804,7 +1822,7 @@
                          long long* replicas, long long* sums29, Mailbox* mb, unsigned long long seq0, IcpGo* go, unsigned int go_base,
                          int last_idx, const MatchArgs* match) {
     ScopedKernel sk("icp_resident", st);
-    const MatchArgs ma = match ? *match : MatchArgs{0.f, 0.f, 0, nullptr, nullptr, nullptr};
+    const MatchArgs ma = match ? *match : MatchArgs{0.f, 0.f, 0, nullptr, nullptr, nullptr, 0};
     Rt none; none.R = m3_identity(); none.t = v3(0, 0, 0);
     unsigned long long* counted = reinterpret_cast<unsigned long long*>(replicas) + SSF_ICP_REPLICAS * 32;
     hipLaunchKernelGGL(k_icp_resident, dim3((n_visible + 255) / 256), dim3(256), 0, st, cam, model, n_visible, pix2, fpack, T0 ? *T0 : none, counted, sums29,
@@ -1827,10 +1845,11 @@
     ScopedKernel sk("update_insert", st);
     const int S = at.S, nchunks = (S + 255) / 256, nb_oov = (span_upper + 255) / 256, nb_vis = (n_visible + 255) / 256;
     const int nupd = (S + UPD_PER_WG - 1) / UPD_PER_WG;
+    ClassifyArgs cr = ca; cr.assoc_rstride = at.rstride;
     hipLaunchKernelGGL(k_update_insert, dim3(nupd + nchunks + nb_vis + (nb_oov + OOV_PER_WG - 1) / OOV_PER_WG), dim3(256), 0, st, model,
                        frame, pose, stamp, id_offset,
                        n_visible, at.best, at.matched, at.cand, S, do_update, capacity, sh.rank, sh.nranks, sh.tile, cnt, nupd, nchunks, nb_vis,
-                       nb_oov, oov, ca, state_vis, state_oov, bc_oov, ws, sh.migrate, tail_in_move);
+                       nb_oov, oov, cr, state_vis, state_oov, bc_oov, ws, sh.migrate, tail_in_move);
 }
 void launch_pack_emigrants(hipStream_t st, SurfelSoA model, const AssocTables& at, long long id_offset, int n_visible,
                            const uint8_t* state_vis, int do_update, const ShardArgs& sh, int32_t* table) {
```

Result: faster. 12490 frames/s, median of 6 (+4.2%).
